# mazrk7/gmvae

Hardware: NVIDIA B200
Metric: GMVAE train samples/sec (fwd+bwd+Adam) (higher is better)
Workload: dtype bf16

## Files before the change

### gmvae_b200/csrc/chain_sched.cuh

```cuda
#pragma once

#if defined(__CUDACC__)
#define GMVAE_SCHED_FN __host__ __device__ __forceinline__
#else
#define GMVAE_SCHED_FN inline
#endif

namespace gmvae {
namespace tc {

constexpr int CHAIN_MAX_DEPS = 4;
constexpr int CHAIN_EPI_BYTES = 128;
constexpr int CHAIN_EPI2_BYTES = 64;
constexpr int SCHED_BLOCK_M = 128;

struct ChainDep { int base, target, by_k, nblocks, seg2; };

struct alignas(16) ChainJob {
  int a1, b1, a2, b2;
  int c;
  int d;
  int gw;
  int M, N, kb1, kb2, kb_per_split, num_splits;
  int block_n, a_mn, b_mn, kind;
  int tiles_n, tiles_mn, total_tiles, tile_base;
  int sig_base;
  int ndeps;
  int epi_dep;
  ChainDep deps[CHAIN_MAX_DEPS];
  alignas(16) unsigned char epi[CHAIN_EPI_BYTES];
  int rot;
  int walk_total;
  int tiles_mn2;
  int wfirst, wcount;
  int share;
  int fuse;
  int zslice;
  alignas(16) unsigned char epi2[CHAIN_EPI2_BYTES];
};
template <int CL>
GMVAE_SCHED_FN void chain_tile(const ChainJob& J, int l, int crank, int& z, int& mb, int& n0) {
  int mn;
  if (CL == 4) {
    z = l / J.tiles_mn2;
    mn = 2 * (l - z * J.tiles_mn2) + (crank >> 1);
  } else {
    z = l / J.tiles_mn;
    mn = l - z * J.tiles_mn;
  }
  int pm = mn / J.tiles_n;
  int nt = mn - pm * J.tiles_n;
  if (CL == 4 && mn >= J.tiles_mn) { pm = J.tiles_mn / J.tiles_n; nt = 0; }
  if (J.rot) { nt += pm % J.tiles_n; if (nt >= J.tiles_n) nt -= J.tiles_n; }
  n0 = nt * J.block_n;
  mb = CL >= 2 ? 2 * pm + (crank & 1) : pm;
}

template <int MUL>
GMVAE_SCHED_FN bool chain_walk(const ChainJob& J, int c, int G, int& first, int& stride) {
  int wf = J.wfirst * MUL, wc = J.wcount * MUL;
  if (wc <= 0 || wf + wc > G) { wf = 0; wc = G; }
  const int cj = c - wf;
  if (cj < 0 || cj >= wc) return false;
  stride = wc;
  first = ((cj - J.tile_base) % wc + wc) % wc;
  return true;
}

inline void chain_job_geometry(ChainJob& J, int M, int N, int block_n, int split_k, int kb_total, bool a_mn, int cl) {
  const int tiles_m = (M + SCHED_BLOCK_M - 1) / SCHED_BLOCK_M, tiles_n = (N + block_n - 1) / block_n;
  const int tiles_m_walk = cl >= 2 ? (tiles_m + 1) / 2 : tiles_m;
  if (split_k < 1) split_k = 1;
  const int per = (kb_total + split_k - 1) / split_k;
  split_k = (kb_total + per - 1) / per;
  J.M = M; J.N = N; J.kb_per_split = per; J.num_splits = split_k;
  J.block_n = block_n; J.a_mn = a_mn ? 1 : 0;
  J.tiles_n = tiles_n; J.tiles_mn = tiles_m_walk * tiles_n; J.total_tiles = J.tiles_mn * split_k;
  J.tiles_mn2 = (J.tiles_mn + 1) / 2;
  J.walk_total = cl == 4 ? J.tiles_mn2 * split_k : J.total_tiles;
  J.share = (cl == 4 && tiles_n % 2 == 0) ? 1 : 0;
  J.rot = (tiles_n > 1 && N % block_n != 0 && !a_mn) ? 1 : 0;
}
GMVAE_SCHED_FN int det_slice_ld(int N) { return (N + 3) / 4 * 4; }
GMVAE_SCHED_FN long long det_slice_index(int z, int m, int n, int M, int ld) { return ((long long)z * M + m) * ld + n; }
GMVAE_SCHED_FN void det_tile_region(const ChainJob& J, int mb, int n0, int& r0, int& r1, int& c0, int& c1) {
  r0 = mb * SCHED_BLOCK_M; r1 = r0 + SCHED_BLOCK_M < J.M ? r0 + SCHED_BLOCK_M : J.M;
  c0 = n0; c1 = n0 + J.block_n < J.N ? n0 + J.block_n : J.N;
  if (r1 < r0) r1 = r0;
}

inline int chain_job_counters(int M, int cl) {
  const int tiles_m = (M + SCHED_BLOCK_M - 1) / SCHED_BLOCK_M;
  return cl >= 2 ? 2 * ((tiles_m + 1) / 2) + (cl == 4 ? 2 : 0) : tiles_m;
}

}
}
```

### gmvae_b200/csrc/engine.cu

```cuda
#include <nccl.h>

#include <algorithm>
#include <cstdio>
#include <cstdlib>
#include <cstring>
#include <functional>
#include <map>
#include <mutex>
#include <string>
#include <tuple>
#include <type_traits>
#include <vector>

#include "../../include/gmvae_abi.h"
#include "common.cuh"
#include "epilogue.cuh"
#include "gemm_simt.cuh"
#include "gemm_tc.cuh"
#include "gemm_chain.cuh"
#include "kernels.cuh"
#include "input.cuh"
#include "peer.cuh"

namespace gmvae {

bool g_use_pdl = true;
static thread_local std::string g_last_error;
void set_error(const std::string& msg) { g_last_error = msg; }

namespace tc {
EncodeTiledFn get_encode_fn() {
  static EncodeTiledFn fn = nullptr;
  static std::once_flag once;
  std::call_once(once, [] {
    void* p = nullptr;
    cudaDriverEntryPointQueryResult q;
    if (cudaGetDriverEntryPoint("cuTensorMapEncodeTiled", &p, cudaEnableDefault, &q) == cudaSuccess &&
        q == cudaDriverEntryPointSuccess)
      fn = reinterpret_cast<EncodeTiledFn>(p);
  });
  return fn;
}

long long* g_trace = nullptr;

int g_reserved_sms = 0;

int current_device() { int dev = 0; cudaGetDevice(&dev); return dev < 0 ? 0 : dev % 64; }
int num_sms() {
  static int n_by_dev[64] = {};
  int& n = n_by_dev[current_device()];
  if (n == 0) {
    int dev = 0;
    cudaGetDevice(&dev);
    cudaDeviceGetAttribute(&n, cudaDevAttrMultiProcessorCount, dev);
    if (n <= 0) n = 148;
  }
  return std::max(8, n - g_reserved_sms);
}

int make_tmap(CUtensorMap* out, const void* ptr, int elem_bytes, uint64_t inner, uint64_t outer, uint64_t outer_stride,
              uint32_t box_inner, uint32_t box_outer, int swizzle) {
  typedef std::tuple<const void*, int, uint64_t, uint64_t, uint64_t, uint32_t, uint32_t, int> Key;
  static thread_local std::map<Key, CUtensorMap> cache;
  Key key(ptr, elem_bytes, inner, outer, outer_stride, box_inner, box_outer, swizzle);
  auto it = cache.find(key);
  if (it != cache.end()) { *out = it->second; return 0; }
  EncodeTiledFn fn = get_encode_fn();
  GM_REQUIRE(fn != nullptr, "cuTensorMapEncodeTiled not available from the driver");
  GM_REQUIRE((reinterpret_cast<uintptr_t>(ptr) & 15) == 0, "TMA operand base must be 16-byte aligned");
  GM_REQUIRE((outer_stride * (uint64_t)elem_bytes) % 16 == 0, "TMA operand row stride must be a multiple of 16 bytes");
  cuuint64_t gdim[2] = {inner, outer};
  cuuint64_t gstride[1] = {outer_stride * (uint64_t)elem_bytes};
  cuuint32_t box[2] = {box_inner, box_outer};
  cuuint32_t estr[2] = {1, 1};
  const CUtensorMapDataType dt = elem_bytes == 2 ? CU_TENSOR_MAP_DATA_TYPE_BFLOAT16 : elem_bytes == 4 ? CU_TENSOR_MAP_DATA_TYPE_FLOAT32
                                                                                                      : CU_TENSOR_MAP_DATA_TYPE_UINT8;
  const CUtensorMapSwizzle sw = swizzle == 128 ? CU_TENSOR_MAP_SWIZZLE_128B : swizzle == 64 ? CU_TENSOR_MAP_SWIZZLE_64B
                                                                                             : CU_TENSOR_MAP_SWIZZLE_NONE;
  CUresult r = fn(out, dt, 2, const_cast<void*>(ptr), gdim, gstride, box, estr, CU_TENSOR_MAP_INTERLEAVE_NONE, sw,
                  CU_TENSOR_MAP_L2_PROMOTION_L2_256B, CU_TENSOR_MAP_FLOAT_OOB_FILL_NONE);
  if (r != CUDA_SUCCESS) {
    set_error("cuTensorMapEncodeTiled failed with CUresult " + std::to_string((int)r));
    return -3;
  }
  if (cache.size() > 4096) cache.clear();
  cache[key] = *out;
  return 0;
}
int make_tmap_bf16(CUtensorMap* out, const void* ptr, uint64_t inner, uint64_t outer, uint64_t outer_stride,
                   uint32_t box_inner, uint32_t box_outer) {
  return make_tmap(out, ptr, 2, inner, outer, outer_stride, box_inner, box_outer, 128);
}
int make_tmap_slices_f32(CUtensorMap* out, const void* ptr, uint64_t inner, uint64_t outer, uint64_t slices, uint64_t ld,
                         uint32_t box_inner, uint32_t box_outer) {
  EncodeTiledFn fn = get_encode_fn();
  GM_REQUIRE(fn != nullptr, "cuTensorMapEncodeTiled not available from the driver");
  GM_REQUIRE((reinterpret_cast<uintptr_t>(ptr) & 15) == 0 && ld % 4 == 0, "TMA slices need 16-byte aligned rows");
  cuuint64_t gdim[3] = {inner, outer, slices};
  cuuint64_t gstride[2] = {ld * 4, outer * ld * 4};
  cuuint32_t box[3] = {box_inner, box_outer, 1};
  cuuint32_t estr[3] = {1, 1, 1};
  CUresult r = fn(out, CU_TENSOR_MAP_DATA_TYPE_FLOAT32, 3, const_cast<void*>(ptr), gdim, gstride, box, estr, CU_TENSOR_MAP_INTERLEAVE_NONE,
                  CU_TENSOR_MAP_SWIZZLE_64B, CU_TENSOR_MAP_L2_PROMOTION_L2_256B, CU_TENSOR_MAP_FLOAT_OOB_FILL_NONE);
  if (r != CUDA_SUCCESS) {
    set_error("cuTensorMapEncodeTiled (slices) failed with CUresult " + std::to_string((int)r));
    return -3;
  }
  return 0;
}
}

static inline int round_up(int v, int m) { return (v + m - 1) / m * m; }

struct Linear {
  int in = 0, out = 0;
  int64_t w_off = 0, b_off = 0;
  bf16* w_bf16 = nullptr;  int ld_w = 0;
};
struct Mlp {
  std::string name;
  std::vector<Linear> layers;
};

struct LinView {
  const float* w; float* dw; const float* b; float* db;
  int in, out, ldw32;
  const bf16* w_bf16; int ld_w;
};

enum { DBG_NO_TC = 1, DBG_NO_TC_WGRAD = 2, DBG_NO_TWO_SEG = 4, DBG_SYNC_EACH = 8, DBG_BN128 = 16, DBG_NO_FUSED_COLSUM = 32,
       DBG_NO_PDL = 128, DBG_NO_CHAIN = 512, DBG_NO_ROW_JOBS = 1024, DBG_NO_SPREAD = 4096, DBG_NO_FUSE_HEADS = 16384,
       DBG_COMM_OVERLAP = 32768 ,
       DBG_ROW_JOBS = 8192 ,
       DBG_NO_PAIR = 65536 ,
       DBG_NO_QUAD = 131072 ,
       DBG_WG_LATE = 262144 ,
       DBG_NO_PARTITION = 524288 ,
       DBG_NO_RELU_BITS = 2048  };
enum { PC_START = -1, PC_TC_GEMM = 0, PC_TC_WGRAD = 1, PC_SIMT_GEMM = 2, PC_HEADS = 3, PC_BIAS_GRAD = 4, PC_ADAM = 5, PC_MISC = 6,
       PC_COMM = 7, PC_COUNT = 8 };

}

using namespace gmvae;

struct gmvae_handle {
  gmvae_config cfg;
  int D, Z, K, L;
  std::vector<int> hidden;
  std::vector<gmvae_param_desc> table;
  int64_t n_params = 0;
  Mlp prior_gmm, decoder, encoder_y, encoder;
  int64_t loc_off = -1, raw_scale_off = -1, mix_off = -1;
  float *params = nullptr, *grads = nullptr, *adam_m = nullptr, *adam_v = nullptr;
  uint8_t* ws = nullptr; size_t ws_bytes = 0;
  struct Buf { size_t off = 0, bytes = 0; };
  std::map<std::string, Buf> bufs;
  size_t ws_needed = 0;
  std::vector<ShadowEntry> shadow_host;
  ShadowEntry* shadow_dev = nullptr; int shadow_tiles = 0;
  DeviceState* state = nullptr;
  uint64_t seed_host = 0;
  bool grads_clean = false;
  bool graph_has_memset = true;
  uint64_t draws = 0;
  bool in_train_step = false;
  int64_t launches = 0;
  int debug_flags = 0;
  bool profiling = false;
  std::vector<std::pair<cudaEvent_t, int>> marks;
  ncclComm_t comm = nullptr; int world = 1, rank = 0;
  cudaStream_t comm_stream = nullptr;
  cudaEvent_t comm_ev[8] = {nullptr, nullptr, nullptr, nullptr, nullptr, nullptr, nullptr, nullptr};
  int comm_ev_next = 0;
  bool overlap_comm = false;
  bool peer_ready = false;
  void* peer_region = nullptr;
  void* peer_mapped[peer::MAX_WORLD] = {};
  long long peer_timeout_cycles = 0;
  float* grads_bound = nullptr;
  peer::Layout peer_layout;
  peer::Peers peer_ptrs;
  int64_t reduced_upto = 0;
  int64_t bucket_end[2] = {0, 0};
  int chunk_samples = 0;
  bool chain_on = false;
  tc::ChainParams chain;
  struct ChainWriter { const char* lo; const char* hi; int job; };
  std::vector<ChainWriter> chain_writers;
  int chain_tiles = 0;
  int max_quads = 0;
  int* chain_counters = nullptr; int chain_counter_cap = 0, chain_counter_next = 0;
  long long* chain_trace = nullptr; int chain_trace_cta = 0, chain_launch_idx = 0;
  unsigned long long* chain_jobstat = nullptr;
  std::vector<int> chain_jobdesc;
  bool chain_flush_after = false;
  bool row_jobs = false;
  bool quad_opt_in = false;
  int chain_split_opt = 0;
  int wide_bn = 0;
  std::vector<std::function<int()>>* wg_late = nullptr;
  int cur_part = 0, part_chain_walkers = 0, part_walkers = 0, part_tiles[3] = {0, 0, 0};
  bool part_on = false, part_last_mlp = false, part_tail = false;
  bool chain_quad = false;
  bool chain_pair = false;
  struct FuseReq { int kind = 0; unsigned char prm[tc::CHAIN_EPI2_BYTES]; std::vector<std::pair<const void*, size_t>> writes; bool consumed = false; };
  FuseReq fuse_next;
  bool last_gemm_chained = false;
  std::map<const void*, bool> relu_bits_valid;
  bool det = false;
  std::vector<DetSeg> det_segs;
  std::vector<std::function<int()>> det_colsums;
  int64_t det_part_next = 0, det_part_cap = 0;
  int64_t det_wg_next = 0, det_wg_cap = 0;
  cudaGraphExec_t graph_exec = nullptr;

  bool bf16_mode() const { return cfg.precision == GMVAE_PRECISION_BF16; }
  size_t act_size() const { return bf16_mode() ? 2 : 4; }
  template <typename T> T* buf(const std::string& name) const {
    auto it = bufs.find(name);
    return it == bufs.end() ? nullptr : reinterpret_cast<T*>(ws + it->second.off);
  }
};

namespace gmvae {

static void add_param(gmvae_handle* h, const std::string& name, int rows, int cols, int64_t* off_out) {
  gmvae_param_desc d;
  memset(&d, 0, sizeof(d));
  snprintf(d.name, GMVAE_NAME_LEN, "%s", name.c_str());
  d.offset = h->n_params; d.rows = rows; d.cols = cols;
  h->table.push_back(d);
  if (off_out) *off_out = h->n_params;
  h->n_params += round_up(rows * cols, 4);
}

static void build_mlp(gmvae_handle* h, Mlp& m, const std::string& name, int in, const std::vector<int>& sizes) {
  m.name = name;
  int prev = in;
  for (size_t i = 0; i < sizes.size(); ++i) {
    Linear l; l.in = prev; l.out = sizes[i];
    add_param(h, name + "_fcnet/linear_" + std::to_string(i) + "/w", l.in, l.out, &l.w_off);
    add_param(h, name + "_fcnet/linear_" + std::to_string(i) + "/b", 1, l.out, &l.b_off);
    m.layers.push_back(l);
    prev = sizes[i];
  }
}

static void plan_buf(gmvae_handle* h, const std::string& name, size_t bytes) {
  gmvae_handle::Buf b; b.off = h->ws_needed; b.bytes = bytes;
  h->bufs[name] = b;
  h->ws_needed += (bytes + 255) / 256 * 256;
}

static void plan_mlp_bufs(gmvae_handle* h, const Mlp& m, size_t B, size_t asz) {
  for (size_t i = 0; i + 1 < m.layers.size(); ++i) {
    plan_buf(h, m.name + ".h" + std::to_string(i), B * round_up(m.layers[i].out, 8) * asz);
    plan_buf(h, m.name + ".dh" + std::to_string(i), B * round_up(m.layers[i].out, 8) * asz);
    plan_buf(h, m.name + ".bits" + std::to_string(i), (size_t)round_up((int)B, 32) * (size_t)((m.layers[i].out + 31) / 32) * 4);
  }
}

static void plan_shadows(gmvae_handle* h, Mlp& m) {
  for (auto& l : m.layers) {
    l.ld_w = round_up(l.out, 8);
    plan_buf(h, "shadow.w." + std::to_string(l.w_off), (size_t)l.in * l.ld_w * 2);
  }
}

constexpr int DET_ROW_BLOCKS = 64;
static int wgrad_split(const gmvae_handle* h, int in, int out, int M, bool pair, bool quad);

static int plan(gmvae_handle* h) {
  const gmvae_config& c = h->cfg;
  h->D = c.data_size; h->Z = c.latent_size; h->K = c.model == GMVAE_MODEL_VAE ? 1 : c.mixture_components;
  h->hidden.assign(c.hidden_sizes, c.hidden_sizes + c.num_hidden);
  h->L = c.num_hidden + 1;
  const int D = h->D, Z = h->Z, K = h->K;
  auto with = [&](int last) { std::vector<int> v = h->hidden; v.push_back(last); return v; };
  if (c.model == GMVAE_MODEL_GMVAE) {
    build_mlp(h, h->decoder, "decoder", Z, with(D));
    h->bucket_end[0] = h->n_params;
    build_mlp(h, h->encoder, "encoder_gmm", D + K, with(2 * Z));
    build_mlp(h, h->prior_gmm, "prior_gmm", K, std::vector<int>{2 * Z});
    h->bucket_end[1] = h->n_params;
    build_mlp(h, h->encoder_y, "encoder_y", D, with(K));
  } else {
    build_mlp(h, h->decoder, "decoder", Z, with(D));
    h->bucket_end[0] = h->n_params;
    if (c.model == GMVAE_MODEL_VAE_GMP) {
      add_param(h, "loc", K, Z, &h->loc_off);
      add_param(h, "raw_scale_diag", K, Z, &h->raw_scale_off);
      add_param(h, "mixture_logits", 1, K, &h->mix_off);
    }
    h->bucket_end[1] = h->n_params;
    build_mlp(h, h->encoder, "encoder", D, with(2 * Z));
  }
  const size_t Bfull = (size_t)c.max_batch, asz = h->act_size();
  const int Kp = round_up(K, 8);
  h->chunk_samples = (int)Bfull;
  if (c.objective == GMVAE_OBJECTIVE_MARGINAL) {
    const char* env = getenv("GMVAE_M_CHUNK_ROWS");
    long max_rows = env ? atol(env) : 131072;
    long bc = std::max(1L, max_rows / K);
    if (bc > 64) bc = bc / 64 * 64;
    h->chunk_samples = (int)std::min<long>((long)Bfull, bc);
  }
  const size_t B = c.objective == GMVAE_OBJECTIVE_MARGINAL ? (size_t)h->chunk_samples * K : Bfull;
  plan_buf(h, "x_act", Bfull * round_up(D, 8) * asz);
  plan_buf(h, "eps", Bfull * (c.objective == GMVAE_OBJECTIVE_MARGINAL ? K : 1) * Z * 4);
  plan_buf(h, "dec.dlogits", B * round_up(D, 8) * asz);
  plan_buf(h, "dz", B * Z * 4);
  plan_buf(h, "enc_out", B * 2 * Z * 4);
  plan_buf(h, "d_enc_out", B * round_up(2 * Z, 8) * asz);
  plan_buf(h, "z_act", B * round_up(Z, 8) * asz);
  plan_mlp_bufs(h, h->decoder, B, asz);
  plan_mlp_bufs(h, h->encoder, B, asz);
  if (c.model == GMVAE_MODEL_GMVAE) {
    plan_mlp_bufs(h, h->encoder_y, Bfull, asz);
    plan_buf(h, "u", Bfull * K * 4);
    plan_buf(h, "logits_y", Bfull * K * 4);
    plan_buf(h, "y_f32", Bfull * K * 4);
    plan_buf(h, "y_act", Bfull * Kp * asz);
    plan_buf(h, "dlogits_y", Bfull * Kp * asz);
    const size_t H0 = (size_t)(h->hidden.empty() ? 2 * Z : h->hidden[0]);
    if (c.objective == GMVAE_OBJECTIVE_MARGINAL) {
      plan_buf(h, "tab", (size_t)K * 2 * Z * 4);
      plan_buf(h, "dtab", (size_t)K * 2 * Z * 4);
      plan_buf(h, "xproj", Bfull * H0 * 4);
      plan_buf(h, "dxproj", Bfull * round_up((int)H0, 8) * asz);
      plan_buf(h, "rec", Bfull * K * 8);
      plan_buf(h, "klrow", Bfull * K * 4);
    } else {
      plan_buf(h, "prior_out", Bfull * 2 * Z * 4);
      plan_buf(h, "d_prior_out", Bfull * round_up(2 * Z, 8) * asz);
      plan_buf(h, "dy", Bfull * K * 4);
      plan_buf(h, "pre_y", Bfull * H0 * 4);
    }
  }
  if (c.model == GMVAE_MODEL_VAE_GMP) {
    plan_buf(h, "z_f32", B * Z * 4);
    plan_buf(h, "dz_prior", B * Z * 4);
  }
  if (h->bf16_mode()) {
    plan_shadows(h, h->decoder); plan_shadows(h, h->encoder);
    if (c.model == GMVAE_MODEL_GMVAE) { plan_shadows(h, h->encoder_y); plan_shadows(h, h->prior_gmm); }
  }
  plan_buf(h, "infer.acc", ACC_SLOTS * 4);
  if (c.deterministic) {
    int64_t cols = 0;
    for (const Mlp* m : {&h->decoder, &h->encoder, &h->encoder_y, &h->prior_gmm})
      for (const Linear& l : m->layers) cols += l.out;
    h->det_part_cap = cols * DET_ROW_BLOCKS;
    plan_buf(h, "det.part", (size_t)h->det_part_cap * 4);
    plan_buf(h, "det.fx", (size_t)(3 + (c.model == GMVAE_MODEL_VAE_GMP ? K + 2 * K * Z : 0)) * 16);
    h->det_wg_cap = 0;
    for (const Mlp* m : {&h->decoder, &h->encoder, &h->encoder_y, &h->prior_gmm})
      for (size_t i = 0; i < m->layers.size(); ++i) {
        const Linear& l = m->layers[i];
        std::vector<int> views{l.in};
        if (m == &h->encoder && i == 0 && c.model == GMVAE_MODEL_GMVAE) views = {D, K};
        for (int in : views) {
          const int kb = (int)((Bfull + tc::BLOCK_K - 1) / tc::BLOCK_K);
          int S = 1;
          for (bool pair : {false, true}) S = std::max(S, wgrad_split(h, in, l.out, (int)Bfull, pair, false));
          S = std::min(S, kb);
          h->det_wg_cap += round_up((int)std::min<int64_t>((int64_t)S * in * tc::det_slice_ld(l.out), 1LL << 30), 64);
        }
      }
    plan_buf(h, "det.wg", (size_t)h->det_wg_cap * 4);
  }
  h->chain_counter_cap = 64 * (int)((Bfull + 127) / 128 + 2);
  plan_buf(h, "chain.counters", (size_t)h->chain_counter_cap * 4);
  return 0;
}

static LinView view(const gmvae_handle* h, const Linear& l, int row0 = 0, int rows = -1) {
  if (rows < 0) rows = l.in - row0;
  LinView v;
  v.w = h->params + l.w_off + (int64_t)row0 * l.out;
  v.dw = h->grads + l.w_off + (int64_t)row0 * l.out;
  v.b = h->params + l.b_off; v.db = h->grads + l.b_off;
  v.in = rows; v.out = l.out; v.ldw32 = l.out;
  v.w_bf16 = l.w_bf16 ? l.w_bf16 + (int64_t)row0 * l.ld_w : nullptr; v.ld_w = l.ld_w;
  return v;
}

static int profile_mark(gmvae_handle* h, cudaStream_t st, int cls) {
  cudaEvent_t e;
  GM_CHECK_CUDA(cudaEventCreate(&e));
  GM_CHECK_CUDA(cudaEventRecord(e, st));
  h->marks.emplace_back(e, cls);
  return 0;
}

static int chain_flush(gmvae_handle* h, cudaStream_t st);
static int comm_bucket(gmvae_handle* h, cudaStream_t st, int64_t upto) {
  if (!h->comm || h->world == 1 || !h->overlap_comm || upto <= h->reduced_upto) return 0;
  GM_TRY(chain_flush(h, st));
  cudaEvent_t ev = h->comm_ev[h->comm_ev_next++ % 8];
  GM_CHECK_CUDA(cudaEventRecord(ev, st));
  GM_CHECK_CUDA(cudaStreamWaitEvent(h->comm_stream, ev, 0));
  ncclResult_t r = ncclAllReduce(h->grads + h->reduced_upto, h->grads + h->reduced_upto, (size_t)(upto - h->reduced_upto), ncclFloat,
                                 ncclSum, h->comm, h->comm_stream);
  if (r != ncclSuccess) { set_error(std::string("ncclAllReduce: ") + ncclGetErrorString(r)); return -5; }
  h->reduced_upto = upto;
  h->launches++;
  return 0;
}

#define GM_LAUNCHED(h, st, cls)                                              \
  do {                                                                       \
    (h)->launches++;                                                         \
    if ((h)->profiling) GM_TRY(profile_mark(h, st, cls));                    \
    if ((h)->debug_flags & DBG_SYNC_EACH) GM_CHECK_CUDA(cudaStreamSynchronize(st)); \
  } while (0)

static inline bool aligned16(const void* p) { return (reinterpret_cast<uintptr_t>(p) & 15) == 0; }
static inline int kpad(int k, int64_t ld) { return (int)std::min<int64_t>(ld, round_up(k, 8)); }

template <typename TA>
static bool tc_ok_fwd(const gmvae_handle* h, const TA* A, int64_t lda, const LinView& L) {
  return std::is_same<TA, bf16>::value && h->bf16_mode() && !(h->debug_flags & DBG_NO_TC) && L.w_bf16 && lda % 8 == 0 &&
         aligned16(A) && aligned16(L.w_bf16);
}
template <typename TD>
static bool tc_ok_dgrad(const gmvae_handle* h, const TD* dY, int64_t ldy, const LinView& L) {
  return std::is_same<TD, bf16>::value && h->bf16_mode() && !(h->debug_flags & DBG_NO_TC) && L.w_bf16 && ldy % 8 == 0 &&
         aligned16(dY) && aligned16(L.w_bf16);
}


static int pair_max_clusters(gmvae_handle* h, int* out) {
  static int max_clusters_by_dev[64] = {};
  int& max_clusters = max_clusters_by_dev[tc::current_device()];
  if (max_clusters == 0) {
    GM_CHECK_CUDA(cudaFuncSetAttribute(tc::gemm_chain_kernel<tc::ChainParams, 2>, cudaFuncAttributeMaxDynamicSharedMemorySize, tc::CHAIN_SMEM_BYTES));
    cudaLaunchConfig_t qc = {};
    qc.gridDim = dim3(tc::num_sms() & ~1); qc.blockDim = dim3(tc::NUM_THREADS2); qc.dynamicSmemBytes = tc::CHAIN_SMEM_BYTES;
    cudaLaunchAttribute qa[1];
    qa[0].id = cudaLaunchAttributeClusterDimension; qa[0].val.clusterDim.x = 2; qa[0].val.clusterDim.y = 1; qa[0].val.clusterDim.z = 1;
    qc.attrs = qa; qc.numAttrs = 1;
    int n = 0;
    GM_CHECK_CUDA(cudaOccupancyMaxActiveClusters(&n, tc::gemm_chain_kernel<tc::ChainParams, 2>, &qc));
    GM_REQUIRE(n >= 1, "the device cannot co-schedule a CTA pair of the chained kernel");
    max_clusters = n;
  }
  *out = max_clusters;
  return 0;
}

static int chain_flush(gmvae_handle* h, cudaStream_t st) {
  h->chain_flush_after = false;
  h->last_gemm_chained = false;
  if (h->chain.njobs == 0) return 0;
  static bool attr_set_by_dev[64] = {};
  bool& attr_set = attr_set_by_dev[tc::current_device()];
  if (!attr_set) {
    GM_CHECK_CUDA(cudaFuncSetAttribute(tc::gemm_chain_kernel<tc::ChainParams, 1>, cudaFuncAttributeMaxDynamicSharedMemorySize, tc::CHAIN_SMEM_BYTES));
    GM_CHECK_CUDA(cudaFuncSetAttribute(tc::gemm_chain_kernel<tc::ChainParamsSmall, 1>, cudaFuncAttributeMaxDynamicSharedMemorySize, tc::CHAIN_SMEM_BYTES));
    attr_set = true;
  }
  h->chain.counters = h->chain_counters;
  h->chain.trace = (h->chain_trace && h->chain_launch_idx < 8) ? h->chain_trace + (size_t)h->chain_launch_idx * 64 * 16 : nullptr;
  h->chain.trace_cta = h->chain_trace_cta;
  { static const int abl = getenv("GMVAE_CHAIN_ABL") ? atoi(getenv("GMVAE_CHAIN_ABL")) : 0; h->chain.abl = abl; }
  h->chain.jobstat = (h->chain_jobstat && h->chain_launch_idx == 0) ? h->chain_jobstat : nullptr;
  if (h->chain.jobstat) {
    h->chain_jobdesc.clear();
    for (int j = 0; j < h->chain.njobs; ++j) {
      const tc::ChainJob& J = h->chain.jobs[j];
      const int d[8] = {J.kind, J.M, J.N, J.kb1 + J.kb2, J.total_tiles, J.num_splits, J.block_n, J.ndeps};
      h->chain_jobdesc.insert(h->chain_jobdesc.end(), d, d + 8);
    }
  }
  h->chain_launch_idx++;
  if (h->chain_quad) {
    const int clusters = std::max(1, std::min(h->chain_tiles, h->max_quads));
    GM_CHECK_CUDA(launch_k_cluster(tc::gemm_chain_kernel<tc::ChainParams, 4>, dim3(4 * clusters), dim3(tc::NUM_THREADS2), (size_t)tc::CHAIN_SMEM_BYTES, st, true, 4,
                           h->chain));
  } else if (h->chain_pair) {
    int max_clusters = 0;
    GM_TRY(pair_max_clusters(h, &max_clusters));
    const int pairs = std::max(1, std::min(std::min(h->chain_tiles, tc::num_sms() / 2), max_clusters));
    GM_CHECK_CUDA(launch_k_cluster(tc::gemm_chain_kernel<tc::ChainParams, 2>, dim3(2 * pairs), dim3(tc::NUM_THREADS2), (size_t)tc::CHAIN_SMEM_BYTES, st, true, 2,
                           h->chain));
  } else {
  const int grid = std::min(h->chain_tiles, tc::num_sms());
  if (h->chain.njobs <= tc::CHAIN_SMALL_JOBS && h->chain.nmaps <= tc::CHAIN_SMALL_MAPS) {
    static tc::ChainParamsSmall small;
    small.njobs = h->chain.njobs; small.nmaps = h->chain.nmaps; small.counters = h->chain.counters;
    small.trace = h->chain.trace; small.trace_cta = h->chain.trace_cta; small.jobstat = h->chain.jobstat; small.abl = h->chain.abl;
    memcpy(small.maps, h->chain.maps, sizeof(CUtensorMap) * h->chain.nmaps);
    memcpy(small.jobs, h->chain.jobs, sizeof(tc::ChainJob) * h->chain.njobs);
    GM_CHECK_CUDA(launch_k(tc::gemm_chain_kernel<tc::ChainParamsSmall, 1>, dim3(grid), dim3(tc::NUM_THREADS2), (size_t)tc::CHAIN_SMEM_BYTES, st, true, small));
  } else {
    GM_CHECK_CUDA(launch_k(tc::gemm_chain_kernel<tc::ChainParams, 1>, dim3(grid), dim3(tc::NUM_THREADS2), (size_t)tc::CHAIN_SMEM_BYTES, st, true, h->chain));
  }
  }
  h->chain.njobs = 0; h->chain.nmaps = 0; h->chain_tiles = 0; h->chain_writers.clear();
  h->launches++;
  if (h->profiling) GM_TRY(profile_mark(h, st, 0 ));
  if (h->debug_flags & DBG_SYNC_EACH) GM_CHECK_CUDA(cudaStreamSynchronize(st));
  return 0;
}

template <typename T, int MODE> static void writer_range(const EpiStore<T, MODE>& e, int M, const char*& lo, const char*& hi) {
  lo = reinterpret_cast<const char*>(e.out); hi = lo + (int64_t)M * e.ld * sizeof(T);
}
template <typename T> static void writer_range(const EpiBCE<T>& e, int M, const char*& lo, const char*& hi) {
  lo = reinterpret_cast<const char*>(e.dlogits); hi = lo + (int64_t)M * e.ld * sizeof(T);
}
template <typename T, typename HT> static void writer_range(const EpiReluMask<T, HT>& e, int M, const char*& lo, const char*& hi) {
  lo = reinterpret_cast<const char*>(e.out); hi = lo + (int64_t)M * e.ld * sizeof(T);
}
static void writer_range(const EpiAtomicAdd&, int, const char*& lo, const char*& hi) { lo = hi = nullptr; }

struct ChainIO { const void* out; int64_t ld; int elem; const void* opnd; int64_t ld_opnd; bool ok; };
static ChainIO chain_io(const EpiStore<bf16, EPI_PLAIN>& e) { return {e.out, e.ld, 2, nullptr, 0, true}; }
static ChainIO chain_io(const EpiStore<float, EPI_PLAIN>& e) { return {nullptr, e.ld, 4, nullptr, 0, true}; }
static ChainIO chain_io(const EpiBCE<bf16>& e) {
  return {e.dlogits, e.ld, 2, nullptr, 0, e.row_weight == nullptr && e.row_sum == nullptr && e.x_row_div == 1};
}
static ChainIO chain_io(const EpiReluMask<bf16, bf16>& e) { return {e.out, e.ld, 2, e.h, e.ldh, true}; }
static ChainIO chain_io(const EpiAtomicAdd& e) {
  const bool tma = e.ld % 4 == 0 && (reinterpret_cast<uintptr_t>(e.out) & 15) == 0;
  return {tma ? e.out : nullptr, e.ld, 4, nullptr, 0, true};
}

template <class Epi>
static int chain_add(gmvae_handle* h, const tc::Operand& A1, const tc::Operand& B1, const tc::Operand* A2, const tc::Operand* B2,
                     int M, int N, int block_n, bool a_mn, bool b_mn, int split_k, const Epi& epi, cudaStream_t st) {
  static_assert(tc::epi_kind<Epi>::value != tc::EK_NONE, "epilogue not supported by the chained kernel");
  static_assert(sizeof(Epi) <= tc::CHAIN_EPI_BYTES, "epilogue parameters do not fit the job record");
  const bool pair = h->chain_pair, quad = h->chain_quad;
  const void* reads[4] = {A1.ptr, A2 ? A2->ptr : nullptr, a_mn ? (const void*)B1.ptr : nullptr, epi.read_ptr()};
  tc::ChainDep deps[tc::CHAIN_MAX_DEPS]; int ndeps = 0, epi_dep = -1;
  bool need_flush = h->chain.njobs >= tc::CHAIN_MAX_JOBS || h->chain.nmaps + 6 > tc::CHAIN_MAX_MAPS;
  for (int i = 0; i < 4 && !need_flush; ++i) {
    const char* p = reinterpret_cast<const char*>(reads[i]);
    if (!p) continue;
    for (const auto& w : h->chain_writers) {
      if (p < w.lo || p >= w.hi) continue;
      const tc::ChainJob& P = h->chain.jobs[w.job];
      if (p != w.lo || P.sig_base < 0) { need_flush = true; break; }
      int dup = -1;
      for (int d = 0; d < ndeps; ++d) if (deps[d].base == P.sig_base) dup = d;
      if (dup >= 0) {
        if (i == 3) { if (deps[dup].by_k) { need_flush = true; break; } epi_dep = dup; }
        if (i != 1) deps[dup].seg2 = 0;
        continue;
      }
      if (ndeps == tc::CHAIN_MAX_DEPS) { need_flush = true; break; }
      if (i == 3) epi_dep = ndeps;
      const bool by_k = a_mn && i != 3;
      deps[ndeps++] = tc::ChainDep{P.sig_base, tc::EPI_WARPS * P.tiles_n * P.num_splits, by_k ? 1 : 0, (P.M + tc::BLOCK_M - 1) / tc::BLOCK_M,
                                   (i == 1 && !a_mn) ? 1 : 0};
    }
  }
  if (need_flush) { GM_TRY(chain_flush(h, st)); ndeps = 0; epi_dep = -1; }
  tc::ChainJob& J = h->chain.jobs[h->chain.njobs];
  auto mk = [&](int* idx, const tc::Operand& o, bool mn, int box_rows) -> int {
    CUtensorMap* m = &h->chain.maps[h->chain.nmaps];
    *idx = h->chain.nmaps++;
    if (mn) return tc::make_tmap_bf16(m, o.ptr, (uint64_t)o.rows, (uint64_t)o.k, (uint64_t)o.ld, 64, tc::BLOCK_K);
    return tc::make_tmap_bf16(m, o.ptr, (uint64_t)o.k, (uint64_t)o.rows, (uint64_t)o.ld, tc::BLOCK_K, (uint32_t)box_rows);
  };
  const int b_box_rows = pair ? block_n / 2 : block_n;
  GM_REQUIRE(!pair || block_n % 16 == 0, "pair tiles need a tile width that is a multiple of 16");
  const int a_box_rows = quad ? 64 : tc::BLOCK_M;
  GM_TRY(mk(&J.a1, A1, a_mn, a_box_rows));
  GM_TRY(mk(&J.b1, B1, b_mn, b_box_rows));
  J.kb1 = (A1.k + tc::BLOCK_K - 1) / tc::BLOCK_K; J.kb2 = 0;
  if (A2 && B2) {
    GM_TRY(mk(&J.a2, *A2, a_mn, a_box_rows));
    GM_TRY(mk(&J.b2, *B2, b_mn, b_box_rows));
    J.kb2 = (A2->k + tc::BLOCK_K - 1) / tc::BLOCK_K;
  } else {
    J.a2 = J.a1; J.b2 = J.b1;
  }
  const int kb_total = J.kb1 + J.kb2;
  tc::chain_job_geometry(J, M, N, block_n, split_k, kb_total, a_mn, quad ? 4 : pair ? 2 : 1);
  J.b_mn = b_mn ? 1 : 0; J.kind = tc::epi_kind<Epi>::value;
  J.tile_base = h->chain_tiles;
  {
    const int part = h->part_on ? h->cur_part : 0;
    J.wfirst = part == 2 ? h->part_chain_walkers : 0;
    J.wcount = part == 1 ? h->part_chain_walkers : part == 2 ? h->part_walkers - h->part_chain_walkers : 0;
    J.tile_base = part == 0 ? h->chain_tiles : h->part_tiles[part];
    h->part_tiles[part] += J.walk_total;
  }
  J.ndeps = ndeps; J.epi_dep = epi_dep;
  for (int d = 0; d < ndeps; ++d) J.deps[d] = deps[d];
  const char *lo, *hi;
  writer_range(epi, M, lo, hi);
  J.sig_base = -1;
  if (lo) {
    const int ncount = tc::chain_job_counters(M, quad ? 4 : pair ? 2 : 1);
    if (h->chain_counter_next + ncount <= h->chain_counter_cap) {
      J.sig_base = h->chain_counter_next; h->chain_counter_next += ncount;
    } else {
      h->chain_flush_after = true;
    }
    h->chain_writers.push_back({lo, hi, h->chain.njobs});
  }
  const ChainIO io = chain_io(epi);
  J.gw = 0; J.c = J.a1; J.d = J.a1;
  J.zslice = (h->det && tc::epi_kind<Epi>::value == tc::EK_ATOMIC) ? 1 : 0;
  GM_REQUIRE(!J.zslice || io.out, "deterministic mode: weight-gradient slices need 16-byte rows");
  if (io.out) {
    J.gw = io.elem == 2 ? 2 : 1;
    J.d = h->chain.nmaps++;
    if (J.zslice)
      GM_TRY(tc::make_tmap_slices_f32(&h->chain.maps[J.d], io.out, (uint64_t)N, (uint64_t)M, (uint64_t)J.num_splits, (uint64_t)io.ld, 16, 32));
    else
      GM_TRY(tc::make_tmap(&h->chain.maps[J.d], io.out, io.elem, (uint64_t)N, (uint64_t)M, (uint64_t)io.ld, io.elem == 2 ? 32 : 16, 32, 64));
    if (io.opnd) {
      J.c = h->chain.nmaps++;
      GM_TRY(tc::make_tmap(&h->chain.maps[J.c], io.opnd, 2, (uint64_t)N, (uint64_t)M, (uint64_t)io.ld_opnd, 32, 32, 64));
    }
  }
  memset(J.epi, 0, sizeof(J.epi));
  memcpy(J.epi, &epi, sizeof(Epi));
  J.fuse = 0;
  if (h->fuse_next.kind != 0 && tc::epi_kind<Epi>::value == tc::EK_STORE_F32 && N <= 16 && J.sig_base >= 0) {
    J.fuse = h->fuse_next.kind;
    memcpy(J.epi2, h->fuse_next.prm, sizeof(J.epi2));
    for (const auto& w : h->fuse_next.writes)
      if (w.first) h->chain_writers.push_back({reinterpret_cast<const char*>(w.first), reinterpret_cast<const char*>(w.first) + w.second, h->chain.njobs});
    h->fuse_next.consumed = true;
  }
  h->chain_tiles += J.walk_total;
  h->chain.njobs++;
  h->last_gemm_chained = true;
  if (h->chain_flush_after) GM_TRY(chain_flush(h, st));
  return 0;
}
template <class P>
static int chain_add_rows(gmvae_handle* h, int kind, const P& prm, int M, std::initializer_list<const void*> reads,
                          std::initializer_list<std::pair<const void*, size_t>> writes, cudaStream_t st, int sub = 1) {
  static_assert(sizeof(P) <= tc::CHAIN_EPI_BYTES, "row-job parameters do not fit the job record");
  const int tiles_m = (M + tc::BLOCK_M - 1) / tc::BLOCK_M;
  tc::ChainDep deps[tc::CHAIN_MAX_DEPS]; int ndeps = 0;
  bool need_flush = h->chain.njobs >= tc::CHAIN_MAX_JOBS;
  for (const void* r : reads) {
    const char* p = reinterpret_cast<const char*>(r);
    if (!p || need_flush) continue;
    for (const auto& w : h->chain_writers) {
      if (p < w.lo || p >= w.hi) continue;
      const tc::ChainJob& Pj = h->chain.jobs[w.job];
      if (p != w.lo || Pj.sig_base < 0) { need_flush = true; break; }
      bool dup = false;
      for (int d = 0; d < ndeps; ++d) dup = dup || deps[d].base == Pj.sig_base;
      if (dup) continue;
      if (ndeps == tc::CHAIN_MAX_DEPS) { need_flush = true; break; }
      deps[ndeps++] = tc::ChainDep{Pj.sig_base, tc::EPI_WARPS * Pj.tiles_n * Pj.num_splits, 0, (Pj.M + tc::BLOCK_M - 1) / tc::BLOCK_M, 0};
    }
  }
  if (need_flush) { GM_TRY(chain_flush(h, st)); ndeps = 0; }
  tc::ChainJob& J = h->chain.jobs[h->chain.njobs];
  memset(&J, 0, sizeof(J));
  J.M = M; J.N = 0; J.kind = kind; J.num_splits = 1;
  J.tiles_n = sub; J.tiles_mn = tiles_m * sub; J.total_tiles = tiles_m * sub; J.tile_base = (h->chain_quad ? 4 : h->chain_pair ? 2 : 1) * h->chain_tiles;
  {
    const int cl = h->chain_quad ? 4 : h->chain_pair ? 2 : 1;
    const int part = h->part_on ? h->cur_part : 0;
    J.wfirst = part == 2 ? h->part_chain_walkers : 0;
    J.wcount = part == 1 ? h->part_chain_walkers : part == 2 ? h->part_walkers - h->part_chain_walkers : 0;
    if (part != 0) J.tile_base = cl * h->part_tiles[part];
    h->part_tiles[part] += (tiles_m * sub + cl - 1) / cl;
  }
  J.ndeps = ndeps; J.epi_dep = -1;
  for (int d = 0; d < ndeps; ++d) J.deps[d] = deps[d];
  J.sig_base = -1;
  if (h->chain_counter_next + tiles_m <= h->chain_counter_cap) {
    J.sig_base = h->chain_counter_next; h->chain_counter_next += tiles_m;
  } else {
    h->chain_flush_after = true;
  }
  for (const auto& w : writes)
    if (w.first) h->chain_writers.push_back({reinterpret_cast<const char*>(w.first), reinterpret_cast<const char*>(w.first) + w.second, h->chain.njobs});
  memcpy(J.epi, &prm, sizeof(P));
  { const int cl = h->chain_quad ? 4 : h->chain_pair ? 2 : 1; h->chain_tiles += (J.total_tiles + cl - 1) / cl; }
  h->chain.njobs++;
  if (h->chain_flush_after) GM_TRY(chain_flush(h, st));
  return 0;
}
template <class Epi> struct chainable { static constexpr bool value = tc::epi_kind<Epi>::value != tc::EK_NONE; };

template <class Epi, bool B_MN = false>
static int tc_dispatch_kk(gmvae_handle* h, const tc::Operand& A, const tc::Operand& B, const tc::Operand* A2,
                          const tc::Operand* B2, int M, int N, const Epi& epi, cudaStream_t st) {
  int r;
  if constexpr (chainable<Epi>::value) {
    if (h->chain_on && chain_io(epi).ok) {
      const bool f32 = tc::epi_kind<Epi>::value == tc::EK_STORE_F32;
      int bn = (!B_MN && f32 && N <= 16) ? 16 : (!B_MN && f32 && N <= 32) ? 32 : N <= 64 ? 64 : (N <= 128 || (h->debug_flags & DBG_BN128)) ? 128 : 256;
      if (bn == 256 && h->wide_bn > 0 && N > h->wide_bn) bn = h->wide_bn;
      return chain_add(h, A, B, A2, B2, M, N, bn, false, B_MN, 1, epi, st);
    }
  }
  GM_TRY(chain_flush(h, st));
  if constexpr (B_MN) {
    if (N <= 64) r = tc::launch_gemm_tc<64, false, true, Epi>(A, B, A2, B2, M, N, 1, epi, st);
    else if (N <= 128 || (h->debug_flags & DBG_BN128)) r = tc::launch_gemm_tc<128, false, true, Epi>(A, B, A2, B2, M, N, 1, epi, st);
    else r = tc::launch_gemm_tc<256, false, true, Epi>(A, B, A2, B2, M, N, 1, epi, st);
  } else {
    if (N <= 16) r = tc::launch_gemm_tc<16, false, false, Epi>(A, B, A2, B2, M, N, 1, epi, st);
    else if (N <= 32) r = tc::launch_gemm_tc<32, false, false, Epi>(A, B, A2, B2, M, N, 1, epi, st);
    else if (N <= 64) r = tc::launch_gemm_tc<64, false, false, Epi>(A, B, A2, B2, M, N, 1, epi, st);
    else if (N <= 128 || (h->debug_flags & DBG_BN128)) r = tc::launch_gemm_tc<128, false, false, Epi>(A, B, A2, B2, M, N, 1, epi, st);
    else r = tc::launch_gemm_tc<256, false, false, Epi>(A, B, A2, B2, M, N, 1, epi, st);
  }
  if (r == 0) GM_LAUNCHED(h, st, PC_TC_GEMM);
  return r;
}

template <typename TA, class Epi, bool ALLOW_TC = true>
static int lin_fwd(gmvae_handle* h, const TA* A, int64_t lda, int M, const LinView& L, const Epi& epi, cudaStream_t st,
                   const TA* A2 = nullptr, int64_t lda2 = 0, const LinView* L2 = nullptr) {
  if constexpr (ALLOW_TC && std::is_same<TA, bf16>::value) {
    bool ok = tc_ok_fwd<TA>(h, A, lda, L);
    if (L2) ok = ok && lda2 % 8 == 0 && aligned16(A2) && aligned16(L2->w_bf16);
    if (ok) {
      tc::Operand a{A, lda, M, kpad(L.in, lda)}, b{L.w_bf16, L.ld_w, L.out, L.in};
      if (L2) {
        tc::Operand a2{A2, lda2, M, kpad(L2->in, lda2)}, b2{L2->w_bf16, L2->ld_w, L2->out, L2->in};
        return tc_dispatch_kk<Epi, true>(h, a, b, &a2, &b2, M, L.out, epi, st);
      }
      return tc_dispatch_kk<Epi, true>(h, a, b, nullptr, nullptr, M, L.out, epi, st);
    }
  }
  GM_REQUIRE(L2 == nullptr, "two-segment forward requires the tensor-core path");
  GM_TRY(chain_flush(h, st));
  GM_CHECK_CUDA((launch_gemm_simt<TA, float, Epi>(A, lda, 1, L.w, L.ldw32, 1, M, L.out, L.in, 1, epi, st)));
  GM_LAUNCHED(h, st, PC_SIMT_GEMM);
  return 0;
}

template <typename TD, class Epi>
static int lin_dgrad(gmvae_handle* h, const TD* dY, int64_t ldy, int M, const LinView& L, const Epi& epi, cudaStream_t st,
                     const TD* dY2 = nullptr, int64_t ldy2 = 0, const LinView* L2 = nullptr) {
  if constexpr (std::is_same<TD, bf16>::value) {
    bool ok = tc_ok_dgrad<TD>(h, dY, ldy, L);
    if (L2) ok = ok && tc_ok_dgrad<TD>(h, dY2, ldy2, *L2) && L2->in == L.in;
    if (ok) {
      tc::Operand a{dY, ldy, M, kpad(L.out, ldy)}, b{L.w_bf16, L.ld_w, L.in, kpad(L.out, L.ld_w)};
      if (L2) {
        tc::Operand a2{dY2, ldy2, M, kpad(L2->out, ldy2)}, b2{L2->w_bf16, L2->ld_w, L2->in, kpad(L2->out, L2->ld_w)};
        return tc_dispatch_kk(h, a, b, &a2, &b2, M, L.in, epi, st);
      }
      return tc_dispatch_kk(h, a, b, nullptr, nullptr, M, L.in, epi, st);
    }
  }
  GM_REQUIRE(L2 == nullptr, "two-segment data gradient requires the tensor-core path");
  GM_TRY(chain_flush(h, st));
  GM_CHECK_CUDA((launch_gemm_simt<TD, float, Epi>(dY, ldy, 1, L.w, 1, L.ldw32, M, L.in, L.out, 1, epi, st)));
  GM_LAUNCHED(h, st, PC_SIMT_GEMM);
  return 0;
}

static int wgrad_bn(const gmvae_handle* h, int out) { return out <= 64 ? 64 : (out <= 128 || (h->debug_flags & DBG_BN128)) ? 128 : 256; }
static int wgrad_split(const gmvae_handle* h, int in, int out, int M, bool pair, bool quad) {
  const int bn = wgrad_bn(h, out);
  const int tiles = pair ? ((in + 255) / 256) * ((out + bn - 1) / bn) : ((in + 127) / 128) * ((out + bn - 1) / bn);
  const int kb = (M + tc::BLOCK_K - 1) / tc::BLOCK_K;
  const int walkers = quad ? h->max_quads : pair ? tc::num_sms() / 2 : tc::num_sms(), units = quad ? (tiles + 1) / 2 : tiles;
  return std::max(1, std::min(std::max(1, kb / 4), walkers / units));
}

template <typename TA, typename TD>
static int lin_wgrad(gmvae_handle* h, const TA* A, int64_t lda, const TD* dY, int64_t ldy, int M, const LinView& L,
                     cudaStream_t st) {
  EpiAtomicAdd epi{L.dw, (int64_t)L.ldw32};
  if constexpr (std::is_same<TA, bf16>::value && std::is_same<TD, bf16>::value) {
    bool ok = h->bf16_mode() && !(h->debug_flags & (DBG_NO_TC | DBG_NO_TC_WGRAD)) && lda % 8 == 0 && ldy % 8 == 0 &&
              aligned16(A) && aligned16(dY);
    if (ok) {
      tc::Operand a{A, lda, kpad(L.in, lda), M}, b{dY, ldy, kpad(L.out, ldy), M};
      const int bn = wgrad_bn(h, L.out);
      const bool pair = h->chain_on && h->chain_pair;
      const int split = wgrad_split(h, L.in, L.out, M, pair, pair && h->chain_quad);
      if (h->chain_on) {
        EpiAtomicAdd e = epi;
        if (h->det) {
          const int kb = (M + tc::BLOCK_K - 1) / tc::BLOCK_K, per = (kb + split - 1) / split, S = (kb + per - 1) / per;
          const int ld = tc::det_slice_ld(L.out);
          const int64_t need = round_up((int)std::min<int64_t>((int64_t)S * L.in * ld, 1LL << 30), 64);
          GM_REQUIRE(h->det_wg_next + need <= h->det_wg_cap && (int)h->det_segs.size() < DET_MAX_SEGS,
                     "deterministic mode: out of weight-gradient partial space");
          float* part = h->buf<float>("det.wg") + h->det_wg_next;
          h->det_wg_next += need;
          e = EpiAtomicAdd{part, (int64_t)ld};
          h->det_segs.push_back(DetSeg{L.dw, part, nullptr, (long long)L.in * ld, L.in, L.out, S, L.ldw32, ld, 0});
        }
        const int saved_part = h->cur_part;
        if (saved_part == 1) h->cur_part = h->part_tail ? 0 : 2;
        const int r = chain_add(h, a, b, nullptr, nullptr, L.in, L.out, bn, true, true, split, e, st);
        h->cur_part = saved_part;
        return r;
      }
      GM_REQUIRE(!h->det, "deterministic mode: weight gradients outside the chained kernel");
      GM_TRY(chain_flush(h, st));
      int r = bn == 64    ? tc::launch_gemm_tc<64, true, true, EpiAtomicAdd>(a, b, nullptr, nullptr, L.in, L.out, split, epi, st)
              : bn == 128 ? tc::launch_gemm_tc<128, true, true, EpiAtomicAdd>(a, b, nullptr, nullptr, L.in, L.out, split, epi, st)
                          : tc::launch_gemm_tc<256, true, true, EpiAtomicAdd>(a, b, nullptr, nullptr, L.in, L.out, split, epi, st);
      if (r == 0) GM_LAUNCHED(h, st, PC_TC_WGRAD);
      return r;
    }
  }
  GM_TRY(chain_flush(h, st));
  const int tiles = ((L.in + SIMT_BM - 1) / SIMT_BM) * ((L.out + SIMT_BN - 1) / SIMT_BN);
  int split = std::max(1, std::min((M + 255) / 256, (4 * 148 + tiles - 1) / tiles));
  if (h->det) split = 1;
  GM_CHECK_CUDA((launch_gemm_simt<TA, TD, EpiAtomicAdd>(A, 1, lda, dY, ldy, 1, L.in, L.out, M, split, epi, st)));
  GM_LAUNCHED(h, st, PC_SIMT_GEMM);
  return 0;
}

template <typename T>
static int bias_grad(gmvae_handle* h, const T* dY, int64_t ldy, int M, int N, float* db, cudaStream_t st) {
  const int col_blocks = (N + 255) / 256;
  int rows_per_block = std::max(64, (M * col_blocks + 2 * 148 - 1) / (2 * 148));
  float* part = nullptr;
  if (h->det) {
    rows_per_block = std::max(8, (M + DET_ROW_BLOCKS - 1) / DET_ROW_BLOCKS);
    GM_REQUIRE(h->det_part_next + (int64_t)N * DET_ROW_BLOCKS <= h->det_part_cap && (int)h->det_segs.size() < DET_MAX_SEGS,
               "deterministic mode: out of partial-sum space");
    part = h->buf<float>("det.part") + h->det_part_next;
    h->det_part_next += (int64_t)N * DET_ROW_BLOCKS;
    h->det_segs.push_back(DetSeg{db, part, nullptr, N, 1, N, DET_ROW_BLOCKS, 0, N, 0});
    const int rpb = round_up(rows_per_block, 8);
    h->det_colsums.push_back([=]() -> int {
      GM_CHECK_CUDA(launch_k(colsum_kernel<T>, dim3(col_blocks, DET_ROW_BLOCKS), dim3(256), 0, st, true, dY, ldy, M, N, rpb, db, part));
      GM_LAUNCHED(h, st, PC_BIAS_GRAD);
      return 0;
    });
    return 0;
  }
  rows_per_block = round_up(rows_per_block, 8);
  dim3 grid(col_blocks, (M + rows_per_block - 1) / rows_per_block);
  GM_TRY(chain_flush(h, st));
  GM_CHECK_CUDA(launch_k(colsum_kernel<T>, grid, dim3(256), 0, st, true, dY, ldy, M, N, rows_per_block, db, part));
  GM_LAUNCHED(h, st, PC_BIAS_GRAD);
  return 0;
}

static inline int ldp(int n) { return round_up(n, 8); }

template <typename A> struct MlpBufs { std::vector<A*> hid, dhid; std::vector<uint32_t*> bits; };

template <typename A>
static MlpBufs<A> mlp_bufs(const gmvae_handle* h, const Mlp& m) {
  MlpBufs<A> b;
  for (size_t i = 0; i + 1 < m.layers.size(); ++i) {
    b.hid.push_back(h->buf<A>(m.name + ".h" + std::to_string(i)));
    b.dhid.push_back(h->buf<A>(m.name + ".dh" + std::to_string(i)));
    b.bits.push_back(h->buf<uint32_t>(m.name + ".bits" + std::to_string(i)));
  }
  return b;
}

template <typename A>
static int mlp_hidden_fwd(gmvae_handle* h, const Mlp& m, const MlpBufs<A>& b, const A* in0, int64_t ld0, int in0_cols, int M,
                          int first, cudaStream_t st) {
  const int nh = (int)m.layers.size() - 1;
  for (int i = first; i < nh; ++i) {
    const A* in = i == 0 ? in0 : b.hid[i - 1];
    int64_t ld = i == 0 ? ld0 : ldp(m.layers[i - 1].out);
    LinView L = view(h, m.layers[i], 0, i == 0 ? in0_cols : -1);
    EpiStore<A> epi{b.hid[i], (int64_t)ldp(m.layers[i].out), L.b, nullptr, 0, 1, 1.f};
    if (tc::CHAIN_RELU_BITS && h->chain_on && h->row_jobs && !(h->debug_flags & DBG_NO_RELU_BITS)) { epi.relu_bits = b.bits[i]; epi.ld_bits = round_up(M, 32); }
    GM_TRY(lin_fwd<A>(h, in, ld, M, L, epi, st));
    h->relu_bits_valid[b.hid[i]] = epi.relu_bits != nullptr && h->last_gemm_chained;
  }
  return 0;
}

template <typename A, typename TD>
static int mlp_backward(gmvae_handle* h, const Mlp& m, const MlpBufs<A>& b, const A* in0, int64_t ld0, int in0_cols,
                        const TD* dOut, int64_t ld_dout, int M, cudaStream_t st, bool dout_bias_done = false, int min_layer = 0,
                        std::vector<std::function<int()>>* defer = nullptr, int defer_below = 0) {
  const int nl = (int)m.layers.size();
  const bool fuse = !(h->debug_flags & DBG_NO_FUSED_COLSUM) && !h->det;
  bool bias_done = dout_bias_done;
  for (int i = nl - 1; i >= min_layer; --i) {
    const Linear& l = m.layers[i];
    const bool first = i == 0;
    LinView L = view(h, l, 0, first ? in0_cols : -1);
    const A* in = first ? in0 : b.hid[i - 1];
    const int64_t ld = first ? ld0 : ldp(m.layers[i - 1].out);
    const bool top = i == nl - 1;
    const A* dA = top ? nullptr : b.dhid[i];
    const int64_t ldd = top ? ld_dout : ldp(l.out);
    bool next_bias_done = false;
    if (!first) {
      LinView Lf = view(h, l);
      const int64_t ldh = ldp(m.layers[i - 1].out);
      const bool ok = top ? tc_ok_dgrad<TD>(h, dOut, ld_dout, Lf) : tc_ok_dgrad<A>(h, dA, ldd, Lf);
      float* cs = (fuse && i - 1 >= min_layer && ok) ? h->grads + m.layers[i - 1].b_off : nullptr;
      EpiReluMask<A, A> epi{b.dhid[i - 1], ldh, b.hid[i - 1], ldh, cs};
      {
        auto it = h->relu_bits_valid.find(b.hid[i - 1]);
        if (h->chain_on && it != h->relu_bits_valid.end() && it->second) { epi.relu_bits = b.bits[i - 1]; epi.ld_bits = round_up(M, 32); }
      }
      if (top) GM_TRY((lin_dgrad<TD>(h, dOut, ld_dout, M, Lf, epi, st)));
      else GM_TRY((lin_dgrad<A>(h, dA, ldd, M, Lf, epi, st)));
      next_bias_done = cs != nullptr;
      if (h->part_last_mlp && i == 1) h->part_tail = true;
    }
    const bool need_bias = !bias_done;
    const int out_cols = l.out;
    std::function<int()> wg;
    if (top) {
      wg = [=]() -> int {
        GM_TRY((lin_wgrad<A, TD>(h, in, ld, dOut, ld_dout, M, L, st)));
        if (need_bias) GM_TRY(bias_grad<TD>(h, dOut, ld_dout, M, out_cols, L.db, st));
        return 0;
      };
    } else {
      wg = [=]() -> int {
        GM_TRY((lin_wgrad<A, A>(h, in, ld, dA, ldd, M, L, st)));
        if (need_bias) GM_TRY(bias_grad<A>(h, dA, ldd, M, out_cols, L.db, st));
        return 0;
      };
    }
    if (h->wg_late) h->wg_late->push_back(wg);
    else if (defer && i < defer_below) defer->push_back(wg); else GM_TRY(wg());
    bias_done = next_bias_done;
  }
  return 0;
}

template <typename A>
static int forward_encoder(gmvae_handle* h, const uint8_t* x_u8, int B, float inv_bg, const float*& eps, const float*& u, float* acc,
                           cudaStream_t st) {
  const gmvae_config& c = h->cfg;
  const int D = h->D, Z = h->Z, K = h->K, nl = h->L;
  const int Dp = ldp(D), Kp = ldp(K);
  const bool gm = c.model == GMVAE_MODEL_GMVAE;
  A* x_act = h->buf<A>("x_act");
  {
    const int64_t n = (int64_t)B * D;
    const bool need_noise = !eps || (gm && !u);
    const uint64_t draw = (need_noise && !h->in_train_step) ? ++h->draws : 0;
    float* e = h->buf<float>("eps"); float* uu = gm ? h->buf<float>("u") : nullptr;
    const int64_t ne = eps ? 0 : (int64_t)B * Z, nu = (gm && !u) ? (int64_t)B * K : 0;
    const int64_t q = (ne + 3) / 4 + (nu + 3) / 4;
    if (D % 16 == 0 && need_noise) {
      const unsigned xb = (unsigned)((n / 16 + 255) / 256), nb = (unsigned)((q + 255) / 256);
      GM_CHECK_CUDA(launch_k(prologue_kernel<A>, dim3(xb + nb), dim3(256), 0, st, false, x_u8, x_act, n, (int)xb, e, ne, uu, nu,
                             (const DeviceState*)h->state, (uint64_t)h->rank, draw));
      GM_LAUNCHED(h, st, PC_MISC);
    } else {
      if (D % 16 == 0) GM_CHECK_CUDA(launch_k(convert_x_kernel<A>, dim3((unsigned)((n / 16 + 255) / 256)), dim3(256), 0, st, false, x_u8, x_act, n));
      else GM_CHECK_CUDA(launch_k(convert_x_rows_kernel<A>, dim3((unsigned)((n + 255) / 256)), dim3(256), 0, st, false, x_u8, x_act, B, D, Dp));
      GM_LAUNCHED(h, st, PC_MISC);
      if (need_noise) {
        GM_CHECK_CUDA(launch_k(fill_noise_kernel, dim3((unsigned)((q + 255) / 256)), dim3(256), 0, st, true, e, ne, uu, nu,
                               (const DeviceState*)h->state, (uint64_t)h->rank, 1, draw));
        GM_LAUNCHED(h, st, PC_MISC);
      }
    }
    if (gm && u) {
      const int64_t nuu = (int64_t)B * K;
      GM_CHECK_CUDA(launch_k(gumbel_from_u_kernel, dim3((unsigned)((nuu + 255) / 256)), dim3(256), 0, st, true, u, uu, nuu));
      GM_LAUNCHED(h, st, PC_MISC);
      u = uu;
    }
    if (!eps) eps = e;
    if (gm && !u) u = uu;
  }
  MlpBufs<A> enc = mlp_bufs<A>(h, h->encoder);
  float* enc_out = h->buf<float>("enc_out");
  const Linear& enc_l0 = h->encoder.layers[0];
  const Linear& enc_last = h->encoder.layers[nl - 1];
  auto hid_ld = [&](int i) { return (int64_t)ldp(h->hidden[i]); };
  if (gm) {
    MlpBufs<A> ey = mlp_bufs<A>(h, h->encoder_y);
    float* logits_y = h->buf<float>("logits_y"); float* y_f32 = h->buf<float>("y_f32"); A* y_act = h->buf<A>("y_act");
    float* prior_out = h->buf<float>("prior_out");
    GM_TRY(mlp_hidden_fwd<A>(h, h->encoder_y, ey, x_act, Dp, D, B, 0, st));
    const bool rows_ok = h->chain_on && h->row_jobs;
    bool y_fused = false;
    {
      const Linear& l = h->encoder_y.layers[nl - 1];
      EpiStore<float> epi{logits_y, (int64_t)K, h->params + l.b_off, nullptr, 0, 0, 1.f};
      if (rows_ok && K <= 16 && Kp <= 16 && u && !(h->debug_flags & DBG_NO_FUSE_HEADS)) {
        tc::RowsYFwd prm{logits_y, u, K, 1.f / c.temperature, inv_bg, y_f32, reinterpret_cast<bf16*>(y_act), Kp, acc};
        h->fuse_next = gmvae_handle::FuseReq();
        h->fuse_next.kind = tc::EK_ROWS_Y_FWD;
        memcpy(h->fuse_next.prm, &prm, sizeof(prm));
        h->fuse_next.writes = {{y_f32, (size_t)B * K * 4}, {y_act, (size_t)B * Kp * 2}};
      }
      GM_TRY(lin_fwd<A>(h, nl == 1 ? x_act : ey.hid[nl - 2], nl == 1 ? Dp : hid_ld(nl - 2), B, view(h, l), epi, st));
      y_fused = h->fuse_next.consumed;
      h->fuse_next = gmvae_handle::FuseReq();
    }
    if (y_fused) {
    } else if (rows_ok && K <= 16 && Kp <= 16 && u) {
      tc::RowsYFwd prm{logits_y, u, K, 1.f / c.temperature, inv_bg, y_f32, reinterpret_cast<bf16*>(y_act), Kp, acc};
      GM_TRY(chain_add_rows(h, tc::EK_ROWS_Y_FWD, prm, B, {logits_y, u},
                            {{y_f32, (size_t)B * K * 4}, {y_act, (size_t)B * Kp * 2}}, st));
    } else {
    GM_TRY(chain_flush(h, st));
    if (std::is_same<A, bf16>::value && K <= 16 && Kp <= 16) {
      GM_CHECK_CUDA(launch_k(head_y_fwd_row_kernel, dim3((B + 127) / 128), dim3(128), 0, st, true, (const float*)logits_y, u, B, K,
                             1.f / c.temperature, inv_bg, y_f32, reinterpret_cast<bf16*>(y_act), Kp, acc));
    } else {
      GM_CHECK_CUDA(launch_k(head_y_fwd_kernel<A>, dim3((B + 7) / 8), dim3(256), 0, st, true, (const float*)logits_y, u, B, K,
                             1.f / c.temperature, inv_bg, y_f32, y_act, Kp, acc));
    }
    GM_LAUNCHED(h, st, PC_HEADS);
    }
    LinView Lx = view(h, enc_l0, 0, D), Ly = view(h, enc_l0, D, K);
    const bool last0 = nl == 1;
    const bool two_seg = tc_ok_fwd<A>(h, x_act, Dp, Lx) && tc_ok_fwd<A>(h, y_act, Kp, Ly) && !(h->debug_flags & DBG_NO_TWO_SEG);
    if (two_seg) {
      if (last0) {
        EpiStore<float> epi{enc_out, (int64_t)2 * Z, Lx.b, nullptr, 0, 0, 1.f};
        GM_TRY(lin_fwd<A>(h, x_act, Dp, B, Lx, epi, st, y_act, Kp, &Ly));
      } else {
        EpiStore<A> epi{enc.hid[0], hid_ld(0), Lx.b, nullptr, 0, 1, 1.f};
        if (tc::CHAIN_RELU_BITS && h->chain_on && h->row_jobs && !(h->debug_flags & DBG_NO_RELU_BITS)) { epi.relu_bits = enc.bits[0]; epi.ld_bits = round_up(B, 32); }
        GM_TRY(lin_fwd<A>(h, x_act, Dp, B, Lx, epi, st, y_act, Kp, &Ly));
        h->relu_bits_valid[enc.hid[0]] = epi.relu_bits != nullptr && h->last_gemm_chained;
      }
    } else {
      float* pre = h->buf<float>("pre_y");
      EpiStore<float> e0{pre, (int64_t)enc_l0.out, Lx.b, nullptr, 0, 0, 1.f};
      GM_TRY((lin_fwd<A, EpiStore<float>, false>(h, y_act, Kp, B, Ly, e0, st)));
      if (last0) {
        EpiStore<float, EPI_ADDEND> epi{enc_out, (int64_t)2 * Z, nullptr, pre, (int64_t)enc_l0.out, 0, 1.f};
        GM_TRY((lin_fwd<A, EpiStore<float, EPI_ADDEND>, false>(h, x_act, Dp, B, Lx, epi, st)));
      } else {
        EpiStore<A, EPI_ADDEND> epi{enc.hid[0], hid_ld(0), nullptr, pre, (int64_t)enc_l0.out, 1, 1.f};
        GM_TRY((lin_fwd<A, EpiStore<A, EPI_ADDEND>, false>(h, x_act, Dp, B, Lx, epi, st)));
      }
    }
    {
      const Linear& l = h->prior_gmm.layers[0];
      EpiStore<float> epi{prior_out, (int64_t)2 * Z, h->params + l.b_off, nullptr, 0, 0, 1.f};
      GM_TRY(lin_fwd<A>(h, y_act, Kp, B, view(h, l), epi, st));
    }
    GM_TRY(mlp_hidden_fwd<A>(h, h->encoder, enc, x_act, Dp, D, B, 1, st));
  } else {
    GM_TRY(mlp_hidden_fwd<A>(h, h->encoder, enc, x_act, Dp, D, B, 0, st));
  }
  if (nl > 1 || !gm) {
    EpiStore<float> epi{enc_out, (int64_t)2 * Z, h->params + enc_last.b_off, nullptr, 0, 0, 1.f};
    GM_TRY(lin_fwd<A>(h, nl == 1 ? x_act : enc.hid[nl - 2], nl == 1 ? Dp : hid_ld(nl - 2), B, view(h, enc_last, 0, nl == 1 ? D : -1),
                      epi, st));
  }
  return 0;
}

template <typename A>
static int forward_backward_body(gmvae_handle* h, const uint8_t* x_u8, int B, int Bg, const float* eps_in, const float* u_in, cudaStream_t st);

static int det_reduce(gmvae_handle* h, cudaStream_t st) {
  DetSegs segs;
  segs.nseg = (int)h->det_segs.size();
  long long nmax = 1;
  for (int i = 0; i < segs.nseg; ++i) { segs.s[i] = h->det_segs[i]; nmax = std::max(nmax, (long long)segs.s[i].rows * segs.s[i].cols); }
  GM_CHECK_CUDA(launch_k(det_reduce_kernel, dim3((unsigned)std::min(1024LL, (nmax + 255) / 256), segs.nseg), dim3(256), 0, st, true, segs));
  GM_LAUNCHED(h, st, PC_BIAS_GRAD);
  return 0;
}

template <typename A>
static int forward_backward_impl(gmvae_handle* h, const uint8_t* x_u8, int B, int Bg, const float* eps_in,
                                 const float* u_in, cudaStream_t st) {
  h->chain.njobs = 0; h->chain.nmaps = 0; h->chain_tiles = 0; h->chain_writers.clear(); h->chain_counter_next = 0; h->chain_launch_idx = 0;
  h->relu_bits_valid.clear();
  h->chain_counters = h->buf<int>("chain.counters");
  h->chain_on = std::is_same<A, bf16>::value && h->bf16_mode() && h->chain_counters && !(h->debug_flags & (DBG_NO_TC | DBG_NO_CHAIN));
  h->row_jobs = h->chain_on && !(h->debug_flags & DBG_NO_ROW_JOBS) && (B >= 32 * tc::BLOCK_M || (h->debug_flags & DBG_ROW_JOBS));
  h->chain_pair = h->row_jobs && !(h->debug_flags & DBG_NO_PAIR) && !(h->comm && h->world > 1 && h->overlap_comm) && tc::g_reserved_sms == 0;
  h->chain_quad = false;
  if (h->chain_pair && h->quad_opt_in && !(h->debug_flags & DBG_NO_QUAD)) {
    static int max_quads_by_dev[64] = {};
    int& mq = max_quads_by_dev[tc::current_device()];
    if (mq == 0) {
      GM_CHECK_CUDA(cudaFuncSetAttribute(tc::gemm_chain_kernel<tc::ChainParams, 4>, cudaFuncAttributeMaxDynamicSharedMemorySize, tc::CHAIN_SMEM_BYTES));
      cudaLaunchConfig_t qc = {};
      qc.gridDim = dim3(tc::num_sms() & ~3); qc.blockDim = dim3(tc::NUM_THREADS2); qc.dynamicSmemBytes = tc::CHAIN_SMEM_BYTES;
      cudaLaunchAttribute qa[1];
      qa[0].id = cudaLaunchAttributeClusterDimension; qa[0].val.clusterDim.x = 4; qa[0].val.clusterDim.y = 1; qa[0].val.clusterDim.z = 1;
      qc.attrs = qa; qc.numAttrs = 1;
      int n = 0;
      if (cudaOccupancyMaxActiveClusters(&n, tc::gemm_chain_kernel<tc::ChainParams, 4>, &qc) != cudaSuccess) { cudaGetLastError(); n = 0; }
      mq = n > 0 ? std::min(n, tc::num_sms() / 4) : -1;
      if (getenv("GMVAE_VERBOSE")) fprintf(stderr, "[gmvae] 4-CTA clusters of the chained kernel co-resident on this device: %d\n", n);
    }
    h->max_quads = mq;
    h->chain_quad = mq >= 28;
  }
  h->part_on = false; h->cur_part = 0; h->part_tail = false; h->part_last_mlp = false;
  h->part_tiles[0] = h->part_tiles[1] = h->part_tiles[2] = 0;
  if (h->chain_pair && !h->chain_quad && !(h->debug_flags & DBG_NO_PARTITION)) {
    int mc = 0;
    GM_TRY(pair_max_clusters(h, &mc));
    const int W = std::min(tc::num_sms() / 2, mc);
    const int split_env = h->chain_split_opt;
    const int x = split_env;
    if (x >= 4 && W - x >= 4) { h->part_on = true; h->part_walkers = W; h->part_chain_walkers = x; }
  }
  if (h->chain_on) GM_CHECK_CUDA(cudaMemsetAsync(h->chain_counters, 0, (size_t)h->chain_counter_cap * 4, st));
  int r = forward_backward_body<A>(h, x_u8, B, Bg, eps_in, u_in, st);
  if (r == 0) r = chain_flush(h, st);
  if (h->det) {
    for (auto& f : h->det_colsums) if (r == 0) r = f();
    h->det_colsums.clear();
    if (r == 0) r = det_reduce(h, st);
  }
  h->chain_on = false; h->chain_pair = false; h->chain_quad = false; h->chain.njobs = 0; h->chain.nmaps = 0;
  return r;
}

template <typename A>
static int forward_backward_body(gmvae_handle* h, const uint8_t* x_u8, int B, int Bg, const float* eps_in,
                                 const float* u_in, cudaStream_t st) {
  const gmvae_config& c = h->cfg;
  const int D = h->D, Z = h->Z, K = h->K, nl = h->L;
  const int Dp = ldp(D), Zp = ldp(Z), Z2p = ldp(2 * Z), Kp = ldp(K);
  const float inv_bg = 1.f / (float)Bg;
  const bool gm = c.model == GMVAE_MODEL_GMVAE;
  float* acc = h->grads + h->n_params;
  if (h->profiling) GM_TRY(profile_mark(h, st, PC_START));
  if (!h->grads_clean) GM_CHECK_CUDA(cudaMemsetAsync(h->grads, 0, (size_t)(h->n_params + ACC_SLOTS) * 4, st));
  h->grads_clean = false;
  h->reduced_upto = 0;
  unsigned long long* fx = h->det ? h->buf<unsigned long long>("det.fx") : nullptr;
  if (h->det) {
    const int nfx = 3 + (c.model == GMVAE_MODEL_VAE_GMP ? K + 2 * K * Z : 0);
    GM_CHECK_CUDA(cudaMemsetAsync(fx, 0, (size_t)nfx * 16, st));
    acc = acc_fixed_tag(fx);
    h->det_segs.clear(); h->det_colsums.clear(); h->det_part_next = 0; h->det_wg_next = 0;
    h->det_segs.push_back(DetSeg{h->grads + h->n_params, nullptr, fx, 0, 3, 1, 0, ACC_PER_TERM, 0, 0});
    if (c.model == GMVAE_MODEL_VAE_GMP) {
      h->det_segs.push_back(DetSeg{h->grads + h->mix_off, nullptr, fx + 2 * 3, 0, 1, K, 0, 0, 0, 0});
      h->det_segs.push_back(DetSeg{h->grads + h->loc_off, nullptr, fx + 2 * (3 + K), 0, 1, K * Z, 0, 0, 0, 0});
      h->det_segs.push_back(DetSeg{h->grads + h->raw_scale_off, nullptr, fx + 2 * (3 + K + K * Z), 0, 1, K * Z, 0, 0, 0, 0});
    }
  }

  const float* eps = eps_in; const float* u = u_in;
  GM_TRY(forward_encoder<A>(h, x_u8, B, inv_bg, eps, u, acc, st));

  A* x_act = h->buf<A>("x_act");
  MlpBufs<A> dec = mlp_bufs<A>(h, h->decoder), enc = mlp_bufs<A>(h, h->encoder);
  float* enc_out = h->buf<float>("enc_out");
  A* d_enc_out = h->buf<A>("d_enc_out");
  A* z_act = h->buf<A>("z_act");
  float* dz = h->buf<float>("dz");
  A* dlogits_x = h->buf<A>("dec.dlogits");
  const Linear& enc_l0 = h->encoder.layers[0];
  const Linear& enc_last = h->encoder.layers[nl - 1];
  auto hid_ld = [&](int i) { return (int64_t)ldp(h->hidden[i]); };
  MlpBufs<A> ey; float *logits_y = nullptr, *y_f32 = nullptr, *prior_out = nullptr; A* y_act = nullptr;
  if (gm) {
    ey = mlp_bufs<A>(h, h->encoder_y);
    logits_y = h->buf<float>("logits_y"); y_f32 = h->buf<float>("y_f32"); y_act = h->buf<A>("y_act");
    prior_out = h->buf<float>("prior_out");
  }
  const int prior_mode = gm ? 2 : (c.model == GMVAE_MODEL_VAE_GMP ? 1 : 0);
  float* z_f32 = h->buf<float>("z_f32");
  {
    int64_t n = (int64_t)B * Z;
    const bool v4 = std::is_same<A, bf16>::value && Z % 4 == 0 && Z <= 256 && aligned16(eps) && aligned16(enc_out) &&
                    (prior_mode != 2 || aligned16(prior_out));
    const bool rows_ok = h->chain_on && h->row_jobs && v4 && prior_mode != 1 && z_f32 == nullptr;
    if (rows_ok) {
      tc::RowsZFwd prm{enc_out, eps, prior_out, prior_mode, Z, c.raw_sigma_bias, c.sigma_min, inv_bg, reinterpret_cast<bf16*>(z_act), Zp, acc};
      GM_TRY(chain_add_rows(h, tc::EK_ROWS_Z_FWD, prm, B, {enc_out, eps, prior_out}, {{z_act, (size_t)B * Zp * 2}}, st, 4));
    } else {
    GM_TRY(chain_flush(h, st));
    if (v4) {
      const int blocks = (int)std::min<int64_t>((n / 4 + 255) / 256, 8 * tc::num_sms());
      GM_CHECK_CUDA(launch_k(head_z_fwd_v4_kernel, dim3(blocks), dim3(256), 0, st, true, (const float*)enc_out, eps, (const float*)prior_out,
                             prior_mode, B, Z, c.raw_sigma_bias, c.sigma_min, inv_bg, reinterpret_cast<bf16*>(z_act), Zp, z_f32, acc));
    } else {
      GM_CHECK_CUDA(launch_k(head_z_fwd_kernel<A>, dim3((unsigned)((n + 255) / 256)), dim3(256), 0, st, true, (const float*)enc_out, eps,
                             (const float*)prior_out, prior_mode, B, Z, c.raw_sigma_bias, c.sigma_min, inv_bg, z_act, Zp, z_f32, acc));
    }
    GM_LAUNCHED(h, st, PC_HEADS);
    }
  }
  float* dz_prior = h->buf<float>("dz_prior");
  if (prior_mode == 1) {
    const int warps = 4;
    GM_TRY(chain_flush(h, st));
    GM_CHECK_CUDA(launch_k(gmp_prior_kernel, dim3((B + warps - 1) / warps), dim3(warps * 32), warps * K * sizeof(float), st, true,
                           (const float*)z_f32, (const float*)(h->params + h->loc_off), (const float*)(h->params + h->raw_scale_off),
                           (const float*)(h->params + h->mix_off), B, K, Z, inv_bg, dz_prior, h->grads + h->loc_off,
                           h->grads + h->raw_scale_off, h->grads + h->mix_off, acc, fx ? fx + 2 * 3 : nullptr));
    GM_LAUNCHED(h, st, PC_HEADS);
  }
  bool dec_bias_fused = false;
  GM_TRY(mlp_hidden_fwd<A>(h, h->decoder, dec, z_act, Zp, Z, B, 0, st));
  {
    const Linear& l = h->decoder.layers[nl - 1];
    const A* in = nl == 1 ? z_act : dec.hid[nl - 2];
    const int64_t ldin = nl == 1 ? Zp : hid_ld(nl - 2);
    LinView Ld = view(h, l);
    dec_bias_fused = !(h->debug_flags & DBG_NO_FUSED_COLSUM) && !h->det && tc_ok_fwd<A>(h, in, ldin, Ld);
    EpiBCE<A> epi{dlogits_x, (int64_t)Dp, h->params + l.b_off, c.gen_bias_init, x_u8, (int64_t)D, 1, nullptr, (double*)nullptr,
                  acc, inv_bg, 0.f, dec_bias_fused ? h->grads + l.b_off : nullptr, h->bf16_mode() ? 1 : 0};
    GM_TRY(lin_fwd<A>(h, in, ldin, B, Ld, epi, st));
  }

  const bool spread = h->chain_on && h->row_jobs && !(h->debug_flags & DBG_NO_SPREAD) && !(h->comm && h->world > 1 && h->overlap_comm);
  std::vector<std::function<int()>> wg_late;
  struct WgLateGuard { gmvae_handle* h; ~WgLateGuard() { h->wg_late = nullptr; } } wg_late_guard{h};
  if (spread && (h->debug_flags & DBG_WG_LATE)) h->wg_late = &wg_late;
  struct PartGuard { gmvae_handle* h; ~PartGuard() { h->cur_part = 0; h->part_tail = false; h->part_last_mlp = false; } } part_guard{h};
  if (h->part_on && spread && !h->wg_late) h->cur_part = 1;
  std::vector<std::function<int()>> wg_dec;
  GM_TRY((mlp_backward<A, A>(h, h->decoder, dec, z_act, Zp, Z, dlogits_x, Dp, B, st, dec_bias_fused, 0, spread ? &wg_dec : nullptr,
                             std::min(2, nl - 1))));
  {
    const Linear& l0 = h->decoder.layers[0];
    EpiStore<float> epi{dz, (int64_t)Z, nullptr, nullptr, 0, 0, 1.f};
    if (nl == 1) GM_TRY((lin_dgrad<A>(h, dlogits_x, Dp, B, view(h, l0), epi, st)));
    else GM_TRY((lin_dgrad<A>(h, dec.dhid[0], hid_ld(0), B, view(h, l0), epi, st)));
  }
  size_t wg_dec_next = 0;
  if (wg_dec.size() > 1) GM_TRY(wg_dec[wg_dec_next++]());
  GM_TRY(comm_bucket(h, st, h->bucket_end[0]));
  A* d_prior_out = h->buf<A>("d_prior_out");
  bool enc_bias_fused = false;
  {
    int64_t n = (int64_t)B * Z;
    const bool z_cs_ok = Z <= 256 && !(h->debug_flags & DBG_NO_FUSED_COLSUM);
    enc_bias_fused = z_cs_ok && !h->det;
    const bool rows_ok = h->chain_on && h->row_jobs && z_cs_ok && prior_mode != 1 &&
                         (Z == 4 || Z == 8 || Z == 16 || Z == 32 || Z == 64) && aligned16(eps) && aligned16(enc_out) && aligned16(dz) &&
                         (prior_mode != 2 || aligned16(prior_out));
    if (rows_ok) {
      tc::RowsZBwd prm{enc_out, eps, prior_out, dz, prior_mode, Z, c.raw_sigma_bias, c.sigma_min, inv_bg, reinterpret_cast<bf16*>(d_enc_out),
                       reinterpret_cast<bf16*>(d_prior_out), Z2p, enc_bias_fused ? h->grads + enc_last.b_off : (float*)nullptr,
                       (gm && enc_bias_fused) ? h->grads + h->prior_gmm.layers[0].b_off : (float*)nullptr};
      GM_TRY(chain_add_rows(h, tc::EK_ROWS_Z_BWD, prm, B, {dz, enc_out, prior_out, eps},
                            {{d_enc_out, (size_t)B * Z2p * 2}, {gm ? d_prior_out : nullptr, (size_t)B * Z2p * 2}}, st, 4));
    } else {
    GM_TRY(chain_flush(h, st));
    const bool v4 = std::is_same<A, bf16>::value && enc_bias_fused && Z % 4 == 0 && aligned16(eps) && aligned16(enc_out) && aligned16(dz) &&
                    (prior_mode != 2 || aligned16(prior_out)) && (prior_mode != 1 || aligned16(dz_prior));
    if (v4) {
      const int rpi = 256 / (Z / 4);
      const int blocks = std::max(1, std::min(4 * tc::num_sms(), (B + rpi - 1) / rpi));
      GM_CHECK_CUDA(launch_k(head_z_bwd_v4_kernel, dim3(blocks), dim3(256), (size_t)16 * 256 * sizeof(float), st, true, (const float*)enc_out,
                             eps, (const float*)prior_out, (const float*)dz, (const float*)dz_prior, prior_mode, B, Z, c.raw_sigma_bias,
                             c.sigma_min, inv_bg, reinterpret_cast<bf16*>(d_enc_out), reinterpret_cast<bf16*>(d_prior_out), Z2p,
                             h->grads + enc_last.b_off, gm ? h->grads + h->prior_gmm.layers[0].b_off : (float*)nullptr));
    } else if (enc_bias_fused) {
      const int lanes = 256 / Z;
      const int blocks = std::max(1, std::min(2 * tc::num_sms(), (B + lanes - 1) / lanes));
      GM_CHECK_CUDA(launch_k(head_z_bwd_cs_kernel<A>, dim3(blocks), dim3(256), 4 * 256 * sizeof(float), st, true, (const float*)enc_out, eps,
                             (const float*)prior_out, (const float*)dz, (const float*)dz_prior, prior_mode, B, Z, c.raw_sigma_bias,
                             c.sigma_min, inv_bg, d_enc_out, d_prior_out, Z2p, h->grads + enc_last.b_off,
                             gm ? h->grads + h->prior_gmm.layers[0].b_off : (float*)nullptr));
    } else {
      GM_CHECK_CUDA(launch_k(head_z_bwd_kernel<A>, dim3((unsigned)((n + 255) / 256)), dim3(256), 0, st, true, (const float*)enc_out, eps,
                             (const float*)prior_out, (const float*)dz, (const float*)dz_prior, prior_mode, B, Z, c.raw_sigma_bias,
                             c.sigma_min, inv_bg, d_enc_out, d_prior_out, Z2p));
    }
    GM_LAUNCHED(h, st, PC_HEADS);
    }
  }
  for (; wg_dec_next < wg_dec.size(); ++wg_dec_next) GM_TRY(wg_dec[wg_dec_next]());
  std::vector<std::function<int()>> wg_enc;
  if (!gm) { h->part_last_mlp = true; if (h->encoder.layers.size() < 2) h->part_tail = true; }
  GM_TRY((mlp_backward<A, A>(h, h->encoder, enc, x_act, Dp, D, d_enc_out, Z2p, B, st, enc_bias_fused, 0, (spread && gm) ? &wg_enc : nullptr, 1)));
  if (gm) {
    float* dy = h->buf<float>("dy"); A* dlogits_y = h->buf<A>("dlogits_y");
    LinView Ly = view(h, enc_l0, D, K);
    const A* dh0 = nl == 1 ? d_enc_out : enc.dhid[0];
    const int64_t ld_dh0 = nl == 1 ? Z2p : hid_ld(0);
    const Linear& lp = h->prior_gmm.layers[0];
    LinView Lp = view(h, lp);
    const bool dy_two_seg = tc_ok_dgrad<A>(h, dh0, ld_dh0, Ly) && tc_ok_dgrad<A>(h, d_prior_out, Z2p, Lp) && !(h->debug_flags & DBG_NO_TWO_SEG);
    const bool y_cs_ok = !(h->debug_flags & DBG_NO_FUSED_COLSUM);
    const bool ey_bias_fused = y_cs_ok && !h->det;
    bool yb_fused = false;
    {
      EpiStore<float> e{dy, (int64_t)K, nullptr, nullptr, 0, 0, 1.f};
      if (dy_two_seg && h->chain_on && h->row_jobs && K <= 16 && Kp <= 16 && y_cs_ok && !(h->debug_flags & DBG_NO_FUSE_HEADS)) {
        tc::RowsYBwd prm{logits_y, y_f32, nullptr, K, 1.f / c.temperature, inv_bg, reinterpret_cast<bf16*>(dlogits_y), Kp,
                         ey_bias_fused ? h->grads + h->encoder_y.layers[nl - 1].b_off : (float*)nullptr};
        h->fuse_next = gmvae_handle::FuseReq();
        h->fuse_next.kind = tc::EK_ROWS_Y_BWD;
        memcpy(h->fuse_next.prm, &prm, sizeof(prm));
        h->fuse_next.writes = {{dlogits_y, (size_t)B * Kp * 2}};
      }
      if (dy_two_seg) GM_TRY((lin_dgrad<A>(h, dh0, ld_dh0, B, Ly, e, st, d_prior_out, Z2p, &Lp)));
      else GM_TRY((lin_dgrad<A>(h, dh0, ld_dh0, B, Ly, e, st)));
      yb_fused = h->fuse_next.consumed;
      h->fuse_next = gmvae_handle::FuseReq();
    }
    if (!dy_two_seg) {
      EpiStore<float, EPI_ACCUM> e{dy, (int64_t)K, nullptr, nullptr, 0, 0, 1.f};
      GM_TRY((lin_dgrad<A>(h, d_prior_out, Z2p, B, Lp, e, st)));
    }
    for (auto& f : wg_enc) GM_TRY(f());
    auto wg_y = [&]() -> int {
      GM_TRY((lin_wgrad<A, A>(h, y_act, Kp, dh0, ld_dh0, B, Ly, st)));
      GM_TRY((lin_wgrad<A, A>(h, y_act, Kp, d_prior_out, Z2p, B, Lp, st)));
      if (!enc_bias_fused) GM_TRY(bias_grad<A>(h, d_prior_out, Z2p, B, 2 * Z, Lp.db, st));
      return 0;
    };
    if (h->wg_late) h->wg_late->push_back(wg_y);
    else if (!spread) GM_TRY(wg_y());
    GM_TRY(comm_bucket(h, st, h->bucket_end[1]));
    if (yb_fused) {
    } else if (h->chain_on && h->row_jobs && K <= 16 && Kp <= 16) {
      tc::RowsYBwd prm{logits_y, y_f32, dy, K, 1.f / c.temperature, inv_bg, reinterpret_cast<bf16*>(dlogits_y), Kp,
                       ey_bias_fused ? h->grads + h->encoder_y.layers[nl - 1].b_off : (float*)nullptr};
      GM_TRY(chain_add_rows(h, tc::EK_ROWS_Y_BWD, prm, B, {dy, logits_y, y_f32}, {{dlogits_y, (size_t)B * Kp * 2}}, st));
    } else {
    GM_TRY(chain_flush(h, st));
    if (std::is_same<A, bf16>::value && K <= 16 && Kp <= 16) {
      GM_CHECK_CUDA(launch_k(head_y_bwd_row_kernel, dim3(std::max(1, std::min(tc::num_sms(), (B + 127) / 128))), dim3(128), 0, st, true,
                             (const float*)logits_y, (const float*)y_f32, (const float*)dy, B, K, 1.f / c.temperature, inv_bg,
                             reinterpret_cast<bf16*>(dlogits_y), Kp, ey_bias_fused ? h->grads + h->encoder_y.layers[nl - 1].b_off : (float*)nullptr));
    } else {
      GM_CHECK_CUDA(launch_k(head_y_bwd_kernel<A>, dim3(std::max(1, std::min(2 * tc::num_sms(), (B + 7) / 8))), dim3(256), 0, st, true,
                             (const float*)logits_y, (const float*)y_f32, (const float*)dy, B, K, 1.f / c.temperature, inv_bg, dlogits_y, Kp,
                             ey_bias_fused ? h->grads + h->encoder_y.layers[nl - 1].b_off : (float*)nullptr));
    }
    GM_LAUNCHED(h, st, PC_HEADS);
    }
    if (spread && !h->wg_late) GM_TRY(wg_y());
    h->part_last_mlp = true;
    if (h->encoder_y.layers.size() < 2) h->part_tail = true;
    GM_TRY((mlp_backward<A, A>(h, h->encoder_y, ey, x_act, Dp, D, dlogits_y, Kp, B, st, ey_bias_fused)));
    if (h->wg_late) {
      h->wg_late = nullptr;
      for (auto& f : wg_late) GM_TRY(f());
      wg_late.clear();
    }
  }
  if (h->wg_late) {
    h->wg_late = nullptr;
    for (auto& f : wg_late) GM_TRY(f());
  }
  return 0;
}


template <typename A>
static int forward_backward_marginal(gmvae_handle* h, const uint8_t* x_u8, int B, int Bg, const float* eps_in, cudaStream_t st) {
  const gmvae_config& c = h->cfg;
  const int D = h->D, Z = h->Z, K = h->K, nl = h->L;
  const int Dp = ldp(D), Zp = ldp(Z), Z2p = ldp(2 * Z), Kp = ldp(K);
  const float inv_bg = 1.f / (float)Bg;
  float* acc = h->grads + h->n_params;
  if (h->profiling) GM_TRY(profile_mark(h, st, PC_START));
  if (!h->grads_clean) GM_CHECK_CUDA(cudaMemsetAsync(h->grads, 0, (size_t)(h->n_params + ACC_SLOTS) * 4, st));
  h->grads_clean = false;
  h->reduced_upto = 0;
  double* rec = h->buf<double>("rec"); float* klrow = h->buf<float>("klrow");
  float* tab = h->buf<float>("tab"); float* dtab = h->buf<float>("dtab");
  GM_CHECK_CUDA(cudaMemsetAsync(rec, 0, (size_t)B * K * 8, st));
  GM_CHECK_CUDA(cudaMemsetAsync(dtab, 0, (size_t)K * 2 * Z * 4, st));

  A* x_act = h->buf<A>("x_act");
  {
    const int64_t n = (int64_t)B * D;
    if (D % 16 == 0) GM_CHECK_CUDA(launch_k(convert_x_kernel<A>, dim3((unsigned)((n / 16 + 255) / 256)), dim3(256), 0, st, false, x_u8, x_act, n));
    else GM_CHECK_CUDA(launch_k(convert_x_rows_kernel<A>, dim3((unsigned)((n + 255) / 256)), dim3(256), 0, st, false, x_u8, x_act, B, D, Dp));
    GM_LAUNCHED(h, st, PC_MISC);
  }
  const float* eps = eps_in;
  if (!eps) {
    float* e = h->buf<float>("eps");
    const int64_t ne = (int64_t)B * K * Z, q = (ne + 3) / 4;
    GM_CHECK_CUDA(launch_k(fill_noise_kernel, dim3((unsigned)((q + 255) / 256)), dim3(256), 0, st, true, e, ne, (float*)nullptr, (int64_t)0,
                           (const DeviceState*)h->state, (uint64_t)h->rank, 0, h->in_train_step ? (uint64_t)0 : ++h->draws));
    GM_LAUNCHED(h, st, PC_MISC);
    eps = e;
  }
  MlpBufs<A> dec = mlp_bufs<A>(h, h->decoder), enc = mlp_bufs<A>(h, h->encoder), ey = mlp_bufs<A>(h, h->encoder_y);
  float* enc_out = h->buf<float>("enc_out"); A* d_enc_out = h->buf<A>("d_enc_out");
  A* z_act = h->buf<A>("z_act"); float* dz = h->buf<float>("dz"); A* dlogits_x = h->buf<A>("dec.dlogits");
  float* logits_y = h->buf<float>("logits_y"); float* pi = h->buf<float>("y_f32"); A* y_act = h->buf<A>("y_act");
  float* xproj = h->buf<float>("xproj"); A* dxproj = h->buf<A>("dxproj"); A* dlogits_y = h->buf<A>("dlogits_y");
  const Linear& enc_l0 = h->encoder.layers[0];
  const Linear& enc_last = h->encoder.layers[nl - 1];
  const Linear& prior = h->prior_gmm.layers[0];
  const int H0 = enc_l0.out, H0p = ldp(H0);
  auto hid_ld = [&](int i) { return (int64_t)ldp(h->hidden[i]); };

  GM_TRY(mlp_hidden_fwd<A>(h, h->encoder_y, ey, x_act, Dp, D, B, 0, st));
  {
    const Linear& l = h->encoder_y.layers[nl - 1];
    EpiStore<float> epi{logits_y, (int64_t)K, h->params + l.b_off, nullptr, 0, 0, 1.f};
    GM_TRY(lin_fwd<A>(h, ey.hid[nl - 2], hid_ld(nl - 2), B, view(h, l), epi, st));
  }
  GM_CHECK_CUDA(launch_k(head_y_fwd_kernel<A>, dim3((B + 7) / 8), dim3(256), 0, st, true, (const float*)logits_y, (const float*)nullptr, B, K,
                         1.f, inv_bg, pi, y_act, Kp, acc));
  GM_LAUNCHED(h, st, PC_HEADS);
  GM_CHECK_CUDA(launch_k(prior_table_kernel, dim3((K * 2 * Z + 255) / 256), dim3(256), 0, st, true, (const float*)(h->params + prior.w_off),
                         (const float*)(h->params + prior.b_off), K, 2 * Z, tab));
  GM_LAUNCHED(h, st, PC_HEADS);
  {
    EpiStore<float> epi{xproj, (int64_t)H0, nullptr, nullptr, 0, 0, 1.f};
    GM_TRY(lin_fwd<A>(h, x_act, Dp, B, view(h, enc_l0, 0, D), epi, st));
  }
  const float* Wy = h->params + enc_l0.w_off + (int64_t)D * H0;

  for (int b0 = 0; b0 < B; b0 += h->chunk_samples) {
    const int nb = std::min(h->chunk_samples, B - b0), R = nb * K, row0 = b0 * K;
    {
      const int64_t work = (int64_t)R * (H0 / 4);
      GM_REQUIRE(H0 % 4 == 0, "objective=marginal needs hidden sizes that are multiples of 4");
      const int blocks = (int)std::min<int64_t>((work + 255) / 256, 16 * tc::num_sms());
      GM_CHECK_CUDA(launch_k(expand_h1_kernel<A>, dim3(blocks), dim3(256), 0, st, true, (const float*)(xproj + (int64_t)b0 * H0), (int64_t)H0, Wy,
                             (const float*)(h->params + enc_l0.b_off), R, K, H0, enc.hid[0], (int64_t)H0p));
      GM_LAUNCHED(h, st, PC_HEADS);
    }
    GM_TRY(mlp_hidden_fwd<A>(h, h->encoder, enc, x_act, Dp, D, R, 1, st));
    {
      EpiStore<float> epi{enc_out, (int64_t)2 * Z, h->params + enc_last.b_off, nullptr, 0, 0, 1.f};
      GM_TRY(lin_fwd<A>(h, enc.hid[nl - 2], hid_ld(nl - 2), R, view(h, enc_last), epi, st));
    }
    GM_CHECK_CUDA(launch_k(head_z_m_fwd_kernel<A>, dim3(std::max(1, std::min(4 * tc::num_sms(), (R + 7) / 8))), dim3(256), 0, st, true,
                           (const float*)enc_out, eps, (const float*)tab, (const float*)pi, row0, R, K, Z, c.raw_sigma_bias, c.sigma_min,
                           inv_bg, z_act, Zp, klrow, acc));
    GM_LAUNCHED(h, st, PC_HEADS);
    GM_TRY(mlp_hidden_fwd<A>(h, h->decoder, dec, z_act, Zp, Z, R, 0, st));
    bool dec_bias_fused = false;
    {
      const Linear& l = h->decoder.layers[nl - 1];
      LinView Ld = view(h, l);
      dec_bias_fused = !(h->debug_flags & DBG_NO_FUSED_COLSUM) && tc_ok_fwd<A>(h, dec.hid[nl - 2], hid_ld(nl - 2), Ld);
      EpiBCE<A> epi{dlogits_x, (int64_t)Dp, h->params + l.b_off, c.gen_bias_init, x_u8 + (int64_t)b0 * D, (int64_t)D, K, pi + row0, rec + row0,
                    acc, inv_bg, 0.f, dec_bias_fused ? h->grads + l.b_off : nullptr, h->bf16_mode() ? 1 : 0};
      GM_TRY(lin_fwd<A>(h, dec.hid[nl - 2], hid_ld(nl - 2), R, Ld, epi, st));
    }
    GM_TRY((mlp_backward<A, A>(h, h->decoder, dec, z_act, Zp, Z, dlogits_x, Dp, R, st, dec_bias_fused)));
    {
      const Linear& l0 = h->decoder.layers[0];
      EpiStore<float> epi{dz, (int64_t)Z, nullptr, nullptr, 0, 0, 1.f};
      GM_TRY((lin_dgrad<A>(h, dec.dhid[0], hid_ld(0), R, view(h, l0), epi, st)));
    }
    {
      const int lanes = 256 / Z;
      const int blocks = std::max(1, std::min(2 * tc::num_sms(), (R + lanes - 1) / lanes));
      const size_t smem = (size_t)(2 * 256 + K * 2 * Z) * sizeof(float);
      GM_REQUIRE(smem <= 200 * 1024, "objective=marginal: mixture_components * latent_size too large for the prior-table gradient tile");
      static size_t smem_set_by_dev[64] = {};
      size_t& smem_set = smem_set_by_dev[tc::current_device()];
      if (smem > smem_set) {
        GM_CHECK_CUDA(cudaFuncSetAttribute(head_z_m_bwd_kernel<A>, cudaFuncAttributeMaxDynamicSharedMemorySize, (int)smem));
        smem_set = smem;
      }
      GM_CHECK_CUDA(launch_k(head_z_m_bwd_kernel<A>, dim3(blocks), dim3(256), smem, st, true, (const float*)enc_out, eps, (const float*)tab,
                             (const float*)pi, (const float*)dz, row0, R, K, Z, c.raw_sigma_bias, c.sigma_min, inv_bg, d_enc_out, Z2p,
                             h->grads + enc_last.b_off, dtab));
      GM_LAUNCHED(h, st, PC_HEADS);
    }
    GM_TRY((mlp_backward<A, A>(h, h->encoder, enc, x_act, Dp, D, d_enc_out, Z2p, R, st, true, 1)));
    {
      const int col_blocks = (H0 + 63) / 64;
      int spb = std::max(4, (nb * col_blocks + 2 * tc::num_sms() - 1) / (2 * tc::num_sms()));
      dim3 grid(col_blocks, (nb + spb - 1) / spb);
      static bool attr_by_dev[64] = {};
      bool& attr = attr_by_dev[tc::current_device()];
      if (!attr) {
        GM_CHECK_CUDA(cudaFuncSetAttribute(reduce_k_kernel<A>, cudaFuncAttributeMaxDynamicSharedMemorySize, 4 * HEAD_MAXK * 64 * (int)sizeof(float)));
        attr = true;
      }
      GM_CHECK_CUDA(launch_k(reduce_k_kernel<A>, grid, dim3(256), (size_t)4 * K * 64 * sizeof(float), st, true, (const A*)enc.dhid[0], (int64_t)H0p,
                             b0, nb, K, H0, dxproj, (int64_t)H0p, h->grads + enc_l0.w_off + (int64_t)D * H0, h->grads + enc_l0.b_off, spb));
      GM_LAUNCHED(h, st, PC_BIAS_GRAD);
    }
  }
  GM_TRY(comm_bucket(h, st, h->bucket_end[0]));
  GM_TRY((lin_wgrad<A, A>(h, x_act, Dp, dxproj, H0p, B, view(h, enc_l0, 0, D), st)));
  GM_CHECK_CUDA(launch_k(prior_table_bwd_kernel, dim3((2 * Z + 127) / 128), dim3(128), 0, st, true, (const float*)dtab, K, 2 * Z,
                         h->grads + prior.w_off, h->grads + prior.b_off));
  GM_LAUNCHED(h, st, PC_HEADS);
  GM_TRY(comm_bucket(h, st, h->bucket_end[1]));
  const bool ey_bias_fused = !(h->debug_flags & DBG_NO_FUSED_COLSUM);
  GM_CHECK_CUDA(launch_k(head_y_m_bwd_kernel<A>, dim3(std::max(1, std::min(2 * tc::num_sms(), (B + 7) / 8))), dim3(256), 0, st, true,
                         (const float*)logits_y, (const float*)pi, (const double*)rec, (const float*)klrow, B, K, inv_bg, dlogits_y, Kp,
                         ey_bias_fused ? h->grads + h->encoder_y.layers[nl - 1].b_off : (float*)nullptr));
  GM_LAUNCHED(h, st, PC_HEADS);
  GM_TRY((mlp_backward<A, A>(h, h->encoder_y, ey, x_act, Dp, D, dlogits_y, Kp, B, st, ey_bias_fused)));
  return 0;
}

static int refresh_shadows(gmvae_handle* h, cudaStream_t st) {
  if (h->shadow_tiles > 0) {
    GM_CHECK_CUDA(launch_k(refresh_shadows_kernel, dim3(h->shadow_tiles), dim3(32, 8), 0, st, true, (const ShadowEntry*)h->shadow_dev,
                           (int)h->shadow_host.size())); GM_LAUNCHED(h, st, PC_ADAM);
  }
  return 0;
}

struct DeviceGuard {
  int prev = -1, want = -1;
  explicit DeviceGuard(const gmvae_handle* h) {
    if (!h) return;
    want = h->cfg.device;
    if (cudaGetDevice(&prev) != cudaSuccess) prev = -1;
    if (prev != want) cudaSetDevice(want);
  }
  ~DeviceGuard() { if (prev >= 0 && prev != want) cudaSetDevice(prev); }
};

static int check_ready(const gmvae_handle* h) {
  GM_REQUIRE(h != nullptr, "null handle");
  GM_REQUIRE(h->params != nullptr, "gmvae_bind has not been called");
  return 0;
}

}

extern "C" {

const char* gmvae_last_error(void) { return g_last_error.c_str(); }
const char* gmvae_build_info(void) { return "gmvae_b200 sm_100a (tcgen05/TMA bf16 + fp32 SIMT validation) abi=1 " __DATE__ " " __TIME__; }

int gmvae_create(const gmvae_config* cfg, gmvae_handle** out) {
  GM_REQUIRE(cfg && out, "null argument");
  GM_REQUIRE(cfg->abi_version == GMVAE_ABI_VERSION, "ABI version mismatch");
  GM_REQUIRE(cfg->model >= 0 && cfg->model <= 2, "unknown model");
  GM_REQUIRE(cfg->precision == GMVAE_PRECISION_FP32 || cfg->precision == GMVAE_PRECISION_BF16, "unknown precision");
  GM_REQUIRE(cfg->num_hidden >= 0 && cfg->num_hidden <= GMVAE_MAX_HIDDEN_LAYERS, "num_hidden out of range");
  GM_REQUIRE(cfg->data_size > 0 && cfg->latent_size > 0 && cfg->max_batch > 0, "sizes must be positive");
  for (int i = 0; i < cfg->num_hidden; ++i) GM_REQUIRE(cfg->hidden_sizes[i] > 0, "hidden sizes must be positive");
  if (cfg->model != GMVAE_MODEL_VAE)
    GM_REQUIRE(cfg->mixture_components >= 1 && cfg->mixture_components <= HEAD_MAXK, "mixture_components must be in [1,128]");
  GM_REQUIRE(cfg->objective == GMVAE_OBJECTIVE_REFERENCE || cfg->model == GMVAE_MODEL_GMVAE, "objective applies to GMVAE only");
  if (cfg->objective == GMVAE_OBJECTIVE_MARGINAL)
    GM_REQUIRE(cfg->num_hidden >= 1 && cfg->latent_size <= 256, "objective=marginal needs at least one hidden layer and latent_size <= 256");
  GM_REQUIRE(cfg->deterministic == 0 || cfg->deterministic == 1, "deterministic must be 0 or 1");
  if (cfg->deterministic) {
    GM_REQUIRE(cfg->objective == GMVAE_OBJECTIVE_REFERENCE, "deterministic mode supports objective=reference only");
    for (const char* v : {"GMVAE_DEBUG_FLAGS", "GMVAE_CHAIN_SPLIT", "GMVAE_CHAIN_QUAD"}) {
      const char* e = getenv(v);
      GM_REQUIRE(!e || atoi(e) == 0, std::string("deterministic mode cannot be combined with ") + v);
    }
  }
  int ndev = 0;
  cudaError_t e = cudaGetDeviceCount(&ndev);
  if (e != cudaSuccess || ndev == 0) {
    set_error("no CUDA device: libgmvae_b200 has no CPU fallback");
    return -4;
  }
  GM_REQUIRE(cfg->device >= 0 && cfg->device < ndev, "device ordinal out of range");
  cudaDeviceProp prop;
  GM_CHECK_CUDA(cudaGetDeviceProperties(&prop, cfg->device));
  GM_REQUIRE(prop.major == 10, "libgmvae_b200 is built for sm_100a (B200) only");
  gmvae_handle* h = new gmvae_handle();
  h->cfg = *cfg;
  DeviceGuard dev_guard(h);
  const char* dbg = getenv("GMVAE_DEBUG_FLAGS");
  h->debug_flags = dbg ? atoi(dbg) : 0;
  h->det = cfg->deterministic == 1;
  g_use_pdl = !(h->debug_flags & DBG_NO_PDL);
  if (const char* q = getenv("GMVAE_CHAIN_QUAD")) h->quad_opt_in = atoi(q) != 0;
  if (const char* q = getenv("GMVAE_CHAIN_SPLIT")) h->chain_split_opt = atoi(q);
  if (const char* bnv = getenv("GMVAE_CHAIN_BN")) { const int v = atoi(bnv); if (v == 128 || v == 192) h->wide_bn = v; }
  plan(h);
  GM_CHECK_CUDA(cudaMalloc(&h->state, sizeof(DeviceState)));
  DeviceState s0; s0.step = 0; s0.seed = 0x243F6A8885A308D3ull; s0.adam_blocks = 0; s0.pad = 0; s0.beta1_power = 1.0; s0.beta2_power = 1.0;
  h->seed_host = s0.seed;
  GM_CHECK_CUDA(cudaMemcpy(h->state, &s0, sizeof(s0), cudaMemcpyHostToDevice));
  *out = h;
  return 0;
}

void gmvae_destroy(gmvae_handle* h) {
  if (!h) return;
  if (h->graph_exec) cudaGraphExecDestroy(h->graph_exec);
  for (void* m : h->peer_mapped) if (m) cudaIpcCloseMemHandle(m);
  if (h->peer_region) cudaFree(h->peer_region);
  if (h->comm) ncclCommDestroy(h->comm);
  if (h->comm_stream) cudaStreamDestroy(h->comm_stream);
  for (auto& e : h->comm_ev) if (e) cudaEventDestroy(e);
  if (h->shadow_dev) cudaFree(h->shadow_dev);
  if (h->state) cudaFree(h->state);
  delete h;
}

int64_t gmvae_param_count(const gmvae_handle* h) { return h ? h->n_params : -1; }
int64_t gmvae_grad_count(const gmvae_handle* h) { return h ? h->n_params + ACC_SLOTS : -1; }
int gmvae_num_params(const gmvae_handle* h) { return h ? (int)h->table.size() : -1; }
int gmvae_param_table(const gmvae_handle* h, gmvae_param_desc* out, int cap) {
  GM_REQUIRE(h && out, "null argument");
  int n = std::min(cap, (int)h->table.size());
  for (int i = 0; i < n; ++i) out[i] = h->table[i];
  return n;
}
size_t gmvae_workspace_bytes(const gmvae_handle* h) { return h ? h->ws_needed : 0; }
int64_t gmvae_launch_count(const gmvae_handle* h) { return h ? h->launches : -1; }

int gmvae_bind(gmvae_handle* h, float* params, float* grads, float* adam_m, float* adam_v, void* workspace, size_t workspace_bytes) {
  DeviceGuard dev_guard(h);
  GM_REQUIRE(h && params && grads && adam_m && adam_v && workspace, "null argument");
  GM_REQUIRE(workspace_bytes >= h->ws_needed, "workspace too small");
  GM_REQUIRE(aligned16(params) && aligned16(grads) && aligned16(adam_m) && aligned16(adam_v), "buffers must be 16-byte aligned");
  GM_REQUIRE((reinterpret_cast<uintptr_t>(workspace) & 255) == 0, "workspace must be 256-byte aligned");
  GM_REQUIRE(!h->peer_ready, "gmvae_bind after gmvae_peer_attach is not supported");
  h->params = params; h->grads = grads; h->grads_bound = grads; h->adam_m = adam_m; h->adam_v = adam_v;
  h->ws = reinterpret_cast<uint8_t*>(workspace); h->ws_bytes = workspace_bytes;
  h->shadow_host.clear(); h->shadow_tiles = 0;
  if (h->bf16_mode()) {
    Mlp* mlps[4] = {&h->decoder, &h->encoder, &h->encoder_y, &h->prior_gmm};
    for (Mlp* m : mlps)
      for (auto& l : m->layers) {
        l.w_bf16 = h->buf<bf16>("shadow.w." + std::to_string(l.w_off));
        ShadowEntry e;
        e.w = params + l.w_off; e.w_bf16 = l.w_bf16;
        e.off = l.w_off; e.rows = l.in; e.cols = l.out; e.ld_w = l.ld_w;
        e.tiles_x = (l.ld_w + 31) / 32;
        int tiles_y = (l.in + 31) / 32;
        e.tile_begin = h->shadow_tiles;
        h->shadow_tiles += e.tiles_x * tiles_y;
        h->shadow_host.push_back(e);
      }
    std::sort(h->shadow_host.begin(), h->shadow_host.end(), [](const ShadowEntry& a, const ShadowEntry& b) { return a.off < b.off; });
    h->shadow_tiles = 0;
    for (auto& e : h->shadow_host) { e.tile_begin = h->shadow_tiles; h->shadow_tiles += e.tiles_x * ((e.rows + 31) / 32); }
    if (h->shadow_dev) cudaFree(h->shadow_dev);
    GM_CHECK_CUDA(cudaMalloc(&h->shadow_dev, sizeof(ShadowEntry) * h->shadow_host.size()));
    GM_CHECK_CUDA(cudaMemcpy(h->shadow_dev, h->shadow_host.data(), sizeof(ShadowEntry) * h->shadow_host.size(), cudaMemcpyHostToDevice));
  }
  return 0;
}

int gmvae_params_updated(gmvae_handle* h, void* stream) {
  DeviceGuard dev_guard(h);
  GM_TRY(check_ready(h));
  return refresh_shadows(h, (cudaStream_t)stream);
}

int gmvae_forward_backward(gmvae_handle* h, const uint8_t* x_u8, int batch, int global_batch, const float* eps,
                           const float* gumbel_u, void* stream) {
  DeviceGuard dev_guard(h);
  GM_TRY(check_ready(h));
  GM_REQUIRE(x_u8 != nullptr, "null input");
  GM_REQUIRE(batch > 0 && batch <= h->cfg.max_batch, "batch must be in [1, max_batch]");
  GM_REQUIRE(global_batch >= batch, "global_batch must be >= batch");
  GM_REQUIRE(aligned16(x_u8), "x must be 16-byte aligned");
  if (h->cfg.objective == GMVAE_OBJECTIVE_MARGINAL) {
    if (h->bf16_mode()) return forward_backward_marginal<bf16>(h, x_u8, batch, global_batch, eps, (cudaStream_t)stream);
    return forward_backward_marginal<float>(h, x_u8, batch, global_batch, eps, (cudaStream_t)stream);
  }
  if (h->bf16_mode()) return forward_backward_impl<bf16>(h, x_u8, batch, global_batch, eps, gumbel_u, (cudaStream_t)stream);
  return forward_backward_impl<float>(h, x_u8, batch, global_batch, eps, gumbel_u, (cudaStream_t)stream);
}

int gmvae_finalize_loss(gmvae_handle* h, float* loss_terms, void* stream) {
  DeviceGuard dev_guard(h);
  GM_TRY(check_ready(h));
  GM_REQUIRE(loss_terms != nullptr, "null loss_terms");
  GM_CHECK_CUDA(launch_k(finalize_loss_kernel, dim3(1), dim3(32), 0, (cudaStream_t)stream, false, (const float*)(h->grads + h->n_params), loss_terms)); GM_LAUNCHED(h, (cudaStream_t)stream, PC_MISC);
  return 0;
}

static int adam_step_impl(gmvae_handle* h, float* loss_terms, cudaStream_t st, bool zero_grads, bool fused_exchange = false) {
  const gmvae_config& c = h->cfg;
  int64_t n = h->n_params;
  const bool pdl = !(h->comm && h->world > 1 && (h->debug_flags & DBG_COMM_OVERLAP));
  const int64_t per_block = (int64_t)ADAM_THREADS * 4 * ADAM_VEC;
  AdamPeer ap = {nullptr, nullptr, nullptr, 0, 0};
  float* g_src = h->grads;
  if (fused_exchange) {
    const peer::Layout& L = h->peer_layout;
    char* base = static_cast<char*>(h->peer_region);
    g_src = reinterpret_cast<float*>(base + L.red_off);
    ap.flags = reinterpret_cast<const unsigned long long*>(base + L.flags_off) + peer::MAX_WORLD;
    ap.epoch = &reinterpret_cast<peer::Local*>(base + L.local_off)->epoch;
    ap.own_grads = h->grads; ap.world = L.world; ap.timeout_cycles = h->peer_timeout_cycles;
    zero_grads = true;
  }
  GM_CHECK_CUDA(launch_k(adam_kernel, dim3((unsigned)((n + per_block - 1) / per_block)), dim3(ADAM_THREADS), 0, st, pdl && !fused_exchange, h->params, g_src,
                         h->adam_m, h->adam_v, n, c.learning_rate, c.beta1, c.beta2, c.epsilon, h->state,
                         g_src + h->n_params, loss_terms, (const ShadowEntry*)h->shadow_dev,
                         h->bf16_mode() ? (int)h->shadow_host.size() : 0, zero_grads ? 1 : 0, ap));
  GM_LAUNCHED(h, st, PC_ADAM);
  h->grads_clean = zero_grads;
  return 0;
}

int gmvae_adam_step(gmvae_handle* h, void* stream) {
  DeviceGuard dev_guard(h);
  GM_TRY(check_ready(h));
  return adam_step_impl(h, nullptr, (cudaStream_t)stream, false);
}

int gmvae_get_step(gmvae_handle* h, int64_t* step, void* stream) {
  DeviceGuard dev_guard(h);
  GM_REQUIRE(h && step, "null argument");
  DeviceState s;
  GM_CHECK_CUDA(cudaMemcpyAsync(&s, h->state, sizeof(s), cudaMemcpyDeviceToHost, (cudaStream_t)stream));
  GM_CHECK_CUDA(cudaStreamSynchronize((cudaStream_t)stream));
  *step = s.step;
  return 0;
}
int gmvae_set_step(gmvae_handle* h, int64_t step, void* stream) {
  DeviceGuard dev_guard(h);
  GM_REQUIRE(h, "null argument");
  long long v = step;
  const double pw[2] = {pow((double)h->cfg.beta1, (double)step), pow((double)h->cfg.beta2, (double)step)};
  GM_CHECK_CUDA(cudaMemcpyAsync(&h->state->step, &v, sizeof(v), cudaMemcpyHostToDevice, (cudaStream_t)stream));
  GM_CHECK_CUDA(cudaMemcpyAsync(&h->state->beta1_power, pw, sizeof(pw), cudaMemcpyHostToDevice, (cudaStream_t)stream));
  GM_CHECK_CUDA(cudaStreamSynchronize((cudaStream_t)stream));
  return 0;
}
int gmvae_set_seed(gmvae_handle* h, uint64_t seed) {
  DeviceGuard dev_guard(h);
  GM_REQUIRE(h, "null argument");
  unsigned long long v = seed;
  GM_CHECK_CUDA(cudaMemcpy(&h->state->seed, &v, sizeof(v), cudaMemcpyHostToDevice));
  h->seed_host = seed;
  return 0;
}

int gmvae_nccl_unique_id(char out[128]) {
  GM_REQUIRE(out, "null argument");
  static_assert(sizeof(ncclUniqueId) == 128, "ncclUniqueId size");
  ncclUniqueId id;
  ncclResult_t r = ncclGetUniqueId(&id);
  if (r != ncclSuccess) { set_error(std::string("ncclGetUniqueId: ") + ncclGetErrorString(r)); return -5; }
  memcpy(out, &id, 128);
  return 0;
}
int gmvae_nccl_init(gmvae_handle* h, const char id[128], int world_size, int rank) {
  GM_REQUIRE(h && id, "null argument");
  GM_REQUIRE(world_size >= 1 && rank >= 0 && rank < world_size, "bad world_size / rank");
  ncclUniqueId uid; memcpy(&uid, id, 128);
  GM_CHECK_CUDA(cudaSetDevice(h->cfg.device));
  if (world_size > 1 && (h->debug_flags & DBG_COMM_OVERLAP)) {
    const char* env = getenv("GMVAE_COMM_SMS");
    int reserve = env ? atoi(env) : 8;
    tc::g_reserved_sms = std::max(0, std::min(64, reserve));
    if (tc::g_reserved_sms > 0) {
      std::string v = std::to_string(tc::g_reserved_sms);
      setenv("NCCL_MAX_NCHANNELS", v.c_str(), 0);
      setenv("NCCL_MAX_CTAS", v.c_str(), 0);
    }
  }
  ncclResult_t r = ncclCommInitRank(&h->comm, world_size, uid, rank);
  if (r != ncclSuccess) { set_error(std::string("ncclCommInitRank: ") + ncclGetErrorString(r)); return -5; }
  h->world = world_size; h->rank = rank;
  GM_CHECK_CUDA(cudaStreamCreateWithFlags(&h->comm_stream, cudaStreamNonBlocking));
  for (auto& e : h->comm_ev) GM_CHECK_CUDA(cudaEventCreateWithFlags(&e, cudaEventDisableTiming));
  return 0;
}
int gmvae_peer_export(gmvae_handle* h, int world_size, int rank, char out[64]) {
  DeviceGuard dev_guard(h);
  GM_REQUIRE(h && out, "null argument");
  GM_TRY(check_ready(h));
  GM_REQUIRE(world_size >= 2 && world_size <= peer::MAX_WORLD && rank >= 0 && rank < world_size, "bad world_size / rank");
  GM_REQUIRE(!h->peer_region, "peer region already exported");
  static_assert(sizeof(cudaIpcMemHandle_t) == 64, "cudaIpcMemHandle_t size");
  const int64_t total = h->n_params + ACC_SLOTS;
  GM_REQUIRE(total % 4 == 0, "gradient buffer length must be a multiple of 4 floats");
  h->peer_layout = peer::make_layout(world_size, total);
  GM_CHECK_CUDA(cudaMalloc(&h->peer_region, h->peer_layout.bytes));
  GM_CHECK_CUDA(cudaMemset(h->peer_region, 0, h->peer_layout.bytes));
  GM_CHECK_CUDA(cudaDeviceSynchronize());
  cudaIpcMemHandle_t ipc;
  GM_CHECK_CUDA(cudaIpcGetMemHandle(&ipc, h->peer_region));
  memcpy(out, &ipc, 64);
  if (h->world == 1) { h->world = world_size; h->rank = rank; }
  GM_REQUIRE(h->world == world_size && h->rank == rank, "world_size / rank differ from the NCCL communicator's");
  return 0;
}
int gmvae_peer_attach(gmvae_handle* h, const char* handles) {
  DeviceGuard dev_guard(h);
  GM_REQUIRE(h && handles, "null argument");
  GM_REQUIRE(h->peer_region && !h->peer_ready, "call gmvae_peer_export first (once)");
  const peer::Layout& L = h->peer_layout;
  for (int r = 0; r < L.world; ++r) {
    void* base = h->peer_region;
    if (r != h->rank) {
      cudaIpcMemHandle_t ipc;
      memcpy(&ipc, handles + 64 * r, 64);
      GM_CHECK_CUDA(cudaIpcOpenMemHandle(&base, ipc, cudaIpcMemLazyEnablePeerAccess));
      h->peer_mapped[r] = base;
    }
    char* b = static_cast<char*>(base);
    h->peer_ptrs.grad[r] = reinterpret_cast<float4*>(b + L.grad_off);
    h->peer_ptrs.red[r] = reinterpret_cast<float4*>(b + L.red_off);
    h->peer_ptrs.flags[r] = reinterpret_cast<unsigned long long*>(b + L.flags_off);
  }
  const char* ts = getenv("GMVAE_PEER_TIMEOUT_S");
  const double secs = ts ? std::max(1.0, atof(ts)) : 120.0;
  int khz = 0;
  cudaDeviceGetAttribute(&khz, cudaDevAttrClockRate, h->cfg.device);
  h->peer_timeout_cycles = (long long)(secs * 1e3 * (double)std::max(khz, 1000000));
  h->grads_bound = h->grads;
  h->grads = reinterpret_cast<float*>(static_cast<char*>(h->peer_region) + L.grad_off);
  h->grads_clean = true;
  if (h->graph_exec) { cudaGraphExecDestroy(h->graph_exec); h->graph_exec = nullptr; }
  h->peer_ready = true;
  return 0;
}
float* gmvae_peer_grads(gmvae_handle* h) { return h ? h->grads : nullptr; }

static int peer_exchange(gmvae_handle* h, cudaStream_t st) {
  const peer::Layout& L = h->peer_layout;
  peer::Local* loc = reinterpret_cast<peer::Local*>(static_cast<char*>(h->peer_region) + L.local_off);
  const int per_block = peer::exchange_block_items(L.world);
  const unsigned blocks = (unsigned)std::max<int64_t>(1, std::min<int64_t>((L.cap4 + per_block - 1) / per_block, 8 * tc::num_sms()));
  auto kern = L.world == 2 ? peer::exchange_kernel<2> : L.world == 4 ? peer::exchange_kernel<4> : L.world == 8 ? peer::exchange_kernel<8>
            : L.world == 16 ? peer::exchange_kernel<16> : peer::exchange_kernel<0>;
  GM_CHECK_CUDA(launch_k(kern, dim3(blocks), dim3(peer::THREADS), 0, st, false, L, h->rank, h->peer_ptrs, loc, h->peer_timeout_cycles));
  GM_LAUNCHED(h, st, PC_COMM);
  return 0;
}

int gmvae_allreduce_grads(gmvae_handle* h, void* stream) {
  DeviceGuard dev_guard(h);
  GM_TRY(check_ready(h));
  if (h->peer_ready && h->world > 1) {
    GM_TRY(peer_exchange(h, (cudaStream_t)stream));
    const peer::Layout& L = h->peer_layout;
    peer::Local* loc = reinterpret_cast<peer::Local*>(static_cast<char*>(h->peer_region) + L.local_off);
    const unsigned blocks = (unsigned)std::max<int64_t>(1, std::min<int64_t>((L.n4 + peer::THREADS - 1) / peer::THREADS, 4 * tc::num_sms()));
    GM_CHECK_CUDA(launch_k(peer::gather_kernel, dim3(blocks), dim3(peer::THREADS), 0, (cudaStream_t)stream, false, L, h->rank, h->peer_ptrs, loc,
                           h->peer_timeout_cycles));
    GM_LAUNCHED(h, (cudaStream_t)stream, PC_COMM);
    return 0;
  }
  if (!h->comm || h->world == 1) return 0;
  cudaStream_t st = (cudaStream_t)stream;
  const int64_t total = h->n_params + ACC_SLOTS;
  if (h->overlap_comm) {
    GM_TRY(comm_bucket(h, st, total));
    cudaEvent_t ev = h->comm_ev[h->comm_ev_next++ % 8];
    GM_CHECK_CUDA(cudaEventRecord(ev, h->comm_stream));
    GM_CHECK_CUDA(cudaStreamWaitEvent(st, ev, 0));
    return 0;
  }
  ncclResult_t r = ncclAllReduce(h->grads, h->grads, (size_t)total, ncclFloat, ncclSum, h->comm, st);
  if (r != ncclSuccess) { set_error(std::string("ncclAllReduce: ") + ncclGetErrorString(r)); return -5; }
  GM_LAUNCHED(h, st, PC_COMM);
  return 0;
}

int gmvae_train_step(gmvae_handle* h, const uint8_t* x_u8, int batch, int global_batch, const float* eps, const float* gumbel_u,
                     float* loss_terms, void* stream) {
  DeviceGuard dev_guard(h);
  GM_REQUIRE(h != nullptr, "null handle");
  h->overlap_comm = h->comm != nullptr && h->world > 1 && (h->debug_flags & DBG_COMM_OVERLAP);
  h->in_train_step = true;
  int r = gmvae_forward_backward(h, x_u8, batch, global_batch, eps, gumbel_u, stream);
  h->in_train_step = false;
  const bool fused = h->peer_ready && h->world > 1;
  if (r == 0) r = fused ? peer_exchange(h, (cudaStream_t)stream) : gmvae_allreduce_grads(h, stream);
  h->overlap_comm = false;
  GM_TRY(r);
  return adam_step_impl(h, loss_terms, (cudaStream_t)stream, true, fused);
}

int gmvae_step_graph_capture(gmvae_handle* h, const uint8_t* x_u8, int batch, int global_batch, const float* eps,
                             const float* gumbel_u, float* loss_terms, void* stream) {
  DeviceGuard dev_guard(h);
  GM_TRY(check_ready(h));
  cudaStream_t st = (cudaStream_t)stream;
  GM_REQUIRE(st != nullptr, "graph capture needs a non-default stream");
  if (h->graph_exec) { cudaGraphExecDestroy(h->graph_exec); h->graph_exec = nullptr; }
// ... 394 lines not shown
```

### gmvae_b200/csrc/gemm_chain.cuh

```cuda
#pragma once
#include "gemm_tc.cuh"
#include "chain_sched.cuh"

namespace gmvae {
namespace tc {

enum EpiKind : int { EK_NONE = -1, EK_STORE_BF16 = 0, EK_STORE_F32 = 1, EK_BCE = 2, EK_RELUMASK = 3, EK_ATOMIC = 4,
                     EK_ROWS_FIRST = 16, EK_ROWS_Y_FWD = 16, EK_ROWS_Z_FWD = 17, EK_ROWS_Z_BWD = 18, EK_ROWS_Y_BWD = 19 };

struct RowsYFwd { const float* logits; const float* u; int K; float inv_T, inv_bg; float* y_f32; bf16* y_act; int ld_yact; float* acc; };
struct RowsZFwd { const float* enc_out; const float* eps; const float* prior_out; int prior_mode, Z; float c, sigma_min, inv_bg;
                  bf16* z_act; int ld_z; float* acc; };
struct RowsZBwd { const float* enc_out; const float* eps; const float* prior_out; const float* dz_dec; int prior_mode, Z; float c, sigma_min, inv_bg;
                  bf16* d_enc_out; bf16* d_prior_out; int ld_out; float* db_enc; float* db_prior; };
struct RowsYBwd { const float* logits; const float* y_f32; const float* dy; int K; float inv_T, inv_bg; bf16* dlogits; int ld_out; float* db; };
template <class Epi> struct epi_kind { static constexpr int value = EK_NONE; };
template <> struct epi_kind<EpiStore<bf16, EPI_PLAIN>> { static constexpr int value = EK_STORE_BF16; };
template <> struct epi_kind<EpiStore<float, EPI_PLAIN>> { static constexpr int value = EK_STORE_F32; };
template <> struct epi_kind<EpiBCE<bf16>> { static constexpr int value = EK_BCE; };
template <> struct epi_kind<EpiReluMask<bf16, bf16>> { static constexpr int value = EK_RELUMASK; };
template <> struct epi_kind<EpiAtomicAdd> { static constexpr int value = EK_ATOMIC; };

constexpr bool CHAIN_RELU_BITS = true;
static_assert(SCHED_BLOCK_M == BLOCK_M, "chain_sched.cuh and gemm_tc.cuh agree on the tile height");
constexpr int CHAIN_MAX_JOBS = 40;
constexpr int CHAIN_MAX_MAPS = 112;
constexpr int CHAIN_STAGES = 4;
constexpr int CHAIN_STAGE_BYTES = A_STAGE_BYTES + 256 * BLOCK_K * 2;
#ifndef GMVAE_PAIR_STAGES
#define GMVAE_PAIR_STAGES 6
#endif
constexpr int CHAIN_STAGES_PAIR = GMVAE_PAIR_STAGES;
constexpr int CHAIN_STAGE_BYTES_PAIR = A_STAGE_BYTES + 128 * BLOCK_K * 2;
static_assert(CHAIN_STAGES_PAIR * CHAIN_STAGE_BYTES_PAIR <= CHAIN_STAGES * CHAIN_STAGE_BYTES, "both modes use the same ring area");
constexpr int CHAIN_PATCH_BYTES = 2048;
constexpr int CHAIN_CARVE_BYTES = CHAIN_STAGES * CHAIN_STAGE_BYTES + EPI_WARPS * CHAIN_PATCH_BYTES + 256  + 256 * 4  + 256 * 4 ;
constexpr int CHAIN_SMEM_BYTES = 232448;
static_assert(CHAIN_CARVE_BYTES + 512 <= CHAIN_SMEM_BYTES, "shared-memory budget");

template <int MAXJ, int MAXM>
struct ChainParamsT {
  int njobs, nmaps;
  int* counters;
  long long* trace;
  int trace_cta;
  int abl;
  unsigned long long* jobstat;
  alignas(64) CUtensorMap maps[MAXM];
  ChainJob jobs[MAXJ];
};
constexpr int CHAIN_SMALL_JOBS = 10, CHAIN_SMALL_MAPS = 44;
typedef ChainParamsT<CHAIN_MAX_JOBS, CHAIN_MAX_MAPS> ChainParams;
typedef ChainParamsT<CHAIN_SMALL_JOBS, CHAIN_SMALL_MAPS> ChainParamsSmall;
static_assert(sizeof(ChainParams) <= 32000, "kernel parameter space");

#ifndef GMVAE_POLL_NS
#define GMVAE_POLL_NS 40
#endif
__device__ __forceinline__ int ld_acquire_gpu(const int* p) {
  int v;
  asm volatile("ld.acquire.gpu.global.s32 %0, [%1];" : "=r"(v) : "l"(p) : "memory");
  return v;
}
__device__ __forceinline__ void fence_proxy_async_global() { asm volatile("fence.proxy.async.global;" ::: "memory"); }
__device__ __forceinline__ unsigned long long gtimer() {
  unsigned long long t;
  asm volatile("mov.u64 %0, %globaltimer;" : "=l"(t));
  return t;
}
__device__ __forceinline__ void release_counter(int* ctr, int legacy) {
  if (!legacy) {
    asm volatile("red.release.gpu.global.add.s32 [%0], %1;" ::"l"(ctr), "r"(1) : "memory");
  } else {
    __threadfence();
    atomicAdd(ctr, 1);
  }
}
__device__ __forceinline__ void wait_counter(const int* p, int target) {
  if (ld_acquire_gpu(p) >= target) return;
  const long long t0 = clock64();
  while (ld_acquire_gpu(p) < target) {
    __nanosleep(GMVAE_POLL_NS);
    if (clock64() - t0 > 4000000000LL) __trap();
  }
}

__device__ __forceinline__ uint64_t make_smem_desc_rt(uint32_t smem_addr, int mn_major) {
  const uint64_t lbo = mn_major ? (uint64_t)(BLOCK_K * 128) : 0;
  const uint64_t sbo = 1024;
  return (uint64_t)((smem_addr & 0x3FFFF) >> 4) | ((lbo >> 4) << 16) | ((sbo >> 4) << 32) | (1ull << 46) | (2ull << 61);
}

struct ChainShared {
  uint8_t* smem; uint64_t* full_bar; uint64_t* empty_bar; uint64_t* tmem_full_bar; uint64_t* tmem_empty_bar;
  uint8_t* patches; float* sbias_all; float* scs_all; uint32_t tmem_base; uint64_t* op_bar;
};

__device__ __forceinline__ void tma_store_2d(const CUtensorMap* m, uint32_t src, int c0, int c1) {
  asm volatile("cp.async.bulk.tensor.2d.global.shared::cta.bulk_group [%0, {%2, %3}], [%1];"
               ::"l"(reinterpret_cast<uint64_t>(m)), "r"(src), "r"(c0), "r"(c1) : "memory");
}
__device__ __forceinline__ void tma_reduce_add_2d(const CUtensorMap* m, uint32_t src, int c0, int c1) {
  asm volatile("cp.reduce.async.bulk.tensor.2d.global.shared::cta.add.tile.bulk_group [%0, {%2, %3}], [%1];"
               ::"l"(reinterpret_cast<uint64_t>(m)), "r"(src), "r"(c0), "r"(c1) : "memory");
}
__device__ __forceinline__ void tma_store_3d(const CUtensorMap* m, uint32_t src, int c0, int c1, int c2) {
  asm volatile("cp.async.bulk.tensor.3d.global.shared::cta.bulk_group [%0, {%2, %3, %4}], [%1];"
               ::"l"(reinterpret_cast<uint64_t>(m)), "r"(src), "r"(c0), "r"(c1), "r"(c2) : "memory");
}
__device__ __forceinline__ void bulk_commit() { asm volatile("cp.async.bulk.commit_group;" ::: "memory"); }
__device__ __forceinline__ void bulk_wait_read0() { asm volatile("cp.async.bulk.wait_group.read 0;" ::: "memory"); }
__device__ __forceinline__ void bulk_wait0() { asm volatile("cp.async.bulk.wait_group 0;" ::: "memory"); }

template <int RB> __device__ __forceinline__ uint32_t patch_unit(uint32_t patch, int r, int u) {
  return RB == 128 ? patch + r * 128 + ((u ^ (r & 7)) << 4) : patch + r * 64 + ((u ^ ((r >> 1) & 3)) << 4);
}

template <int RB>
__device__ __forceinline__ void patch_colsum_bf16(uint32_t patch, float* scs, int ncols, int lane) {
  constexpr int WORDS = RB / 4;
  constexpr int GROUPS = 32 / WORDS;
  const int w = lane % WORDS, grp = lane / WORDS;
  float s0 = 0.f, s1 = 0.f;
#pragma unroll 8
  for (int i = 0; i < 32 / GROUPS; ++i) {
    const int r = grp * (32 / GROUPS) + i;
    const uint32_t t = lds32(patch_unit<RB>(patch, r, w >> 2) + 4 * (w & 3));
    const float2 f = __bfloat1622float2(*reinterpret_cast<const __nv_bfloat162*>(&t));
    s0 += f.x; s1 += f.y;
  }
  if (GROUPS == 2) { s0 += __shfl_xor_sync(0xffffffffu, s0, 16); s1 += __shfl_xor_sync(0xffffffffu, s1, 16); }
  if (grp == 0) {
    const uint32_t a = smem_addr(scs) + 8 * w;
    if (2 * w < ncols && s0 != 0.f) asm volatile("red.shared.add.f32 [%0], %1;" ::"r"(a), "f"(s0) : "memory");
    if (2 * w + 1 < ncols && s1 != 0.f) asm volatile("red.shared.add.f32 [%0], %1;" ::"r"(a + 4), "f"(s1) : "memory");
  }
}

__device__ __forceinline__ void pack16(const float* v, uint4& lo, uint4& hi) {
  lo.x = pack_bf16x2(v[0], v[1]); lo.y = pack_bf16x2(v[2], v[3]); lo.z = pack_bf16x2(v[4], v[5]); lo.w = pack_bf16x2(v[6], v[7]);
  hi.x = pack_bf16x2(v[8], v[9]); hi.y = pack_bf16x2(v[10], v[11]); hi.z = pack_bf16x2(v[12], v[13]); hi.w = pack_bf16x2(v[14], v[15]);
}

__device__ __forceinline__ float exp2f_approx(float x) { float y; asm("ex2.approx.ftz.f32 %0, %1;" : "=f"(y) : "f"(x)); return y; }
__device__ __forceinline__ float lg2_approx(float x) { float y; asm("lg2.approx.ftz.f32 %0, %1;" : "=f"(y) : "f"(x)); return y; }
__device__ __forceinline__ float rcp_approx(float x) { float y; asm("rcp.approx.ftz.f32 %0, %1;" : "=f"(y) : "f"(x)); return y; }
__device__ __forceinline__ float fast_softplus(float t) { return fmaxf(t, 0.f) + __logf(1.f + __expf(-fabsf(t))); }
__device__ __forceinline__ float fast_sigmoid(float t) {
  const float e = __expf(-fabsf(t));
  const float s = __fdividef(1.f, 1.f + e);
  return t >= 0.f ? s : e * s;
}
__device__ __forceinline__ void ld_row16(const float* p, int K, float* v, float fill) {
  if ((K & 1) == 0) {
#pragma unroll
    for (int k = 0; k < 16; k += 2) {
      if (k < K) { const float2 t = __ldcg(reinterpret_cast<const float2*>(p + k)); v[k] = t.x; v[k + 1] = t.y; }
      else { v[k] = fill; v[k + 1] = fill; }
    }
  } else {
#pragma unroll
    for (int k = 0; k < 16; ++k) v[k] = k < K ? __ldcg(p + k) : fill;
  }
}
__device__ __forceinline__ void st_row16(float* p, int K, const float* v) {
  if ((K & 1) == 0) {
#pragma unroll
    for (int k = 0; k < 16; k += 2)
      if (k < K) *reinterpret_cast<float2*>(p + k) = make_float2(v[k], v[k + 1]);
  } else {
#pragma unroll
    for (int k = 0; k < 16; ++k)
      if (k < K) p[k] = v[k];
  }
}
__device__ __noinline__ float y_head_fwd_row(const float* lg, const RowsYFwd& prm, int64_t row, bool valid, const float* noise = nullptr) {
  if (!valid) return 0.f;
  const int K = prm.K;
  float a[16];
  if (noise) {
#pragma unroll
    for (int k = 0; k < 16; ++k) a[k] = noise[k];
  } else {
    ld_row16(prm.u + row * K, K, a, 0.f);
  }
  float ml = -INFINITY, ma = -INFINITY;
#pragma unroll
  for (int k = 0; k < 16; ++k) {
    if (k < K) {
      a[k] = (lg[k] + a[k]) * prm.inv_T;
      ml = fmaxf(ml, lg[k]);
    } else {
      a[k] = -INFINITY;
    }
    ma = fmaxf(ma, a[k]);
  }
  float sl = 0.f, sa = 0.f;
  float pl[16];
#pragma unroll
  for (int k = 0; k < 16; ++k) {
    pl[k] = 0.f;
    if (k < K) { a[k] = __expf(a[k] - ma); pl[k] = __expf(lg[k] - ml); sl += pl[k]; sa += a[k]; }
  }
  const float lse = ml + __logf(sl), inv_sa = __fdividef(1.f, sa), inv_sl = __fdividef(1.f, sl);
  float y[16];
  float ent = 0.f;
#pragma unroll
  for (int k = 0; k < 16; ++k) {
    y[k] = 0.f;
    if (k < K) {
      ent = fmaf(pl[k] * inv_sl, lg[k] - lse, ent);
      y[k] = a[k] * inv_sa;
    }
  }
  st_row16(prm.y_f32 + row * K, K, y);
  uint4* dst = reinterpret_cast<uint4*>(prm.y_act + row * prm.ld_yact);
  dst[0] = make_uint4(pack_bf16x2(y[0], y[1]), pack_bf16x2(y[2], y[3]), pack_bf16x2(y[4], y[5]), pack_bf16x2(y[6], y[7]));
  if (prm.ld_yact > 8) dst[1] = make_uint4(pack_bf16x2(y[8], y[9]), pack_bf16x2(y[10], y[11]), pack_bf16x2(y[12], y[13]), pack_bf16x2(y[14], y[15]));
  return ent;
}
__device__ __noinline__ void y_head_bwd_row(const float* g, const RowsYBwd& prm, int64_t row, bool valid, float* scs) {
  const int K = prm.K;
  float lg[16], o[16];
#pragma unroll
  for (int k = 0; k < 16; ++k) o[k] = 0.f;
  if (valid) {
    float y[16];
    ld_row16(prm.logits + row * K, K, lg, -INFINITY);
    ld_row16(prm.y_f32 + row * K, K, y, 0.f);
    float ml = -INFINITY, ydy = 0.f;
#pragma unroll
    for (int k = 0; k < 16; ++k)
      if (k < K) { ml = fmaxf(ml, lg[k]); ydy = fmaf(y[k], g[k], ydy); }
    float sl = 0.f;
    float pl[16];
#pragma unroll
    for (int k = 0; k < 16; ++k) {
      pl[k] = 0.f;
      if (k < K) { pl[k] = __expf(lg[k] - ml); sl += pl[k]; }
    }
    const float lse = ml + __logf(sl), inv_sl = __fdividef(1.f, sl);
    float plogp = 0.f;
#pragma unroll
    for (int k = 0; k < 16; ++k)
      if (k < K) { lg[k] -= lse; pl[k] *= inv_sl; plogp = fmaf(pl[k], lg[k], plogp); }
#pragma unroll
    for (int k = 0; k < 16; ++k)
      if (k < K) o[k] = __bfloat162float(__float2bfloat16_rn(y[k] * (g[k] - ydy) * prm.inv_T + pl[k] * (lg[k] - plogp) * prm.inv_bg));
    uint4* dst = reinterpret_cast<uint4*>(prm.dlogits + row * prm.ld_out);
    dst[0] = make_uint4(pack_bf16x2(o[0], o[1]), pack_bf16x2(o[2], o[3]), pack_bf16x2(o[4], o[5]), pack_bf16x2(o[6], o[7]));
    if (prm.ld_out > 8) dst[1] = make_uint4(pack_bf16x2(o[8], o[9]), pack_bf16x2(o[10], o[11]), pack_bf16x2(o[12], o[13]), pack_bf16x2(o[14], o[15]));
  }
  const int lane = (int)threadIdx.x & 31;
#pragma unroll
  for (int w = 8, bit = 16; w >= 1; w >>= 1, bit >>= 1) {
    const bool up = (lane & bit) != 0;
#pragma unroll
    for (int i = 0; i < w; ++i) {
      const float send = up ? o[i] : o[i + w];
      const float keep = up ? o[i + w] : o[i];
      o[i] = keep + __shfl_xor_sync(0xffffffffu, send, bit);
    }
  }
  const float t = o[0] + __shfl_xor_sync(0xffffffffu, o[0], 1);
  const int col = lane >> 1;
  if ((lane & 1) == 0 && col < K && t != 0.f) atomicAdd(scs + col, t);
}

template <class Epi, int KIND, int CL>
__device__ __forceinline__ void chain_epilogue_job(const ChainJob& J, const CUtensorMap* maps, int* counters, const ChainShared& S, int& it,
                                                   uint32_t& op_phase, int warp, int lane, long long* trace, int jidx,
                                                   unsigned long long* jobstat = nullptr, int abl = 0) {
  constexpr int CW = 16;
  constexpr bool PAIR = CL >= 2;
  Epi epi = *reinterpret_cast<const Epi*>(J.epi);
  const int G = (int)gridDim.x / CL;
  const int cidx = (int)blockIdx.x / CL;
  const int rank = (int)blockIdx.x % CL;
  int first, wstride;
  if (!chain_walk<1>(J, cidx, G, first, wstride) || first >= J.walk_total) return;
  const int M = J.M, N = J.N, BN = J.block_n;
  const int nchunk = BN / CW;
  const int e = warp - 2, quad = warp & 3, slot = e >> 2;
  const int et = (int)threadIdx.x - 64;
  float* const cs_dst = epi.colsum_dst();
  const float* const bias = epi.bias_ptr();
  float* const scs_all = S.scs_all;
  const uint32_t patch = smem_addr(S.patches + e * CHAIN_PATCH_BYTES);
  uint64_t* const op_bar = S.op_bar + e;
  const int gw = J.gw;
  int cs_n0 = -1;
  int staged_n0 = -1;
  float fuse_acc = 0.f;
  bool fuse_bwd = false;
  if constexpr (KIND == EK_STORE_F32) fuse_bwd = J.fuse == EK_ROWS_Y_BWD;
  if (cs_dst || fuse_bwd) { for (int i = et; i < 256; i += EPI_WARPS * 32) scs_all[i] = 0.f; }
  auto cs_flush = [&]() {
    for (int i = et; i < BN; i += EPI_WARPS * 32) {
      const float v = scs_all[i];
      if (v != 0.f && cs_n0 + i < N) atomicAdd(cs_dst + cs_n0 + i, v);
      scs_all[i] = 0.f;
    }
  };
  for (int l = first; l < J.walk_total; l += wstride, ++it) {
    int z, mb, n0;
    chain_tile<CL>(J, l, rank, z, mb, n0);
    const int m0 = mb * BLOCK_M;
    const int as = it & 1; const uint32_t ap = (it >> 1) & 1;
    const int mrow0 = m0 + quad * 32;
    const int m = mrow0 + lane;
    float* sbias = S.sbias_all;
    if (n0 != staged_n0) {
      asm volatile("bar.sync 1, %0;" ::"n"(EPI_WARPS * 32) : "memory");
      const uint32_t sb = smem_addr(sbias);
      float shift = 0.f;
      if constexpr (KIND == EK_BCE) shift = epi.gen_bias;
      for (int i = et; i < BN; i += EPI_WARPS * 32) sts32f(sb + 4 * i, ((bias && n0 + i < N) ? __ldg(bias + n0 + i) : 0.f) + shift);
      asm volatile("bar.sync 1, %0;" ::"n"(EPI_WARPS * 32) : "memory");
      staged_n0 = n0;
    }
    if (cs_dst && cs_n0 != n0) {
      if (cs_n0 >= 0) {
        cs_flush();
        asm volatile("bar.sync 1, %0;" ::"n"(EPI_WARPS * 32) : "memory");
      }
      cs_n0 = n0;
    }
    const bool mvalid = m < M;
#ifdef GMVAE_CHAIN_ABL
    if (abl & 1) {
      mbar_wait(&S.tmem_full_bar[it & 1], (it >> 1) & 1);
      tc_fence_after(); tc_fence_before();
      __syncwarp();
      if (lane == 0) {
        if (PAIR) mbar_arrive_leader(&S.tmem_empty_bar[it & 1]); else mbar_arrive(&S.tmem_empty_bar[it & 1]);
        if (J.sig_base >= 0) { __threadfence(); atomicAdd(counters + J.sig_base + mb, 1); }
      }
      continue;
    }
#endif
    const bool tr = trace && e == 0 && lane == 0 && it < 64;
    if (tr) { trace[16 * it + 6] = clock64(); trace[16 * it + 15] = jidx; trace[16 * it + 14] = l; }
    const bool js = jobstat && e == 0 && lane == 0;
    unsigned long long js_t0 = 0, js_t1 = 0;
    if (J.epi_dep >= 0 && m0 < M) {
      if (lane == 0) { wait_counter(counters + J.deps[J.epi_dep].base + mb, J.deps[J.epi_dep].target); fence_proxy_async_global(); }
      __syncwarp();
    }
    const uint32_t taddr = S.tmem_base + ((uint32_t)(quad * 32) << 16) + (uint32_t)(as * 256);
    bool acc_ready = false;
    auto wait_acc = [&]() {
      if (!acc_ready) {
        if (tr) trace[16 * it + 7] = clock64();
        if (js) js_t0 = gtimer();
        mbar_wait(&S.tmem_full_bar[as], ap);
        tc_fence_after();
        if (tr) trace[16 * it + 8] = clock64();
        if (js) js_t1 = gtimer();
        acc_ready = true;
      }
    };

    if (KIND == EK_STORE_F32 || gw == 0) {
     if constexpr (KIND == EK_STORE_F32 || KIND == EK_ATOMIC) {
      EpiCtx ctx{nullptr, max(0, min(32, M - mrow0)), sbias, scs_all};
      float noise[CW];
      bool have_noise = false;
      if constexpr (KIND == EK_STORE_F32) {
        if (J.fuse == EK_ROWS_Y_FWD && slot == 0 && mvalid) {
          const RowsYFwd& yp = *reinterpret_cast<const RowsYFwd*>(J.epi2);
          ld_row16(yp.u + (int64_t)m * yp.K, yp.K, noise, 0.f);
          have_noise = true;
        }
      }
      wait_acc();
#pragma unroll 1
      for (int ci = slot; ci < nchunk && n0 + ci * CW < N; ci += 4) {
        const int n = n0 + ci * CW;
        uint32_t r[CW];
        tmem_ld16_issue(taddr + ci * CW, r);
        tmem_ld16_wait(r);
        float v[CW];
#pragma unroll
        for (int i = 0; i < CW; ++i) v[i] = __uint_as_float(r[i]);
        ctx.sbias = sbias + ci * CW;
        if constexpr (KIND == EK_STORE_F32) {
          if (J.fuse != 0) {
            float lg[CW];
#pragma unroll
            for (int i = 0; i < CW; ++i) lg[i] = fmaf(v[i], epi.scale, sbias[i]);
            if (J.fuse == EK_ROWS_Y_FWD) {
              if (mvalid) {
                if (epi.ld == N) st_row16(epi.out + (int64_t)m * epi.ld, N, lg);
                else {
#pragma unroll
                  for (int i = 0; i < CW; ++i)
                    if (i < N) epi.out[(int64_t)m * epi.ld + i] = lg[i];
                }
              }
              fuse_acc += y_head_fwd_row(lg, *reinterpret_cast<const RowsYFwd*>(J.epi2), (int64_t)m, mvalid, have_noise ? noise : nullptr);
            } else {
              y_head_bwd_row(lg, *reinterpret_cast<const RowsYBwd*>(J.epi2), (int64_t)m, mvalid, scs_all);
            }
            continue;
          }
        }
        typename Epi::template Pre<CW> pre;
        epi.template row<CW>(m, n, v, min(CW, N - n), mvalid, pre, ctx);
      }
     }
    } else if constexpr (KIND != EK_STORE_F32) {
      const int ngroups = (nchunk + gw - 1) / gw;
#pragma unroll 1
      for (int g = slot; g < ngroups && n0 + g * gw * CW < N; g += 4) {
        const int gcol = g * gw * CW;
        if (lane == 0) bulk_wait_read0();
        uint32_t hbits = 0;
        bool use_bits = false;
        if constexpr (KIND == EK_RELUMASK) {
          use_bits = CHAIN_RELU_BITS && epi.relu_bits != nullptr;
          if (!use_bits) fence_proxy_async();
        }
        __syncwarp();
        if constexpr (KIND == EK_RELUMASK) {
          if (use_bits) {
            if (mvalid) hbits = __ldcg(epi.relu_bits + (int64_t)((n0 + gcol) >> 5) * epi.ld_bits + m);
          } else if (lane == 0) {
            mbar_expect_tx(op_bar, (uint32_t)CHAIN_PATCH_BYTES);
            tma_load_2d(&maps[J.c], op_bar, S.patches + e * CHAIN_PATCH_BYTES, n0 + gcol, mrow0);
          }
        }
        uint32_t obits = 0; int obits_chunks = 0;
        uint4 xq[2];
        if constexpr (KIND == EK_BCE) {
#pragma unroll
          for (int c = 0; c < 2; ++c) {
            const int n = n0 + gcol + c * CW;
            xq[c] = make_uint4(0, 0, 0, 0);
            if (c < gw && mvalid && n < N) {
              const uint8_t* px = epi.x + (int64_t)m * epi.ldx + n;
              if (n + CW <= N && (reinterpret_cast<uintptr_t>(px) & 15) == 0) {
                xq[c] = *reinterpret_cast<const uint4*>(px);
              } else {
                uint8_t* b = reinterpret_cast<uint8_t*>(&xq[c]);
                for (int i = 0; i < CW && n + i < N; ++i) b[i] = px[i];
              }
            }
          }
        }
        wait_acc();
        if constexpr (KIND == EK_RELUMASK) {
          if (!use_bits) {
            mbar_wait(op_bar, op_phase);
            op_phase ^= 1;
          }
        }
#pragma unroll
        for (int c = 0; c < 2; ++c) {
          const int ci = g * gw + c;
          if (c < gw && ci < nchunk && n0 + ci * CW < N) {
            uint32_t r[CW];
            tmem_ld16_issue(taddr + ci * CW, r);
            float bb[CW];
            if constexpr (KIND == EK_STORE_BF16 || KIND == EK_BCE) {
              const uint32_t sb = smem_addr(sbias + ci * CW);
#pragma unroll
              for (int i = 0; i < CW; i += 4) { float4 t = lds128f(sb + 4 * i); bb[i] = t.x; bb[i + 1] = t.y; bb[i + 2] = t.z; bb[i + 3] = t.w; }
            }
            uint4 h0, h1;
            if constexpr (KIND == EK_RELUMASK) {
              if (!use_bits) { h0 = lds128(patch_unit<64>(patch, lane, 2 * c)); h1 = lds128(patch_unit<64>(patch, lane, 2 * c + 1)); }
            }
            tmem_ld16_wait(r);
            float v[CW];
#pragma unroll
            for (int i = 0; i < CW; ++i) v[i] = __uint_as_float(r[i]);
            if constexpr (KIND == EK_ATOMIC) {
#pragma unroll
              for (int u = 0; u < 4; ++u)
                sts128(patch_unit<64>(patch, lane, u),
                       make_uint4(__float_as_uint(v[4 * u]), __float_as_uint(v[4 * u + 1]), __float_as_uint(v[4 * u + 2]), __float_as_uint(v[4 * u + 3])));
            } else {
              if constexpr (KIND == EK_STORE_BF16) {
#pragma unroll
                for (int i = 0; i < CW; ++i) {
                  v[i] = fmaf(v[i], epi.scale, bb[i]);
                  if (epi.relu == 1) v[i] = fmaxf(v[i], 0.f);
                  else if (epi.relu == 2) v[i] = sigmoid_f(v[i] + epi.shift);
                }
                if (CHAIN_RELU_BITS && epi.relu_bits) {
#pragma unroll
                  for (int i = 0; i < CW; ++i) obits = __funnelshift_l(__float_as_uint(v[i]) - 1u, obits, 1);
                  ++obits_chunks;
                }
              } else if constexpr (KIND == EK_RELUMASK) {
               if (use_bits) {
#pragma unroll
                for (int i = 0; i < CW; ++i) v[i] = ((hbits >> (31 - (c * CW + i))) & 1u) ? v[i] : 0.f;
               } else {
                const __nv_bfloat162* ph0 = reinterpret_cast<const __nv_bfloat162*>(&h0);
                const __nv_bfloat162* ph1 = reinterpret_cast<const __nv_bfloat162*>(&h1);
#pragma unroll
                for (int k = 0; k < 4; ++k) {
                  const float2 a = __bfloat1622float2(ph0[k]), b = __bfloat1622float2(ph1[k]);
                  v[2 * k] = a.x > 0.f ? v[2 * k] : 0.f; v[2 * k + 1] = a.y > 0.f ? v[2 * k + 1] : 0.f;
                  v[8 + 2 * k] = b.x > 0.f ? v[8 + 2 * k] : 0.f; v[8 + 2 * k + 1] = b.y > 0.f ? v[8 + 2 * k + 1] : 0.f;
                }
               }
              } else if constexpr (KIND == EK_BCE) {
                const int nvalid = min(CW, N - (n0 + ci * CW));
                float ll = 0.f;
                if (nvalid == CW && m0 + BLOCK_M <= M) {
                  const uint32_t* xw = reinterpret_cast<const uint32_t*>(&xq[c]);
#pragma unroll
                  for (int i = 0; i < CW; ++i) {
                    const uint32_t sgn = (xw[i >> 2] << (31 - 8 * (i & 3))) & 0x80000000u;
                    const float t = __uint_as_float(__float_as_uint(v[i] + bb[i]) ^ sgn);
                    const float e = exp2f_approx(fabsf(t) * -1.4426950408889634f);
                    const float d = 1.f + e;
                    const float r = rcp_approx(d);
                    ll -= fmaxf(t, 0.f);
                    ll = fmaf(lg2_approx(d), -0.6931471805599453f, ll);
                    const float sg = r * (t >= 0.f ? 1.f : e);
                    v[i] = __uint_as_float(__float_as_uint(sg * epi.inv_bg) ^ sgn);
                  }
                } else {
                  const uint8_t* xb = reinterpret_cast<const uint8_t*>(&xq[c]);
#pragma unroll
                  for (int i = 0; i < CW; ++i) {
                    const float lg = v[i] + bb[i];
                    const float xv = __uint_as_float(0x4B000000u | (uint32_t)xb[i]) - 8388608.f;
                    const float ex = __expf(-fabsf(lg));
                    const float sp = fmaxf(lg, 0.f) + __logf(1.f + ex);
                    const float inv1pe = __fdividef(1.f, 1.f + ex);
                    const float sg = lg >= 0.f ? inv1pe : ex * inv1pe;
                    const bool ok = mvalid && i < nvalid;
                    ll += ok ? fmaf(xv, lg, -sp) : 0.f;
                    v[i] = ok ? (sg - xv) * epi.inv_bg : 0.f;
                  }
                }
                epi.partial += ll;
              }
              uint4 lo, hi;
              pack16(v, lo, hi);
              sts128(patch_unit<64>(patch, lane, 2 * c), lo); sts128(patch_unit<64>(patch, lane, 2 * c + 1), hi);
            }
          }
        }
        if constexpr (KIND == EK_STORE_BF16) {
          if (CHAIN_RELU_BITS && epi.relu_bits && mvalid) {
            if (obits_chunks < 2) obits = (obits << 16) | 0xFFFFu;
            epi.relu_bits[(int64_t)((n0 + gcol) >> 5) * epi.ld_bits + m] = ~obits;
          }
        }
        fence_proxy_async();
        __syncwarp();
        if (lane == 0) {
          if constexpr (KIND == EK_ATOMIC) {
            if (J.zslice) tma_store_3d(&maps[J.d], patch, n0 + gcol, mrow0, z);
            else tma_reduce_add_2d(&maps[J.d], patch, n0 + gcol, mrow0);
          } else {
            tma_store_2d(&maps[J.d], patch, n0 + gcol, mrow0);
          }
          bulk_commit();
        }
        if constexpr (KIND == EK_RELUMASK || KIND == EK_BCE) {
          if (cs_dst) {
            const int ncols = min(gw * CW, N - (n0 + gcol));
            patch_colsum_bf16<64>(patch, scs_all + gcol, ncols, lane);
          }
        }
      }
    }
    tc_fence_before();
    if (tr) trace[16 * it + 9] = clock64();
    if constexpr (KIND == EK_STORE_F32) {
      if (J.fuse != 0) fence_proxy_async_global();
    }
    __syncwarp();
    if (lane == 0) {
      if (PAIR) mbar_arrive_leader(&S.tmem_empty_bar[as]);
      else mbar_arrive(&S.tmem_empty_bar[as]);
      if (J.sig_base >= 0) {
        if constexpr (KIND != EK_STORE_F32) { bulk_wait0(); fence_proxy_async_global(); }
        release_counter(counters + J.sig_base + mb, abl & 8);
      }
    }
    if (tr) trace[16 * it + 10] = clock64();
    if (js) {
      const unsigned long long t2 = gtimer();
      atomicMax(jobstat + 8 * jidx + 1, t2);
      atomicAdd(jobstat + 8 * jidx + 4, t2 - js_t1);
      atomicAdd(jobstat + 8 * jidx + 5, js_t1 - js_t0);
      atomicAdd(jobstat + 8 * jidx + 6, 1ull);
    }
  }
  epi.finish_warp();
  if constexpr (KIND == EK_STORE_F32) {
    if (J.fuse == EK_ROWS_Y_FWD) {
      const RowsYFwd& yp = *reinterpret_cast<const RowsYFwd*>(J.epi2);
      const float sacc = warp_sum(fuse_acc);
      if (lane == 0 && sacc != 0.f) acc_add(yp.acc, ACC_NENT, sacc * yp.inv_bg);
    } else if (J.fuse == EK_ROWS_Y_BWD) {
      const RowsYBwd& yp = *reinterpret_cast<const RowsYBwd*>(J.epi2);
      asm volatile("bar.sync 1, %0;" ::"n"(EPI_WARPS * 32) : "memory");
      if (et < yp.K && yp.db && scs_all[et] != 0.f) atomicAdd(yp.db + et, scs_all[et]);
      asm volatile("bar.sync 1, %0;" ::"n"(EPI_WARPS * 32) : "memory");
    }
  }
  if (cs_dst && cs_n0 >= 0) {
    asm volatile("bar.sync 1, %0;" ::"n"(EPI_WARPS * 32) : "memory");
    cs_flush();
    asm volatile("bar.sync 1, %0;" ::"n"(EPI_WARPS * 32) : "memory");
  }
}

__device__ __forceinline__ float4 ldcg4(const float* p) { return __ldcg(reinterpret_cast<const float4*>(p)); }

template <int KIND, class P, int CL>
__device__ __forceinline__ void chain_rows_job(const ChainJob& J, int* counters, const ChainShared& S, int warp, int lane,
                                               unsigned long long* jobstat = nullptr, int jidx = 0, int abl = 0) {
  const P prm = *reinterpret_cast<const P*>(J.epi);
  int first, wstride;
  if (!chain_walk<CL>(J, (int)blockIdx.x, (int)gridDim.x, first, wstride) || first >= J.total_tiles) return;
  const int M = J.M;
  const int et = (int)threadIdx.x - 64;
  constexpr int NT = EPI_WARPS * 32;
  float red_acc = 0.f;
  float cs[16];
#pragma unroll
  for (int i = 0; i < 16; ++i) cs[i] = 0.f;
  if constexpr (KIND == EK_ROWS_Y_BWD) {
    asm volatile("bar.sync 1, %0;" ::"n"(EPI_WARPS * 32) : "memory");
    for (int i = et; i < 256; i += NT) S.scs_all[i] = 0.f;
    asm volatile("bar.sync 1, %0;" ::"n"(EPI_WARPS * 32) : "memory");
  }
  const int sub = J.tiles_n, rpt = BLOCK_M / sub;
  for (int l = first; l < J.total_tiles; l += wstride) {
    const int mb = l / sub, m0 = l * rpt;
    const int rows = max(0, min(rpt, M - m0));
    const bool js = jobstat && warp == 2 && lane == 0;
    unsigned long long js_t0 = 0, js_t1 = 0;
    if (js) js_t0 = gtimer();
    if (lane == 0) {
      for (int d = 0; d < J.ndeps; ++d) wait_counter(counters + J.deps[d].base + mb, J.deps[d].target);
    }
    __syncwarp();
    if (js) { js_t1 = gtimer(); atomicMin(jobstat + 8 * jidx + 0, js_t0); atomicAdd(jobstat + 8 * jidx + 2, js_t1 - js_t0); }
    if constexpr (KIND == EK_ROWS_Z_FWD) {
      const int Z = prm.Z, tpr = Z >> 2;
      for (int t = et; t < rows * tpr; t += NT) {
        const int b = m0 + t / tpr, j = (t % tpr) * 4;
        const float4 mu = ldcg4(prm.enc_out + (int64_t)b * 2 * Z + j), raw = ldcg4(prm.enc_out + (int64_t)b * 2 * Z + Z + j);
        const float4 e4 = ldcg4(prm.eps + (int64_t)b * Z + j);
        float4 mp = make_float4(0.f, 0.f, 0.f, 0.f), rp = mp;
        if (prm.prior_mode == 2) { mp = ldcg4(prm.prior_out + (int64_t)b * 2 * Z + j); rp = ldcg4(prm.prior_out + (int64_t)b * 2 * Z + Z + j); }
        const float* MU = &mu.x; const float* RAW = &raw.x; const float* E = &e4.x; const float* MP = &mp.x; const float* RP = &rp.x;
        float z[4];
#pragma unroll
        for (int q = 0; q < 4; ++q) {
          const float sg = fmaxf(fast_softplus(RAW[q] + prm.c), prm.sigma_min);
          z[q] = fmaf(sg, E[q], MU[q]);
          float d = -0.5f * E[q] * E[q];
          if (prm.prior_mode == 0) {
            d = fmaf(0.5f * z[q], z[q], d) - __logf(sg);
          } else if (prm.prior_mode == 2) {
            const float sp = fmaxf(fast_softplus(RP[q] + prm.c), prm.sigma_min);
            const float isp = __fdividef(1.f, sp);
            const float tt = (z[q] - MP[q]) * isp;
            d = fmaf(0.5f * tt, tt, d) - __logf(sg * isp);
          } else {
            d -= __logf(sg);
          }
          red_acc += d;
        }
        *reinterpret_cast<uint2*>(prm.z_act + (int64_t)b * prm.ld_z + j) = make_uint2(pack_bf16x2(z[0], z[1]), pack_bf16x2(z[2], z[3]));
      }
    } else if constexpr (KIND == EK_ROWS_Z_BWD) {
      const int Z = prm.Z, tpr = Z >> 2;
      const int j = (et % tpr) * 4;
      for (int t = et; t < rows * tpr; t += NT) {
        const int b = m0 + t / tpr;
        const float4 mu = ldcg4(prm.enc_out + (int64_t)b * 2 * Z + j), raw = ldcg4(prm.enc_out + (int64_t)b * 2 * Z + Z + j);
        const float4 e4 = ldcg4(prm.eps + (int64_t)b * Z + j), dzd = ldcg4(prm.dz_dec + (int64_t)b * Z + j);
        float4 mp = make_float4(0.f, 0.f, 0.f, 0.f), rp = mp;
        if (prm.prior_mode == 2) { mp = ldcg4(prm.prior_out + (int64_t)b * 2 * Z + j); rp = ldcg4(prm.prior_out + (int64_t)b * 2 * Z + Z + j); }
        const float* MU = &mu.x; const float* RAW = &raw.x; const float* E = &e4.x; const float* DZ = &dzd.x;
        const float* MP = &mp.x; const float* RP = &rp.x;
        float g0[4], g1[4], a0[4], a1[4];
#pragma unroll
        for (int q = 0; q < 4; ++q) {
          const float tq = RAW[q] + prm.c;
          const float eq = __expf(-fabsf(tq)), iq = __fdividef(1.f, 1.f + eq);
          const float spq = fmaxf(tq, 0.f) + __logf(1.f + eq);
          const float sgm_q = tq >= 0.f ? iq : eq * iq;
          const float sg = fmaxf(spq, prm.sigma_min);
          const float z = fmaf(sg, E[q], MU[q]);
          float dz = DZ[q];
          a0[q] = 0.f; a1[q] = 0.f;
          if (prm.prior_mode == 0) {
            dz += z * prm.inv_bg;
          } else {
            const float tp = RP[q] + prm.c;
            const float ep = __expf(-fabsf(tp)), ip = __fdividef(1.f, 1.f + ep);
            const float spp = fmaxf(tp, 0.f) + __logf(1.f + ep);
            const float sgm_p = tp >= 0.f ? ip : ep * ip;
            const float sp = fmaxf(spp, prm.sigma_min);
            const float d = z - MP[q];
            const float isp = __fdividef(1.f, sp);
            const float isp2 = isp * isp;
            dz += d * isp2 * prm.inv_bg;
            const float dsp = (isp - d * d * isp2 * isp) * prm.inv_bg;
            a0[q] = __bfloat162float(__float2bfloat16_rn(-d * isp2 * prm.inv_bg));
            a1[q] = __bfloat162float(__float2bfloat16_rn(spp >= prm.sigma_min ? dsp * sgm_p : 0.f));
          }
          const float dsg = dz * E[q] - prm.inv_bg * __fdividef(1.f, sg);
          g0[q] = __bfloat162float(__float2bfloat16_rn(dz));
          g1[q] = __bfloat162float(__float2bfloat16_rn(spq >= prm.sigma_min ? dsg * sgm_q : 0.f));
          cs[q] += g0[q]; cs[4 + q] += g1[q]; cs[8 + q] += a0[q]; cs[12 + q] += a1[q];
        }
        *reinterpret_cast<uint2*>(prm.d_enc_out + (int64_t)b * prm.ld_out + j) = make_uint2(pack_bf16x2(g0[0], g0[1]), pack_bf16x2(g0[2], g0[3]));
        *reinterpret_cast<uint2*>(prm.d_enc_out + (int64_t)b * prm.ld_out + Z + j) = make_uint2(pack_bf16x2(g1[0], g1[1]), pack_bf16x2(g1[2], g1[3]));
        if (prm.prior_mode == 2) {
          *reinterpret_cast<uint2*>(prm.d_prior_out + (int64_t)b * prm.ld_out + j) = make_uint2(pack_bf16x2(a0[0], a0[1]), pack_bf16x2(a0[2], a0[3]));
          *reinterpret_cast<uint2*>(prm.d_prior_out + (int64_t)b * prm.ld_out + Z + j) = make_uint2(pack_bf16x2(a1[0], a1[1]), pack_bf16x2(a1[2], a1[3]));
        }
      }
    } else if constexpr (KIND == EK_ROWS_Y_FWD) {
      if (et < BLOCK_M) {
        const int64_t row = m0 + et;
        const bool valid = et < rows;
        float lg[16];
#pragma unroll
        for (int k = 0; k < 16; ++k) lg[k] = -INFINITY;
        if (valid) ld_row16(prm.logits + row * prm.K, prm.K, lg, -INFINITY);
        red_acc += y_head_fwd_row(lg, prm, row, valid);
      }
    } else if constexpr (KIND == EK_ROWS_Y_BWD) {
      if (et < BLOCK_M) {
        const int64_t row = m0 + et;
        const bool valid = et < rows;
        float g[16];
#pragma unroll
        for (int k = 0; k < 16; ++k) g[k] = (valid && k < prm.K) ? __ldcg(prm.dy + row * prm.K + k) : 0.f;
        y_head_bwd_row(g, prm, row, valid, S.scs_all);
      }
    }
    fence_proxy_async_global();
    __syncwarp();
    if (lane == 0 && J.sig_base >= 0) release_counter(counters + J.sig_base + mb, abl & 8);
    if (js) {
      const unsigned long long t2 = gtimer();
      atomicMax(jobstat + 8 * jidx + 1, t2); atomicAdd(jobstat + 8 * jidx + 4, t2 - js_t1); atomicAdd(jobstat + 8 * jidx + 6, 1ull);
    }
  }
  if constexpr (KIND == EK_ROWS_Z_FWD || KIND == EK_ROWS_Y_FWD) {
    const float s = warp_sum(red_acc);
    if (lane == 0 && s != 0.f) acc_add(prm.acc, KIND == EK_ROWS_Z_FWD ? ACC_KL : ACC_NENT, s * prm.inv_bg);
  }
  if constexpr (KIND == EK_ROWS_Z_BWD) {
    float* const scs = S.scs_all;
    asm volatile("bar.sync 1, %0;" ::"n"(EPI_WARPS * 32) : "memory");
    for (int i = et; i < 256; i += NT) scs[i] = 0.f;
    asm volatile("bar.sync 1, %0;" ::"n"(EPI_WARPS * 32) : "memory");
    const int Z = prm.Z, j = (et % (Z >> 2)) * 4;
#pragma unroll
    for (int p4 = 0; p4 < 4; ++p4)
#pragma unroll
      for (int q = 0; q < 4; ++q)
        if (cs[4 * p4 + q] != 0.f) atomicAdd(scs + p4 * Z + j + q, cs[4 * p4 + q]);
    asm volatile("bar.sync 1, %0;" ::"n"(EPI_WARPS * 32) : "memory");
    for (int col = et; col < 4 * Z; col += NT) {
      const int p4 = col / Z, jj = col % Z;
      const float t = scs[col];
      if (prm.db_enc && t != 0.f && (p4 < 2 || prm.prior_mode == 2)) atomicAdd((p4 < 2 ? prm.db_enc : prm.db_prior) + (p4 & 1) * Z + jj, t);
    }
    asm volatile("bar.sync 1, %0;" ::"n"(EPI_WARPS * 32) : "memory");
  }
  if constexpr (KIND == EK_ROWS_Y_BWD) {
    asm volatile("bar.sync 1, %0;" ::"n"(EPI_WARPS * 32) : "memory");
    if (et < prm.K && S.scs_all[et] != 0.f && prm.db) atomicAdd(prm.db + et, S.scs_all[et]);
    asm volatile("bar.sync 1, %0;" ::"n"(EPI_WARPS * 32) : "memory");
  }
}

template <class Params, int CL>
__global__ void __launch_bounds__(NUM_THREADS2, 1) gemm_chain_kernel(const __grid_constant__ Params p) {
  constexpr bool PAIR = CL >= 2, QUAD = CL == 4;
  constexpr int STAGES = PAIR ? CHAIN_STAGES_PAIR : CHAIN_STAGES, STAGE_BYTES = PAIR ? CHAIN_STAGE_BYTES_PAIR : CHAIN_STAGE_BYTES;
  extern __shared__ uint8_t smem_raw[];
  uint8_t* smem = reinterpret_cast<uint8_t*>((reinterpret_cast<uintptr_t>(smem_raw) + 1023) & ~(uintptr_t)1023);
  if (smem - smem_raw + CHAIN_CARVE_BYTES > CHAIN_SMEM_BYTES) __trap();
  uint8_t* patches = smem + STAGES * STAGE_BYTES;
  uint64_t* bars = reinterpret_cast<uint64_t*>(patches + EPI_WARPS * CHAIN_PATCH_BYTES);
  uint64_t* full_bar = bars;
  uint64_t* empty_bar = bars + STAGES;
  uint64_t* tmem_full_bar = bars + 2 * STAGES;
  uint64_t* tmem_empty_bar = bars + 2 * STAGES + 2;
  uint64_t* op_bar = bars + 2 * STAGES + 4;
  uint32_t* tmem_slot = reinterpret_cast<uint32_t*>(op_bar + EPI_WARPS);
  float* sbias_all = reinterpret_cast<float*>(reinterpret_cast<uint8_t*>(bars) + 256);
  float* scs_all = sbias_all + 256;

  const int warp = threadIdx.x >> 5, lane = threadIdx.x & 31;
  const int G = (int)gridDim.x / CL, c = (int)blockIdx.x / CL;
  const int crank = (int)blockIdx.x % CL;
  const int rank = crank & 1;
  long long* const trace = (p.trace && (int)blockIdx.x == p.trace_cta) ? p.trace : nullptr;

  if (warp == 0 && lane == 0) {
    for (int i = 0; i < p.nmaps; ++i) tma_prefetch_desc(&p.maps[i]);
    for (int s = 0; s < STAGES; ++s) { mbar_init(&full_bar[s], 1); mbar_init(&empty_bar[s], QUAD ? 2 : 1); }
    for (int s = 0; s < 2; ++s) { mbar_init(&tmem_full_bar[s], 1); mbar_init(&tmem_empty_bar[s], PAIR ? 2 * EPI_WARPS : EPI_WARPS); }
    for (int s = 0; s < EPI_WARPS; ++s) mbar_init(&op_bar[s], 1);
    fence_barrier_init();
  } else if (warp == 1) {
    if (PAIR) tmem_alloc_pair(tmem_slot, 512); else tmem_alloc(tmem_slot, 512);
  }
  tc_fence_before();
  __syncthreads();
  if (PAIR) {
    if (cluster_ctarank() != (uint32_t)crank) __trap();
    cluster_sync_all();
  }
  tc_fence_after();
  const uint32_t tmem_base = *tmem_slot;
  griddep_wait();
  griddep_launch();

  if (warp == 0) {
    int stage = 0; uint32_t phase = 0;
    int pit = 0;
    for (int j = 0; j < p.njobs; ++j) {
      const ChainJob& J = p.jobs[j];
      if (J.kind >= EK_ROWS_FIRST) continue;
      const int BN = J.block_n, kb1 = J.kb1, kb_total = J.kb1 + J.kb2, a_mn = J.a_mn, b_mn = J.b_mn, ndeps = J.ndeps;
      const int JM = J.M, JN = J.N, kps = J.kb_per_split, walk_total = J.walk_total, share = J.share;
      const CUtensorMap* const ta1 = &p.maps[J.a1];
      const CUtensorMap* const tb1 = &p.maps[J.b1];
      const CUtensorMap* const ta2 = &p.maps[J.a2];
      const CUtensorMap* const tb2 = &p.maps[J.b2];
      const int bhalf = BN >> 1;
      const int b_slabs = PAIR ? (bhalf + 63) / 64 : BN / 64;
      const uint32_t b_bytes = PAIR ? (uint32_t)(b_mn ? b_slabs * (BLOCK_K * 128) : bhalf * BLOCK_K * 2) : (uint32_t)(BN * BLOCK_K * 2);
      const uint32_t tx_bytes = (PAIR ? 2u : 1u) * ((uint32_t)A_STAGE_BYTES + b_bytes);
      bool any_seg2 = false;
      for (int d = 0; d < ndeps; ++d) any_seg2 = any_seg2 || J.deps[d].seg2 != 0;
      int first, wstride;
      if (!chain_walk<1>(J, c, G, first, wstride)) continue;
      for (int l = first; l < walk_total; l += wstride, ++pit) {
        int z, mb, n0;
        chain_tile<CL>(J, l, crank, z, mb, n0);
        const int m0 = mb * BLOCK_M;
        const bool real = a_mn || m0 < JM;
        const int n_eff = min(BN, (JN - n0 + 15) & ~15);
        const int nb = PAIR ? n0 + rank * (n_eff >> 1) : n0;
        const int kb_begin = z * kps, kb_end = min(kb_total, kb_begin + kps);
        const bool tr = trace && pit < 64 && lane == 0;
        if (tr) trace[16 * pit + 0] = clock64();
        unsigned long long js_t0 = 0;
        if (p.jobstat) js_t0 = gtimer();
        if (ndeps > 0) {
          for (int d = 0; d < ndeps; ++d) {
            const ChainDep& D = J.deps[d];
            if (D.seg2) continue;
            if (!D.by_k) {
              if (real) wait_counter(p.counters + D.base + mb, D.target);
            } else {
              const int lo = (kb_begin * BLOCK_K) / BLOCK_M, hi = min(D.nblocks - 1, (kb_end * BLOCK_K - 1) / BLOCK_M);
              for (int b0 = lo; b0 <= hi; b0 += 32) {
                if (b0 + lane <= hi) wait_counter(p.counters + D.base + b0 + lane, D.target);
                __syncwarp();
              }
            }
          }
          fence_proxy_async_global();
          __syncwarp();
        }
        if (tr) trace[16 * pit + 1] = clock64();
        if (p.jobstat && lane == 0) { atomicMin(p.jobstat + 8 * j + 0, js_t0); atomicAdd(p.jobstat + 8 * j + 2, gtimer() - js_t0); }
        for (int kb = kb_begin; kb < kb_end; ++kb) {
          if (kb == kb1 && any_seg2) {
            for (int d = 0; d < ndeps; ++d)
              if (J.deps[d].seg2 && real) wait_counter(p.counters + J.deps[d].base + mb, J.deps[d].target);
            fence_proxy_async_global();
          }
          mbar_wait(&empty_bar[stage], phase ^ 1);
          const bool seg2 = kb >= kb1;
          const CUtensorMap* const ta = seg2 ? ta2 : ta1;
          const CUtensorMap* const tb = seg2 ? tb2 : tb1;
          const int k_elem = (seg2 ? kb - kb1 : kb) * BLOCK_K;
          uint8_t* const sa = smem + stage * STAGE_BYTES;
          uint8_t* const sb = sa + A_STAGE_BYTES;
          uint64_t* const fb = &full_bar[stage];
          if (elect_one()) {
#ifdef GMVAE_CHAIN_ABL
            if (p.abl & 2) {
              if (!PAIR || rank == 0) mbar_arrive(fb);
            } else
#endif
            {
              if (!PAIR || rank == 0) mbar_expect_tx(fb, tx_bytes);
              auto ld = [&](const CUtensorMap* m, void* dst, int c0, int c1) {
                if (PAIR) tma_load_2d_pair(m, fb, dst, c0, c1); else tma_load_2d(m, fb, dst, c0, c1);
              };
              if (QUAD) {
                const int hh = crank >> 1;
                if (share) {
                  const uint16_t mask = (uint16_t)((1u << rank) | (1u << (rank + 2)));
                  if (a_mn) tma_load_2d_pair_mc(ta, fb, sa + hh * 8192, m0 + hh * 64, k_elem, mask);
                  else tma_load_2d_pair_mc(ta, fb, sa + hh * 8192, k_elem, m0 + hh * 64, mask);
                } else {
#pragma unroll
                  for (int i = 0; i < 2; ++i) {
                    if (a_mn) ld(ta, sa + i * 8192, m0 + i * 64, k_elem); else ld(ta, sa + i * 8192, k_elem, m0 + i * 64);
                  }
                }
              } else if (a_mn) {
#pragma unroll
                for (int i = 0; i < BLOCK_M / 64; ++i) ld(ta, sa + i * (BLOCK_K * 128), m0 + i * 64, k_elem);
              } else {
                ld(ta, sa, k_elem, m0);
              }
              if (b_mn) {
                for (int i = 0; i < b_slabs; ++i) ld(tb, sb + i * (BLOCK_K * 128), nb + i * 64, k_elem);
              } else {
                ld(tb, sb, k_elem, nb);
              }
            }
          }
          if (++stage == STAGES) { stage = 0; phase ^= 1; }
        }
        if (tr) trace[16 * pit + 2] = clock64();
      }
    }
  } else if (warp == 1) {
    int stage = 0; uint32_t phase = 0;
    int it = 0;
    for (int j = 0; (!PAIR || rank == 0) && j < p.njobs; ++j) {
      const ChainJob& J = p.jobs[j];
      if (J.kind >= EK_ROWS_FIRST) continue;
      const int kb_total = J.kb1 + J.kb2, kps = J.kb_per_split, walk_total = J.walk_total, BN = J.block_n, JN = J.N;
      const int a_mn = J.a_mn, b_mn = J.b_mn;
      const uint32_t idesc0 = (1u << 4) | (1u << 7) | (1u << 10) | ((uint32_t)a_mn << 15) | ((uint32_t)b_mn << 16) |
                              ((uint32_t)((PAIR ? 2 * BLOCK_M : BLOCK_M) >> 4) << 24);
      const uint64_t a_step = a_mn ? (UMMA_K * 128) >> 4 : (UMMA_K * 2) >> 4;
      const uint64_t b_step = b_mn ? (UMMA_K * 128) >> 4 : (UMMA_K * 2) >> 4;
      const uint64_t adesc_hi = make_smem_desc_rt(0, a_mn), bdesc_hi = make_smem_desc_rt(0, b_mn);
      int first, wstride;
      if (!chain_walk<1>(J, c, G, first, wstride)) continue;
      for (int l = first; l < walk_total; l += wstride, ++it) {
        int z, mb_unused, n0;
        chain_tile<CL>(J, l, crank, z, mb_unused, n0);
        const int kb_begin = z * kps, kb_end = min(kb_total, kb_begin + kps);
        const int as = it & 1; const uint32_t ap = (it >> 1) & 1;
        const int n_eff = min(BN, (JN - n0 + 15) & ~15);
        const uint32_t idesc = idesc0 | ((uint32_t)(n_eff >> 3) << 17);
        const bool tr = trace && it < 64 && lane == 0;
        if (tr) trace[16 * it + 3] = clock64();
        unsigned long long js_t0 = 0, js_t1 = 0;
        if (p.jobstat) js_t0 = gtimer();
        mbar_wait(&tmem_empty_bar[as], ap ^ 1);
        tc_fence_after();
        if (p.jobstat) js_t1 = gtimer();
        const uint32_t tmem_d = tmem_base + (uint32_t)(as * 256);
        for (int kb = kb_begin; kb < kb_end; ++kb) {
          mbar_wait(&full_bar[stage], phase);
          tc_fence_after();
          if (tr && kb == kb_begin) trace[16 * it + 4] = clock64();
          const uint32_t sa = smem_u32(smem + stage * STAGE_BYTES);
          const uint64_t adesc = adesc_hi | (uint64_t)((sa & 0x3FFFF) >> 4);
          const uint64_t bdesc = bdesc_hi | (uint64_t)(((sa + A_STAGE_BYTES) & 0x3FFFF) >> 4);
          if (elect_one()) {
#ifdef GMVAE_CHAIN_ABL
            if (!(p.abl & 4))
#endif
#pragma unroll
            for (int k = 0; k < BLOCK_K / UMMA_K; ++k) {
              if (PAIR) umma_bf16_pair(adesc + (uint64_t)k * a_step, bdesc + (uint64_t)k * b_step, tmem_d, idesc, (kb > kb_begin || k > 0) ? 1u : 0u);
              else umma_bf16(adesc + (uint64_t)k * a_step, bdesc + (uint64_t)k * b_step, tmem_d, idesc, (kb > kb_begin || k > 0) ? 1u : 0u);
            }
            if (QUAD) umma_commit_mc(&empty_bar[stage], (uint16_t)0xF);
            else if (PAIR) umma_commit_pair(&empty_bar[stage]); else umma_commit(&empty_bar[stage]);
          }
          if (++stage == STAGES) { stage = 0; phase ^= 1; }
        }
        if (elect_one()) {
          if (QUAD) umma_commit_mc(&tmem_full_bar[as], (uint16_t)(3u << (crank & 2)));
          else if (PAIR) umma_commit_pair(&tmem_full_bar[as]); else umma_commit(&tmem_full_bar[as]);
        }
        if (tr) trace[16 * it + 5] = clock64();
        if (p.jobstat && lane == 0) { atomicAdd(p.jobstat + 8 * j + 3, gtimer() - js_t1); atomicAdd(p.jobstat + 8 * j + 7, js_t1 - js_t0); }
      }
    }
  } else {
    ChainShared S{smem, full_bar, empty_bar, tmem_full_bar, tmem_empty_bar, patches, sbias_all, scs_all, tmem_base, op_bar};
    int it = 0;
    uint32_t op_phase = 0;
    for (int j = 0; j < p.njobs; ++j) {
      const ChainJob& J = p.jobs[j];
      switch (J.kind) {
        case EK_STORE_BF16: chain_epilogue_job<EpiStore<bf16, EPI_PLAIN>, EK_STORE_BF16, CL>(J, p.maps, p.counters, S, it, op_phase, warp, lane, trace, j, p.jobstat, p.abl); break;
        case EK_STORE_F32: chain_epilogue_job<EpiStore<float, EPI_PLAIN>, EK_STORE_F32, CL>(J, p.maps, p.counters, S, it, op_phase, warp, lane, trace, j, p.jobstat, p.abl); break;
        case EK_BCE: chain_epilogue_job<EpiBCE<bf16>, EK_BCE, CL>(J, p.maps, p.counters, S, it, op_phase, warp, lane, trace, j, p.jobstat, p.abl); break;
        case EK_RELUMASK: chain_epilogue_job<EpiReluMask<bf16, bf16>, EK_RELUMASK, CL>(J, p.maps, p.counters, S, it, op_phase, warp, lane, trace, j, p.jobstat, p.abl); break;
        case EK_ATOMIC: chain_epilogue_job<EpiAtomicAdd, EK_ATOMIC, CL>(J, p.maps, p.counters, S, it, op_phase, warp, lane, trace, j, p.jobstat, p.abl); break;
#ifndef GMVAE_NO_ROWS
        case EK_ROWS_Y_FWD: chain_rows_job<EK_ROWS_Y_FWD, RowsYFwd, CL>(J, p.counters, S, warp, lane, p.jobstat, j, p.abl); break;
        case EK_ROWS_Z_FWD: chain_rows_job<EK_ROWS_Z_FWD, RowsZFwd, CL>(J, p.counters, S, warp, lane, p.jobstat, j, p.abl); break;
        case EK_ROWS_Z_BWD: chain_rows_job<EK_ROWS_Z_BWD, RowsZBwd, CL>(J, p.counters, S, warp, lane, p.jobstat, j, p.abl); break;
        case EK_ROWS_Y_BWD: chain_rows_job<EK_ROWS_Y_BWD, RowsYBwd, CL>(J, p.counters, S, warp, lane, p.jobstat, j, p.abl); break;
#endif
        default: break;
      }
    }
  }
  if (warp >= 2 && lane == 0) bulk_wait0();
  tc_fence_before();
  __syncthreads();
  if (PAIR) cluster_sync_all();
  if (warp == 1) {
    tc_fence_after();
    if (PAIR) tmem_dealloc_pair(tmem_base, 512); else tmem_dealloc(tmem_base, 512);
  }
}

}
}
```

Measured before the change: 45.72 million.

## Fuse encoder z head, reparameterization, and first decoder GEMM into one chained job

Adds a compound chained-GEMM job (EK_ZFWD). It computes the encoder's last linear layer into TMEM, and the epilogue warps then apply the bias, softplus sigma, reparameterized z and KL term. The epilogue writes the bf16 z tile straight into the shared-memory ring, where the MMA warp consumes it as the A operand of the first decoder layer GEMM. This removes the separate encoder-head GEMM job, the rows z-forward job, and the global round-trip of z before the decoder's first layer. In exchange it adds a new barrier handshake, extra ring-slot accounting (kq) and a recomputation of the head for every N tile of the decoder layer, and it applies only under CTA-pair plans with certain Z sizes.

```diff
diff --git a/gmvae_b200/csrc/chain_sched.cuh b/gmvae_b200/csrc/chain_sched.cuh
--- a/gmvae_b200/csrc/chain_sched.cuh
+++ b/gmvae_b200/csrc/chain_sched.cuh
@@ -37,6 +37,7 @@
   int fuse;
   int zslice;
   alignas(16) unsigned char epi2[CHAIN_EPI2_BYTES];
+  int zn;
 };
 template <int CL>
 GMVAE_SCHED_FN void chain_tile(const ChainJob& J, int l, int crank, int& z, int& mb, int& n0) {
@@ -89,6 +90,12 @@
   if (r1 < r0) r1 = r0;
 }
 
+GMVAE_SCHED_FN int chain_tile_ring_blocks(const ChainJob& J, int l) {
+  if (J.zn > 0) return J.kb1 + 1;
+  const int z = l / J.tiles_mn, kb_total = J.kb1 + J.kb2, b = z * J.kb_per_split;
+  return (b + J.kb_per_split < kb_total ? b + J.kb_per_split : kb_total) - b;
+}
+
 inline int chain_job_counters(int M, int cl) {
   const int tiles_m = (M + SCHED_BLOCK_M - 1) / SCHED_BLOCK_M;
   return cl >= 2 ? 2 * ((tiles_m + 1) / 2) + (cl == 4 ? 2 : 0) : tiles_m;
diff --git a/gmvae_b200/csrc/engine.cu b/gmvae_b200/csrc/engine.cu
--- a/gmvae_b200/csrc/engine.cu
+++ b/gmvae_b200/csrc/engine.cu
@@ -207,6 +207,10 @@
   bool chain_pair = false;
   struct FuseReq { int kind = 0; unsigned char prm[tc::CHAIN_EPI2_BYTES]; std::vector<std::pair<const void*, size_t>> writes; bool consumed = false; };
   FuseReq fuse_next;
+  struct ZFwdReq { bool on = false; tc::ZFuseFwd prm; tc::Operand w_dec0; int zn = 0; };
+  ZFwdReq zfwd_next;
+  bool zfuse_opt = true;
+  bool zfuse = false;
   bool last_gemm_chained = false;
   std::map<const void*, bool> relu_bits_valid;
   bool det = false;
@@ -535,7 +539,10 @@
   static_assert(tc::epi_kind<Epi>::value != tc::EK_NONE, "epilogue not supported by the chained kernel");
   static_assert(sizeof(Epi) <= tc::CHAIN_EPI_BYTES, "epilogue parameters do not fit the job record");
   const bool pair = h->chain_pair, quad = h->chain_quad;
-  const void* reads[4] = {A1.ptr, A2 ? A2->ptr : nullptr, a_mn ? (const void*)B1.ptr : nullptr, epi.read_ptr()};
+  const gmvae_handle::ZFwdReq* zf = (h->zfwd_next.on && tc::epi_kind<Epi>::value == tc::EK_STORE_BF16) ? &h->zfwd_next : nullptr;
+  GM_REQUIRE(!zf || (pair && !quad && !A2 && !a_mn && b_mn), "compound z job: CTA-pair plan, one K segment");
+  const void* reads[4] = {A1.ptr, A2 ? A2->ptr : nullptr, a_mn ? (const void*)B1.ptr : nullptr,
+                          zf ? (const void*)zf->prm.prior_out : epi.read_ptr()};
   tc::ChainDep deps[tc::CHAIN_MAX_DEPS]; int ndeps = 0, epi_dep = -1;
   bool need_flush = h->chain.njobs >= tc::CHAIN_MAX_JOBS || h->chain.nmaps + 6 > tc::CHAIN_MAX_MAPS;
   for (int i = 0; i < 4 && !need_flush; ++i) {
@@ -580,9 +587,11 @@
   } else {
     J.a2 = J.a1; J.b2 = J.b1;
   }
+  if (zf) GM_TRY(mk(&J.b2, zf->w_dec0, true, b_box_rows));
   const int kb_total = J.kb1 + J.kb2;
   tc::chain_job_geometry(J, M, N, block_n, split_k, kb_total, a_mn, quad ? 4 : pair ? 2 : 1);
-  J.b_mn = b_mn ? 1 : 0; J.kind = tc::epi_kind<Epi>::value;
+  J.zn = zf ? zf->zn : 0;
+  J.b_mn = b_mn ? 1 : 0; J.kind = zf ? (int)tc::EK_ZFWD : tc::epi_kind<Epi>::value;
   J.tile_base = h->chain_tiles;
   {
     const int part = h->part_on ? h->cur_part : 0;
@@ -624,6 +633,14 @@
   memset(J.epi, 0, sizeof(J.epi));
   memcpy(J.epi, &epi, sizeof(Epi));
   J.fuse = 0;
+  if (zf) {
+    memset(J.epi2, 0, sizeof(J.epi2));
+    memcpy(J.epi2, &zf->prm, sizeof(zf->prm));
+    const int Z = zf->prm.Z;
+    h->chain_writers.push_back({reinterpret_cast<const char*>(zf->prm.enc_out), reinterpret_cast<const char*>(zf->prm.enc_out + (size_t)M * 2 * Z), h->chain.njobs});
+    h->chain_writers.push_back({reinterpret_cast<const char*>(zf->prm.z_act), reinterpret_cast<const char*>(zf->prm.z_act + (size_t)M * Z), h->chain.njobs});
+    h->zfwd_next.on = false;
+  }
   if (h->fuse_next.kind != 0 && tc::epi_kind<Epi>::value == tc::EK_STORE_F32 && N <= 16 && J.sig_base >= 0) {
     J.fuse = h->fuse_next.kind;
     memcpy(J.epi2, h->fuse_next.prm, sizeof(J.epi2));
@@ -1048,7 +1065,7 @@
   } else {
     GM_TRY(mlp_hidden_fwd<A>(h, h->encoder, enc, x_act, Dp, D, B, 0, st));
   }
-  if (nl > 1 || !gm) {
+  if ((nl > 1 || !gm) && !h->zfuse) {
     EpiStore<float> epi{enc_out, (int64_t)2 * Z, h->params + enc_last.b_off, nullptr, 0, 0, 1.f};
     GM_TRY(lin_fwd<A>(h, nl == 1 ? x_act : enc.hid[nl - 2], nl == 1 ? Dp : hid_ld(nl - 2), B, view(h, enc_last, 0, nl == 1 ? D : -1),
                       epi, st));
@@ -1107,6 +1124,14 @@
     const int x = split_env;
     if (x >= 4 && W - x >= 4) { h->part_on = true; h->part_walkers = W; h->part_chain_walkers = x; }
   }
+  {
+    const int Z = h->Z, nl = h->L, model = h->cfg.model;
+    const int n2 = nl > 1 ? h->decoder.layers[0].out : 0;
+    h->zfuse = h->zfuse_opt && h->chain_pair && !h->chain_quad && !h->part_on && model != GMVAE_MODEL_VAE_GMP &&
+               (Z == 16 || Z == 32 || Z == 64) && nl > 1 && (n2 <= 128 || h->wide_bn == 0) && !(h->debug_flags & DBG_BN128) &&
+               (eps_in == nullptr || aligned16(eps_in)) && h->buf<float>("z_f32") == nullptr;
+    h->zfwd_next.on = false;
+  }
   if (h->chain_on) GM_CHECK_CUDA(cudaMemsetAsync(h->chain_counters, 0, (size_t)h->chain_counter_cap * 4, st));
   int r = forward_backward_body<A>(h, x_u8, B, Bg, eps_in, u_in, st);
   if (r == 0) r = chain_flush(h, st);
@@ -1115,7 +1140,7 @@
     h->det_colsums.clear();
     if (r == 0) r = det_reduce(h, st);
   }
-  h->chain_on = false; h->chain_pair = false; h->chain_quad = false; h->chain.njobs = 0; h->chain.nmaps = 0;
+  h->chain_on = false; h->chain_pair = false; h->chain_quad = false; h->chain.njobs = 0; h->chain.nmaps = 0; h->zfuse = false;
   return r;
 }
 
@@ -1172,7 +1197,28 @@
     const bool v4 = std::is_same<A, bf16>::value && Z % 4 == 0 && Z <= 256 && aligned16(eps) && aligned16(enc_out) &&
                     (prior_mode != 2 || aligned16(prior_out));
     const bool rows_ok = h->chain_on && h->row_jobs && v4 && prior_mode != 1 && z_f32 == nullptr;
-    if (rows_ok) {
+    if constexpr (std::is_same<A, bf16>::value) {
+      if (h->zfuse) {
+        GM_REQUIRE(aligned16(eps) && v4, "compound z job: 16-byte aligned eps rows");
+        const Linear& l0 = h->decoder.layers[0];
+        LinView Lh = view(h, enc_last), L0 = view(h, l0, 0, Z);
+        const int64_t ldin = hid_ld(nl - 2);
+        h->zfwd_next.on = true;
+        h->zfwd_next.prm = tc::ZFuseFwd{h->params + enc_last.b_off, enc_out, eps, gm ? prior_out : nullptr, z_act, acc, Z,
+                                        c.raw_sigma_bias, c.sigma_min, inv_bg};
+        h->zfwd_next.w_dec0 = tc::Operand{L0.w_bf16, L0.ld_w, L0.out, L0.in};
+        h->zfwd_next.zn = 2 * Z;
+        EpiStore<A> epi{dec.hid[0], (int64_t)ldp(l0.out), L0.b, nullptr, 0, 1, 1.f};
+        if (tc::CHAIN_RELU_BITS && !(h->debug_flags & DBG_NO_RELU_BITS)) { epi.relu_bits = dec.bits[0]; epi.ld_bits = round_up(B, 32); }
+        tc::Operand a{enc.hid[nl - 2], ldin, B, kpad(Lh.in, ldin)}, b{Lh.w_bf16, Lh.ld_w, Lh.out, Lh.in};
+        const int n2 = l0.out, bn2 = n2 <= 64 ? 64 : n2 <= 128 ? 128 : 256;
+        GM_TRY(chain_add(h, a, b, nullptr, nullptr, B, n2, bn2, false, true, 1, epi, st));
+        GM_REQUIRE(!h->zfwd_next.on, "compound z job not recorded");
+        h->relu_bits_valid[dec.hid[0]] = epi.relu_bits != nullptr;
+      }
+    }
+    if (h->zfuse) {
+    } else if (rows_ok) {
       tc::RowsZFwd prm{enc_out, eps, prior_out, prior_mode, Z, c.raw_sigma_bias, c.sigma_min, inv_bg, reinterpret_cast<bf16*>(z_act), Zp, acc};
       GM_TRY(chain_add_rows(h, tc::EK_ROWS_Z_FWD, prm, B, {enc_out, eps, prior_out}, {{z_act, (size_t)B * Zp * 2}}, st, 4));
     } else {
@@ -1199,7 +1245,7 @@
     GM_LAUNCHED(h, st, PC_HEADS);
   }
   bool dec_bias_fused = false;
-  GM_TRY(mlp_hidden_fwd<A>(h, h->decoder, dec, z_act, Zp, Z, B, 0, st));
+  GM_TRY(mlp_hidden_fwd<A>(h, h->decoder, dec, z_act, Zp, Z, B, h->zfuse ? 1 : 0, st));
   {
     const Linear& l = h->decoder.layers[nl - 1];
     const A* in = nl == 1 ? z_act : dec.hid[nl - 2];
@@ -1566,6 +1612,7 @@
   if (const char* q = getenv("GMVAE_CHAIN_QUAD")) h->quad_opt_in = atoi(q) != 0;
   if (const char* q = getenv("GMVAE_CHAIN_SPLIT")) h->chain_split_opt = atoi(q);
   if (const char* bnv = getenv("GMVAE_CHAIN_BN")) { const int v = atoi(bnv); if (v == 128 || v == 192) h->wide_bn = v; }
+  if (const char* zv = getenv("GMVAE_ZFUSE")) h->zfuse_opt = atoi(zv) != 0;
   plan(h);
   GM_CHECK_CUDA(cudaMalloc(&h->state, sizeof(DeviceState)));
   DeviceState s0; s0.step = 0; s0.seed = 0x243F6A8885A308D3ull; s0.adam_blocks = 0; s0.pad = 0; s0.beta1_power = 1.0; s0.beta2_power = 1.0;
diff --git a/gmvae_b200/csrc/gemm_chain.cuh b/gmvae_b200/csrc/gemm_chain.cuh
--- a/gmvae_b200/csrc/gemm_chain.cuh
+++ b/gmvae_b200/csrc/gemm_chain.cuh
@@ -6,6 +6,7 @@
 namespace tc {
 
 enum EpiKind : int { EK_NONE = -1, EK_STORE_BF16 = 0, EK_STORE_F32 = 1, EK_BCE = 2, EK_RELUMASK = 3, EK_ATOMIC = 4,
+                     EK_ZFWD = 5,
                      EK_ROWS_FIRST = 16, EK_ROWS_Y_FWD = 16, EK_ROWS_Z_FWD = 17, EK_ROWS_Z_BWD = 18, EK_ROWS_Y_BWD = 19 };
 
 struct RowsYFwd { const float* logits; const float* u; int K; float inv_T, inv_bg; float* y_f32; bf16* y_act; int ld_yact; float* acc; };
@@ -13,6 +14,9 @@
                   bf16* z_act; int ld_z; float* acc; };
 struct RowsZBwd { const float* enc_out; const float* eps; const float* prior_out; const float* dz_dec; int prior_mode, Z; float c, sigma_min, inv_bg;
                   bf16* d_enc_out; bf16* d_prior_out; int ld_out; float* db_enc; float* db_prior; };
+struct ZFuseFwd { const float* bias; float* enc_out; const float* eps; const float* prior_out; bf16* z_act; float* acc; int Z;
+                  float c, sigma_min, inv_bg; };
+static_assert(sizeof(ZFuseFwd) <= CHAIN_EPI2_BYTES, "z head parameters fit the job record");
 struct RowsYBwd { const float* logits; const float* y_f32; const float* dy; int K; float inv_T, inv_bg; bf16* dlogits; int ld_out; float* db; };
 template <class Epi> struct epi_kind { static constexpr int value = EK_NONE; };
 template <> struct epi_kind<EpiStore<bf16, EPI_PLAIN>> { static constexpr int value = EK_STORE_BF16; };
@@ -34,7 +38,8 @@
 constexpr int CHAIN_STAGE_BYTES_PAIR = A_STAGE_BYTES + 128 * BLOCK_K * 2;
 static_assert(CHAIN_STAGES_PAIR * CHAIN_STAGE_BYTES_PAIR <= CHAIN_STAGES * CHAIN_STAGE_BYTES, "both modes use the same ring area");
 constexpr int CHAIN_PATCH_BYTES = 2048;
-constexpr int CHAIN_CARVE_BYTES = CHAIN_STAGES * CHAIN_STAGE_BYTES + EPI_WARPS * CHAIN_PATCH_BYTES + 256  + 256 * 4  + 256 * 4 ;
+constexpr int CHAIN_CARVE_BYTES = CHAIN_STAGES * CHAIN_STAGE_BYTES + EPI_WARPS * CHAIN_PATCH_BYTES + 256  + 256 * 4  + 256 * 4  +
+                                  16 ;
 constexpr int CHAIN_SMEM_BYTES = 232448;
 static_assert(CHAIN_CARVE_BYTES + 512 <= CHAIN_SMEM_BYTES, "shared-memory budget");
 
@@ -94,6 +99,7 @@
 struct ChainShared {
   uint8_t* smem; uint64_t* full_bar; uint64_t* empty_bar; uint64_t* tmem_full_bar; uint64_t* tmem_empty_bar;
   uint8_t* patches; float* sbias_all; float* scs_all; uint32_t tmem_base; uint64_t* op_bar;
+  uint64_t* zop_bar;
 };
 
 __device__ __forceinline__ void tma_store_2d(const CUtensorMap* m, uint32_t src, int c0, int c1) {
@@ -267,9 +273,112 @@
   if ((lane & 1) == 0 && col < K && t != 0.f) atomicAdd(scs + col, t);
 }
 
-template <class Epi, int KIND, int CL>
+__device__ __forceinline__ float z_head_fwd_elem(float mu, float raw, float e, float mp, float rp, int prior_mode, float c, float sigma_min,
+                                                 float& z) {
+  const float sg = fmaxf(fast_softplus(raw + c), sigma_min);
+  z = fmaf(sg, e, mu);
+  float d = -0.5f * e * e;
+  if (prior_mode == 0) {
+    d = fmaf(0.5f * z, z, d) - __logf(sg);
+  } else if (prior_mode == 2) {
+    const float sp = fmaxf(fast_softplus(rp + c), sigma_min);
+    const float isp = __fdividef(1.f, sp);
+    const float tt = (z - mp) * isp;
+    d = fmaf(0.5f * tt, tt, d) - __logf(sg * isp);
+  } else {
+    d -= __logf(sg);
+  }
+  return d;
+}
+
+template <int CL>
+__device__ __noinline__ float zfwd_head_unit(const ChainJob& J, const int* counters, const ChainShared& S, int it, int q, bool first, int mb,
+                                             int warp, int lane) {
+  constexpr bool PAIR = CL >= 2;
+  const ZFuseFwd& zp = *reinterpret_cast<const ZFuseFwd*>(J.epi2);
+  const int Z = zp.Z, quad = warp & 3, slot = (warp - 2) >> 2, j0 = slot * 16;
+  const int m0 = mb * BLOCK_M, r = quad * 32 + lane;
+  const int64_t m = m0 + r;
+  const bool mine = j0 < Z, valid = mine && m < J.M, store = valid && first;
+  const int as = it & 1; const uint32_t ap = (it >> 1) & 1;
+  const int prior_mode = zp.prior_out ? 2 : 0;
+  if (prior_mode == 2 && mine && m0 < J.M && J.epi_dep >= 0) {
+    if (lane == 0) wait_counter(counters + J.deps[J.epi_dep].base + mb, J.deps[J.epi_dep].target);
+    __syncwarp();
+  }
+  float e[16], mp[16], rp[16];
+#pragma unroll
+  for (int i = 0; i < 16; i += 4) {
+    float4 a = make_float4(0.f, 0.f, 0.f, 0.f), b = a, c = a;
+    if (valid) {
+      a = __ldcg(reinterpret_cast<const float4*>(zp.eps + m * Z + j0 + i));
+      if (prior_mode == 2) {
+        b = __ldcg(reinterpret_cast<const float4*>(zp.prior_out + m * 2 * Z + j0 + i));
+        c = __ldcg(reinterpret_cast<const float4*>(zp.prior_out + m * 2 * Z + Z + j0 + i));
+      }
+    }
+    e[i] = a.x; e[i + 1] = a.y; e[i + 2] = a.z; e[i + 3] = a.w;
+    mp[i] = b.x; mp[i + 1] = b.y; mp[i + 2] = b.z; mp[i + 3] = b.w;
+    rp[i] = c.x; rp[i + 1] = c.y; rp[i + 2] = c.z; rp[i + 3] = c.w;
+  }
+  mbar_wait(&S.tmem_full_bar[as], ap);
+  tc_fence_after();
+  float kl = 0.f;
+  uint4 lo = make_uint4(0, 0, 0, 0), hi = lo;
+  if (mine) {
+    const uint32_t taddr = S.tmem_base + ((uint32_t)(quad * 32) << 16) + (uint32_t)(as * 256);
+    uint32_t rm[16], rr[16];
+    tmem_ld16_issue(taddr + j0, rm);
+    tmem_ld16_issue(taddr + Z + j0, rr);
+    tmem_ld16_wait(rm);
+    tmem_ld16_wait(rr);
+    const float* zb = S.scs_all;
+    float mu[16], raw[16], z[16];
+#pragma unroll
+    for (int i = 0; i < 16; ++i) {
+      mu[i] = fmaf(__uint_as_float(rm[i]), 1.f, zb[j0 + i]);
+      raw[i] = fmaf(__uint_as_float(rr[i]), 1.f, zb[Z + j0 + i]);
+    }
+    if (store) {
+      float4* o = reinterpret_cast<float4*>(zp.enc_out + m * 2 * Z + j0);
+      float4* o2 = reinterpret_cast<float4*>(zp.enc_out + m * 2 * Z + Z + j0);
+#pragma unroll
+      for (int i = 0; i < 4; ++i) {
+        o[i] = make_float4(mu[4 * i], mu[4 * i + 1], mu[4 * i + 2], mu[4 * i + 3]);
+        o2[i] = make_float4(raw[4 * i], raw[4 * i + 1], raw[4 * i + 2], raw[4 * i + 3]);
+      }
+    }
+    if (valid) {
+      float d = 0.f;
+#pragma unroll
+      for (int i = 0; i < 16; ++i) d += z_head_fwd_elem(mu[i], raw[i], e[i], mp[i], rp[i], prior_mode, zp.c, zp.sigma_min, z[i]);
+      if (first) kl = d;
+      pack16(z, lo, hi);
+      if (store) {
+        uint4* dz = reinterpret_cast<uint4*>(zp.z_act + m * Z + j0);
+        dz[0] = lo; dz[1] = hi;
+      }
+    }
+  }
+  const int st = q % CHAIN_STAGES_PAIR;
+  mbar_wait(&S.empty_bar[st], ((uint32_t)(q / CHAIN_STAGES_PAIR) & 1) ^ 1);
+  const uint32_t tile = smem_addr(S.smem + st * CHAIN_STAGE_BYTES_PAIR);
+  sts128(patch_unit<128>(tile, r, 2 * slot), lo);
+  sts128(patch_unit<128>(tile, r, 2 * slot + 1), hi);
+  fence_proxy_async();
+  fence_proxy_async_global();
+  tc_fence_before();
+  __syncwarp();
+  if (lane == 0) {
+    if (PAIR) { mbar_arrive_leader(S.zop_bar); mbar_arrive_leader(&S.tmem_empty_bar[as]); }
+    else { mbar_arrive(S.zop_bar); mbar_arrive(&S.tmem_empty_bar[as]); }
+  }
+  return kl;
+}
+
+template <class Epi, int KIND, int CL, bool ZF = false>
 __device__ __forceinline__ void chain_epilogue_job(const ChainJob& J, const CUtensorMap* maps, int* counters, const ChainShared& S, int& it,
-                                                   uint32_t& op_phase, int warp, int lane, long long* trace, int jidx,
+                                                   int& kq, uint32_t& op_phase, int warp, int lane, long long* trace, int jidx,
                                                    unsigned long long* jobstat = nullptr, int abl = 0) {
   constexpr int CW = 16;
   constexpr bool PAIR = CL >= 2;
@@ -302,9 +411,20 @@
       scs_all[i] = 0.f;
     }
   };
+  float zkl = 0.f;
+  if constexpr (ZF) {
+    const ZFuseFwd& zp = *reinterpret_cast<const ZFuseFwd*>(J.epi2);
+    asm volatile("bar.sync 1, %0;" ::"n"(EPI_WARPS * 32) : "memory");
+    for (int i = et; i < 2 * zp.Z; i += EPI_WARPS * 32) scs_all[i] = __ldg(zp.bias + i);
+    asm volatile("bar.sync 1, %0;" ::"n"(EPI_WARPS * 32) : "memory");
+  }
   for (int l = first; l < J.walk_total; l += wstride, ++it) {
     int z, mb, n0;
     chain_tile<CL>(J, l, rank, z, mb, n0);
+    if constexpr (CL == 2) {
+      if constexpr (ZF) zkl += zfwd_head_unit<CL>(J, counters, S, it++, kq + J.kb1, n0 == 0, mb, warp, lane);
+      kq += chain_tile_ring_blocks(J, l);
+    }
     const int m0 = mb * BLOCK_M;
     const int as = it & 1; const uint32_t ap = (it >> 1) & 1;
     const int mrow0 = m0 + quad * 32;
@@ -343,7 +463,7 @@
     if (tr) { trace[16 * it + 6] = clock64(); trace[16 * it + 15] = jidx; trace[16 * it + 14] = l; }
     const bool js = jobstat && e == 0 && lane == 0;
     unsigned long long js_t0 = 0, js_t1 = 0;
-    if (J.epi_dep >= 0 && m0 < M) {
+    if (!ZF && J.epi_dep >= 0 && m0 < M) {
       if (lane == 0) { wait_counter(counters + J.deps[J.epi_dep].base + mb, J.deps[J.epi_dep].target); fence_proxy_async_global(); }
       __syncwarp();
     }
@@ -595,6 +715,12 @@
       atomicAdd(jobstat + 8 * jidx + 6, 1ull);
     }
   }
+  if constexpr (ZF) {
+    const ZFuseFwd& zp = *reinterpret_cast<const ZFuseFwd*>(J.epi2);
+    const float s = warp_sum(zkl);
+    if (lane == 0 && s != 0.f) acc_add(zp.acc, ACC_KL, s * zp.inv_bg);
+    asm volatile("bar.sync 1, %0;" ::"n"(EPI_WARPS * 32) : "memory");
+  }
   epi.finish_warp();
   if constexpr (KIND == EK_STORE_F32) {
     if (J.fuse == EK_ROWS_Y_FWD) {
@@ -658,22 +784,7 @@
         const float* MU = &mu.x; const float* RAW = &raw.x; const float* E = &e4.x; const float* MP = &mp.x; const float* RP = &rp.x;
         float z[4];
 #pragma unroll
-        for (int q = 0; q < 4; ++q) {
-          const float sg = fmaxf(fast_softplus(RAW[q] + prm.c), prm.sigma_min);
-          z[q] = fmaf(sg, E[q], MU[q]);
-          float d = -0.5f * E[q] * E[q];
-          if (prm.prior_mode == 0) {
-            d = fmaf(0.5f * z[q], z[q], d) - __logf(sg);
-          } else if (prm.prior_mode == 2) {
-            const float sp = fmaxf(fast_softplus(RP[q] + prm.c), prm.sigma_min);
-            const float isp = __fdividef(1.f, sp);
-            const float tt = (z[q] - MP[q]) * isp;
-            d = fmaf(0.5f * tt, tt, d) - __logf(sg * isp);
-          } else {
-            d -= __logf(sg);
-          }
-          red_acc += d;
-        }
+        for (int q = 0; q < 4; ++q) red_acc += z_head_fwd_elem(MU[q], RAW[q], E[q], MP[q], RP[q], prm.prior_mode, prm.c, prm.sigma_min, z[q]);
         *reinterpret_cast<uint2*>(prm.z_act + (int64_t)b * prm.ld_z + j) = make_uint2(pack_bf16x2(z[0], z[1]), pack_bf16x2(z[2], z[3]));
       }
     } else if constexpr (KIND == EK_ROWS_Z_BWD) {
@@ -801,6 +912,7 @@
   uint32_t* tmem_slot = reinterpret_cast<uint32_t*>(op_bar + EPI_WARPS);
   float* sbias_all = reinterpret_cast<float*>(reinterpret_cast<uint8_t*>(bars) + 256);
   float* scs_all = sbias_all + 256;
+  uint64_t* zop_bar = reinterpret_cast<uint64_t*>(scs_all + 256);
 
   const int warp = threadIdx.x >> 5, lane = threadIdx.x & 31;
   const int G = (int)gridDim.x / CL, c = (int)blockIdx.x / CL;
@@ -813,6 +925,7 @@
     for (int s = 0; s < STAGES; ++s) { mbar_init(&full_bar[s], 1); mbar_init(&empty_bar[s], QUAD ? 2 : 1); }
     for (int s = 0; s < 2; ++s) { mbar_init(&tmem_full_bar[s], 1); mbar_init(&tmem_empty_bar[s], PAIR ? 2 * EPI_WARPS : EPI_WARPS); }
     for (int s = 0; s < EPI_WARPS; ++s) mbar_init(&op_bar[s], 1);
+    if (CL == 2) mbar_init(zop_bar, 2 * EPI_WARPS);
     fence_barrier_init();
   } else if (warp == 1) {
     if (PAIR) tmem_alloc_pair(tmem_slot, 512); else tmem_alloc(tmem_slot, 512);
@@ -834,8 +947,9 @@
     for (int j = 0; j < p.njobs; ++j) {
       const ChainJob& J = p.jobs[j];
       if (J.kind >= EK_ROWS_FIRST) continue;
-      const int BN = J.block_n, kb1 = J.kb1, kb_total = J.kb1 + J.kb2, a_mn = J.a_mn, b_mn = J.b_mn, ndeps = J.ndeps;
-      const int JM = J.M, JN = J.N, kps = J.kb_per_split, walk_total = J.walk_total, share = J.share;
+      const int zn = J.zn;
+      const int BN = zn ? zn : J.block_n, kb1 = J.kb1, kb_total = J.kb1 + J.kb2, a_mn = J.a_mn, b_mn = J.b_mn, ndeps = J.ndeps;
+      const int JM = J.M, JN = zn ? zn : J.N, kps = J.kb_per_split, walk_total = J.walk_total, share = J.share;
       const CUtensorMap* const ta1 = &p.maps[J.a1];
       const CUtensorMap* const tb1 = &p.maps[J.b1];
       const CUtensorMap* const ta2 = &p.maps[J.a2];
@@ -853,8 +967,9 @@
         chain_tile<CL>(J, l, crank, z, mb, n0);
         const int m0 = mb * BLOCK_M;
         const bool real = a_mn || m0 < JM;
-        const int n_eff = min(BN, (JN - n0 + 15) & ~15);
-        const int nb = PAIR ? n0 + rank * (n_eff >> 1) : n0;
+        const int n0g = zn ? 0 : n0;
+        const int n_eff = min(BN, (JN - n0g + 15) & ~15);
+        const int nb = PAIR ? n0g + rank * (n_eff >> 1) : n0g;
         const int kb_begin = z * kps, kb_end = min(kb_total, kb_begin + kps);
         const bool tr = trace && pit < 64 && lane == 0;
         if (tr) trace[16 * pit + 0] = clock64();
@@ -931,16 +1046,31 @@
           }
           if (++stage == STAGES) { stage = 0; phase ^= 1; }
         }
+        if constexpr (CL == 2) {
+          if (zn) {
+            const int slabs2 = ((J.block_n >> 1) + 63) / 64, ne = min(J.block_n, (J.N - n0 + 15) & ~15);
+            mbar_wait(&empty_bar[stage], phase ^ 1);
+            uint64_t* const fb = &full_bar[stage];
+            uint8_t* const sb = smem + stage * STAGE_BYTES + A_STAGE_BYTES;
+            if (elect_one()) {
+              if (rank == 0) mbar_expect_tx(fb, 2u * (uint32_t)(slabs2 * BLOCK_K * 128));
+              for (int i = 0; i < slabs2; ++i) tma_load_2d_pair(tb2, fb, sb + i * (BLOCK_K * 128), n0 + rank * (ne >> 1) + i * 64, 0);
+            }
+            if (++stage == STAGES) { stage = 0; phase ^= 1; }
+          }
+        }
         if (tr) trace[16 * pit + 2] = clock64();
       }
     }
   } else if (warp == 1) {
     int stage = 0; uint32_t phase = 0;
     int it = 0;
+    uint32_t zphase = 0;
     for (int j = 0; (!PAIR || rank == 0) && j < p.njobs; ++j) {
       const ChainJob& J = p.jobs[j];
       if (J.kind >= EK_ROWS_FIRST) continue;
-      const int kb_total = J.kb1 + J.kb2, kps = J.kb_per_split, walk_total = J.walk_total, BN = J.block_n, JN = J.N;
+      const int zn = J.zn;
+      const int kb_total = J.kb1 + J.kb2, kps = J.kb_per_split, walk_total = J.walk_total, BN = zn ? zn : J.block_n, JN = zn ? zn : J.N;
       const int a_mn = J.a_mn, b_mn = J.b_mn;
       const uint32_t idesc0 = (1u << 4) | (1u << 7) | (1u << 10) | ((uint32_t)a_mn << 15) | ((uint32_t)b_mn << 16) |
                               ((uint32_t)((PAIR ? 2 * BLOCK_M : BLOCK_M) >> 4) << 24);
@@ -954,7 +1084,7 @@
         chain_tile<CL>(J, l, crank, z, mb_unused, n0);
         const int kb_begin = z * kps, kb_end = min(kb_total, kb_begin + kps);
         const int as = it & 1; const uint32_t ap = (it >> 1) & 1;
-        const int n_eff = min(BN, (JN - n0 + 15) & ~15);
+        const int n_eff = min(BN, (JN - (zn ? 0 : n0) + 15) & ~15);
         const uint32_t idesc = idesc0 | ((uint32_t)(n_eff >> 3) << 17);
         const bool tr = trace && it < 64 && lane == 0;
         if (tr) trace[16 * it + 3] = clock64();
@@ -991,20 +1121,47 @@
         }
         if (tr) trace[16 * it + 5] = clock64();
         if (p.jobstat && lane == 0) { atomicAdd(p.jobstat + 8 * j + 3, gtimer() - js_t1); atomicAdd(p.jobstat + 8 * j + 7, js_t1 - js_t0); }
+        if constexpr (CL == 2) {
+          if (zn) {
+            ++it;
+            const int as2 = it & 1; const uint32_t ap2 = (it >> 1) & 1;
+            const int ne = min(J.block_n, (J.N - n0 + 15) & ~15);
+            mbar_wait(&tmem_empty_bar[as2], ap2 ^ 1);
+            mbar_wait(zop_bar, zphase);
+            zphase ^= 1;
+            mbar_wait(&full_bar[stage], phase);
+            tc_fence_after();
+            const uint32_t sa = smem_u32(smem + stage * STAGE_BYTES);
+            const uint64_t adesc = make_smem_desc_rt(sa, 0);
+            const uint64_t bdesc = bdesc_hi | (uint64_t)(((sa + A_STAGE_BYTES) & 0x3FFFF) >> 4);
+            if (elect_one()) {
+#pragma unroll
+              for (int k = 0; k < BLOCK_K / UMMA_K; ++k)
+                umma_bf16_pair(adesc + (uint64_t)k * a_step, bdesc + (uint64_t)k * b_step, tmem_base + (uint32_t)(as2 * 256),
+                               idesc0 | ((uint32_t)(ne >> 3) << 17), k > 0 ? 1u : 0u);
+              umma_commit_pair(&empty_bar[stage]);
+              umma_commit_pair(&tmem_full_bar[as2]);
+            }
+            if (++stage == STAGES) { stage = 0; phase ^= 1; }
+          }
+        }
       }
     }
   } else {
-    ChainShared S{smem, full_bar, empty_bar, tmem_full_bar, tmem_empty_bar, patches, sbias_all, scs_all, tmem_base, op_bar};
-    int it = 0;
+    ChainShared S{smem, full_bar, empty_bar, tmem_full_bar, tmem_empty_bar, patches, sbias_all, scs_all, tmem_base, op_bar, zop_bar};
+    int it = 0, kq = 0;
     uint32_t op_phase = 0;
     for (int j = 0; j < p.njobs; ++j) {
       const ChainJob& J = p.jobs[j];
       switch (J.kind) {
-        case EK_STORE_BF16: chain_epilogue_job<EpiStore<bf16, EPI_PLAIN>, EK_STORE_BF16, CL>(J, p.maps, p.counters, S, it, op_phase, warp, lane, trace, j, p.jobstat, p.abl); break;
-        case EK_STORE_F32: chain_epilogue_job<EpiStore<float, EPI_PLAIN>, EK_STORE_F32, CL>(J, p.maps, p.counters, S, it, op_phase, warp, lane, trace, j, p.jobstat, p.abl); break;
-        case EK_BCE: chain_epilogue_job<EpiBCE<bf16>, EK_BCE, CL>(J, p.maps, p.counters, S, it, op_phase, warp, lane, trace, j, p.jobstat, p.abl); break;
-        case EK_RELUMASK: chain_epilogue_job<EpiReluMask<bf16, bf16>, EK_RELUMASK, CL>(J, p.maps, p.counters, S, it, op_phase, warp, lane, trace, j, p.jobstat, p.abl); break;
-        case EK_ATOMIC: chain_epilogue_job<EpiAtomicAdd, EK_ATOMIC, CL>(J, p.maps, p.counters, S, it, op_phase, warp, lane, trace, j, p.jobstat, p.abl); break;
+        case EK_STORE_BF16: chain_epilogue_job<EpiStore<bf16, EPI_PLAIN>, EK_STORE_BF16, CL>(J, p.maps, p.counters, S, it, kq, op_phase, warp, lane, trace, j, p.jobstat, p.abl); break;
+        case EK_STORE_F32: chain_epilogue_job<EpiStore<float, EPI_PLAIN>, EK_STORE_F32, CL>(J, p.maps, p.counters, S, it, kq, op_phase, warp, lane, trace, j, p.jobstat, p.abl); break;
+        case EK_BCE: chain_epilogue_job<EpiBCE<bf16>, EK_BCE, CL>(J, p.maps, p.counters, S, it, kq, op_phase, warp, lane, trace, j, p.jobstat, p.abl); break;
+        case EK_RELUMASK: chain_epilogue_job<EpiReluMask<bf16, bf16>, EK_RELUMASK, CL>(J, p.maps, p.counters, S, it, kq, op_phase, warp, lane, trace, j, p.jobstat, p.abl); break;
+        case EK_ATOMIC: chain_epilogue_job<EpiAtomicAdd, EK_ATOMIC, CL>(J, p.maps, p.counters, S, it, kq, op_phase, warp, lane, trace, j, p.jobstat, p.abl); break;
+        case EK_ZFWD:
+          if constexpr (CL == 2) chain_epilogue_job<EpiStore<bf16, EPI_PLAIN>, EK_STORE_BF16, CL, true>(J, p.maps, p.counters, S, it, kq, op_phase, warp, lane, trace, j, p.jobstat, p.abl);
+          break;
 #ifndef GMVAE_NO_ROWS
         case EK_ROWS_Y_FWD: chain_rows_job<EK_ROWS_Y_FWD, RowsYFwd, CL>(J, p.counters, S, warp, lane, p.jobstat, j, p.abl); break;
         case EK_ROWS_Z_FWD: chain_rows_job<EK_ROWS_Z_FWD, RowsZFwd, CL>(J, p.counters, S, warp, lane, p.jobstat, j, p.abl); break;
```

After: 40.64 million (median of 6 runs). -11.1%, worse.
